# senresearch/BulkLMM.jl

Hardware: AMD Instinct MI355X
Metric: trait x marker LOD tests/sec (higher is better)
Workload: dtype f64

## Files before the change

### bulklmm.jl_amd/csrc/blmm_api.hip

```cpp
#include "blmm_internal.h"
#include "fastmath.h"
#include <algorithm>
#include <cmath>
#include <cstddef>
#include <chrono>
#include <cstring>
#include <limits>
#include <cstdlib>
#include <mutex>

using namespace blmm;

namespace blmm {

int fail(blmm_ctx* ctx, int code, const std::string& msg) {
  if (ctx) ctx->err = msg;
  return code;
}

int ensure(blmm_ctx* ctx, DevBuf& b, size_t bytes) {
  if (&b == &ctx->outL) clear_last(ctx);
  if (&b == &ctx->outL || &b == &ctx->outP) ctx->last_P = nullptr;
  if (bytes == 0) bytes = 8;
  if (b.cap >= bytes) return BLMM_OK;
// ... 223 lines not shown
  return {dCovar, ncov, add_int, ncov + add_int};
}

int prepare_eigen(blmm_ctx* ctx, const blmm_opts* o, int64_t n, const double* dCovar, int64_t ncov, const double* dK,
                  const double* dweights, int centered, Pipe& P, Timer& tm, const EigPre* pre = nullptr) {
  ctx->prep_valid = false;
  if (n < 1 || ncov < 0) return fail(ctx, BLMM_ERR_DIM, "Dimension mismatch.");
  if (n > 2048) return fail(ctx, BLMM_ERR_UNSUPPORTED, "more than 2048 individuals: the device eigensolver (tridiagonalisation + divide and conquer) stops at n = 2048");
  const NullCov nc = null_cov(o, dCovar, ncov);
  const int c = (int)nc.c;
  if (c < 1 || c > CMAX) return fail(ctx, BLMM_ERR_UNSUPPORTED, BLMM_C_ERR);
  if (c >= n) return fail(ctx, BLMM_ERR_DIM, "Dimension mismatch.");
  P.n = (int)n; P.c = c; P.npad = (int)round_up(n, 8); P.ldr = (int)round_up(P.npad, 16);
  int rc;
  if ((rc = ensure(ctx, ctx->U, sizeof(double) * n * n))) return rc;
  if ((rc = ensure(ctx, ctx->lam, sizeof(double) * n))) return rc;
  if ((rc = ensure(ctx, ctx->Zs, sizeof(double) * n * c))) return rc;
  if ((rc = ensure(ctx, ctx->Z0, sizeof(double) * n * c))) return rc;
  if ((rc = ensure(ctx, ctx->Rp, sizeof(double) * (size_t)P.npad * P.ldr))) return rc;
  P.Z0 = ptr<double>(ctx->Z0); P.lam = ptr<double>(ctx->lam);
  if (pre) {
    P.stat = pre->stat;
    ctx->audit_ran = false;
    ctx->brent_cnt_used = false;
    P.big = n > jacobi_lds_max_n();
    bool post_done = false;
    tm.mark();
    if ((rc = launch_jacobi_post(ctx, pre->Ks, pre->V, (int)n, pre->lraw, P.stat, ptr<double>(ctx->Zs), dweights, c, P.npad, P.ldr,
                                 o->decomp_scheme, centered, P.lam, ptr<double>(ctx->U), P.Z0, ptr<double>(ctx->Rp), &post_done))) return rc;
    if (!post_done && (rc = launch_post_eigen(ctx, pre->lraw, pre->V, ptr<double>(ctx->Zs), dweights, (int)n, c, P.npad, P.ldr,
                                              o->decomp_scheme, centered, P.lam, ptr<double>(ctx->U), P.Z0, ptr<double>(ctx->Rp), P.stat))) return rc;
    tm.mark();
    return BLMM_OK;
  }
  if ((rc = ensure(ctx, ctx->Ks, sizeof(double) * n * n))) return rc;
  if ((rc = ensure(ctx, ctx->V, sizeof(double) * (n * n + 4 * n + 16)))) return rc;
  if ((rc = ensure(ctx, ctx->lraw, sizeof(double) * n))) return rc;
  if ((rc = reset_stat(ctx, &P.stat))) return rc;
  tm.mark();
  if ((rc = launch_design(ctx, dK, nc.d, (int)nc.ncov, nc.add_int, dweights, (int)n, ptr<double>(ctx->Ks), ptr<double>(ctx->Zs)))) return rc;
  const double* evec = ptr<double>(ctx->V);
  const char* eig_env = dev_env("BLMM_EIGEN");
  if (!eig_env && ctx->tune.eigen_solver == 1) eig_env = "jacobi";
  if (!eig_env && ctx->tune.eigen_solver == 2) eig_env = "dc";
  const bool big = n > jacobi_lds_max_n();
  P.big = big;
  bool done = false, post_done = false;
  const bool want_dc = eig_env ? std::strcmp(eig_env, "dc") == 0 : big;
  if (!done && want_dc && n >= 3) {
    rc = launch_eig_dc(ctx, ptr<double>(ctx->Ks), (int)n, ptr<double>(ctx->lraw), ptr<double>(ctx->V), P.stat);
    if (rc == BLMM_OK) { done = true; P.big = true; }
    else if (rc != BLMM_ERR_UNSUPPORTED) return rc;
  }
  if (!done) {
    const bool want_fast = !(eig_env && std::strcmp(eig_env, "jacobi") == 0) && n >= 3 && n <= eig_fast_max_n();
    if (want_fast) {
      rc = launch_eig_fast(ctx, ptr<double>(ctx->Ks), (int)n, ptr<double>(ctx->lraw), ptr<double>(ctx->V), P.stat);
      if (rc != BLMM_OK && rc != BLMM_ERR_UNSUPPORTED) return rc;
    }
    if ((rc = launch_jacobi_post(ctx, ptr<double>(ctx->Ks), ptr<double>(ctx->V), (int)n, ptr<double>(ctx->lraw), P.stat, ptr<double>(ctx->Zs),
                                 dweights, c, P.npad, P.ldr, o->decomp_scheme, centered, P.lam, ptr<double>(ctx->U), P.Z0, ptr<double>(ctx->Rp),
                                 &post_done))) return rc;
  }
  if (!post_done && (rc = launch_post_eigen(ctx, ptr<double>(ctx->lraw), evec, ptr<double>(ctx->Zs), dweights, (int)n, c,
                              P.npad, P.ldr, o->decomp_scheme, centered, P.lam, ptr<double>(ctx->U), P.Z0,
                              ptr<double>(ctx->Rp), P.stat))) return rc;
  tm.mark();
  return BLMM_OK;
}

static int flush_upload(blmm_ctx* ctx) {
  if (!ctx->up_pending) return BLMM_OK;
  ctx->up_pending = false;
  for (int i = 0; i < 2; ++i) {
    if (ctx->up_bytes[i]) BLMM_HIP(hipMemcpyAsync(ctx->up_dst[i], ctx->up_src[i], ctx->up_bytes[i], hipMemcpyHostToDevice, ctx->copy));
    if (i == 0) BLMM_HIP(hipEventRecord(ctx->ev_inY, ctx->copy));
  }
  BLMM_HIP(hipEventRecord(ctx->ev_in, ctx->copy));
  ctx->in_wait = true;
  return BLMM_OK;
}

int rotate_markers(blmm_ctx* ctx, Pipe& P, const double* dG, int64_t p);
int start_wbasis(blmm_ctx* ctx, Pipe& P, const double* dG = nullptr, int64_t p = 0, bool xt_recorded = false) {
  int rc;
  const int64_t n = P.n;
  const LrSeg seg = lr_segments(ctx, P.n);
  if ((rc = ensure(ctx, ctx->wbQ, sizeof(double) * (size_t)seg.S * P.npad * n))) return rc;
  if ((rc = ensure(ctx, ctx->wbW, sizeof(double) * (size_t)n * (256 + 16)))) return rc;
  if ((rc = ensure(ctx, ctx->wbRk, sizeof(int) * 4 * LR_SEG_MAX))) return rc;
  if (!xt_recorded) BLMM_HIP(hipEventRecord(ctx->ev_xt, ctx->stream));
  BLMM_HIP(hipStreamWaitEvent(ctx->side, ctx->ev_xt, 0));
  ctx->wb_on_side2 = false;
  if (!dG) {
    OnStream on(ctx, ctx->side);
    return launch_wbasis(ctx, P.lam, (int)n, P.npad, seg, ptr<double>(ctx->wbW), ptr<double>(ctx->wbQ), ptr<int>(ctx->wbRk), P.stat);
  }
  {
    BLMM_HIP(hipStreamWaitEvent(ctx->side2, ctx->ev_xt, 0));
    ctx->wb_on_side2 = true;
    OnStream on(ctx, ctx->side2);
    if ((rc = launch_wbasis(ctx, P.lam, (int)n, P.npad, seg, ptr<double>(ctx->wbW), ptr<double>(ctx->wbQ), ptr<int>(ctx->wbRk), P.stat))) return rc;
  }
  OnStream on(ctx, ctx->side);
  if (ctx->in_wait) BLMM_HIP(hipStreamWaitEvent(ctx->side, ctx->ev_in, 0));
  if ((rc = rotate_markers(ctx, P, dG, p))) return rc;
  BLMM_HIP(hipEventRecord(ctx->ev_wb, ctx->side));
  return BLMM_OK;
}

int rotate_traits(blmm_ctx* ctx, Pipe& P, const double* dY, int64_t m) {
  if (m < 0) return fail(ctx, BLMM_ERR_DIM, "Dimension mismatch.");
  P.m = m; P.ldy = round_up(m > 0 ? m : 1, 128);
  int rc = ensure(ctx, ctx->Yt, sizeof(double) * (size_t)P.npad * P.ldy);
  if (rc) return rc;
  P.Yt = ptr<double>(ctx->Yt);
  return launch_rotate(ctx, ptr<double>(ctx->Rp), P.ldr, P.n, P.npad, dY, m, P.Yt, P.ldy, P.ldy);
}
int rotate_markers(blmm_ctx* ctx, Pipe& P, const double* dG, int64_t p) {
  if (p < 0) return fail(ctx, BLMM_ERR_DIM, "Dimension mismatch.");
  P.p = p; P.ldx = round_up(p > 0 ? p : 1, 128);
  int rc = ensure(ctx, ctx->Xt, sizeof(double) * (size_t)P.npad * P.ldx);
  if (rc) return rc;
  P.Xt = ptr<double>(ctx->Xt);
  return launch_rotate(ctx, ptr<double>(ctx->Rp), P.ldr, P.n, P.npad, dG, p, P.Xt, P.ldx, P.ldx);
}

int prepare(blmm_ctx* ctx, const blmm_opts* o, const double* dY, int64_t n, int64_t m, const double* dG, int64_t p,
            const double* dCovar, int64_t ncov, const double* dK, const double* dweights, int centered, Pipe& P, Timer& tm,
            bool early_wbasis = false, bool grid_side = false, bool skip_markers = false, const EigPre* pre = nullptr) {
  if (m < 0 || p < 0) return fail(ctx, BLMM_ERR_DIM, "Dimension mismatch.");
  const bool forks = m > 0 && p > 0 && (early_wbasis || grid_side);
  ctx->stop_event_used = false;
  ctx->stop_event_next = forks ? ctx->ev_xt : nullptr;
  int rc = prepare_eigen(ctx, o, n, dCovar, ncov, dK, dweights, centered, P, tm, pre);
  const bool xt_recorded = ctx->stop_event_used;
  ctx->stop_event_next = nullptr; ctx->stop_event_used = false;
  if (rc) return rc;
  if (ctx->up_pending) {
    if ((rc = flush_upload(ctx))) return rc;
    BLMM_HIP(hipStreamWaitEvent(ctx->stream, ctx->ev_inY, 0));
  }
  const bool up_flight = ctx->in_wait;
  static const bool rot_side = !(dev_env("BLMM_ROTATE_SIDE") && dev_env("BLMM_ROTATE_SIDE")[0] == '0');
  const bool side_g = early_wbasis && m > 0 && p > 0 && rot_side && n <= 160;
  if (early_wbasis && m > 0 && p > 0 && (rc = start_wbasis(ctx, P, side_g ? dG : nullptr, p, xt_recorded))) return rc;
  P.xt_side = side_g;
  if (grid_side && !early_wbasis && m > 0 && p > 0 && rot_side && n <= 160) {
    if (!xt_recorded) BLMM_HIP(hipEventRecord(ctx->ev_xt, ctx->stream));
    BLMM_HIP(hipStreamWaitEvent(ctx->side, ctx->ev_xt, 0));
    if (ctx->in_wait) BLMM_HIP(hipStreamWaitEvent(ctx->side, ctx->ev_in, 0));
    OnStream on(ctx, ctx->side);
    if ((rc = rotate_markers(ctx, P, dG, p))) return rc;
    P.xt_side = true;
  }
  if ((rc = rotate_traits(ctx, P, dY, m))) return rc;
  if (skip_markers) { P.p = p; P.ldx = round_up(p > 0 ? p : 1, 128); P.Xt = nullptr; }
  else if (!P.xt_side) {
    if (up_flight) BLMM_HIP(hipStreamWaitEvent(ctx->stream, ctx->ev_in, 0));
    if ((rc = rotate_markers(ctx, P, dG, p))) return rc;
  }
  ctx->in_wait = false;
  tm.mark();
  return BLMM_OK;
}

NullModel null_model(const Pipe& P, const blmm_opts* o) {
  NullModel nm;
  nm.n = P.n; nm.c = P.c; nm.npad = P.npad; nm.reml = o->reml ? 1 : 0;
  nm.optim_interval = o->optim_interval < 1 ? 1 : o->optim_interval;
  nm.prior_a = o->prior_variance; nm.prior_b = o->prior_sample_size;
  return nm;
}

int stage_to_device(blmm_ctx* ctx, DevBuf& dst, const void* src, size_t bytes) {
  blmm_ctx::GridSlot* slot = nullptr;
  for (auto& g : ctx->gstage)
    if (g.cap >= bytes && (!g.used || hipEventQuery(g.ev) == hipSuccess)) { slot = &g; break; }
  if (!slot) {
    blmm_ctx::GridSlot g;
    g.cap = bytes < 4096 ? 4096 : bytes;
    void* h = nullptr;
    BLMM_HIP(hipHostMalloc(&h, g.cap, hipHostMallocDefault));
    g.h = h;
    if (hipEventCreateWithFlags(&g.ev, hipEventDisableTiming) != hipSuccess) { (void)hipHostFree(h); return fail(ctx, BLMM_ERR_HIP, "hipEventCreate failed"); }
    ctx->gstage.push_back(g);
    slot = &ctx->gstage.back();
  }
  std::memcpy(slot->h, src, bytes);
  BLMM_HIP(hipMemcpyAsync(dst.p, slot->h, bytes, hipMemcpyHostToDevice, ctx->stream));
  BLMM_HIP(hipEventRecord(slot->ev, ctx->stream));
  slot->used = true;
  return BLMM_OK;
}

int check_grid(blmm_ctx* ctx, const double* h2_grid_host, int64_t ngrid) {
  if (!h2_grid_host || ngrid < 1) return fail(ctx, BLMM_ERR_INVALID, "h2 grid is empty");
  for (int64_t g = 0; g < ngrid; ++g) {
    const double h = h2_grid_host[g];
    if (std::isinf(h / (1.0 - h))) return fail(ctx, BLMM_ERR_H2_ONE, "Heritability of 1 is not allowed.");
  }
  return BLMM_OK;
}

int grid_to_device(blmm_ctx* ctx, const double* h2_grid_host, int64_t ngrid, double** out) {
  int rc;
  if ((rc = check_grid(ctx, h2_grid_host, ngrid)) || (rc = ensure(ctx, ctx->gridd, sizeof(double) * ngrid))) return rc;
  const size_t bytes = sizeof(double) * (size_t)ngrid;
  if (ctx->grid_async) {
    if ((rc = stage_to_device(ctx, ctx->gridd, h2_grid_host, bytes))) return rc;
  } else {
    BLMM_HIP(hipMemcpyAsync(ctx->gridd.p, h2_grid_host, bytes, hipMemcpyHostToDevice, ctx->stream));
    BLMM_HIP(hipStreamSynchronize(ctx->stream));
  }
  *out = ptr<double>(ctx->gridd);
  return BLMM_OK;
}

ScanArgs scan_args(blmm_ctx* ctx, const Pipe& P, const double* panels, int64_t ldp, double* L, int64_t ldL, int64_t m) {
  ScanArgs a;
  a.Xt = P.Xt; a.ldx = P.ldx; a.P = panels; a.ldp = ldp; a.pstride = (int64_t)P.npad * ldp;
  a.ks = P.npad / 4; a.n = P.n; a.p = P.p; a.m = m; a.L = L; a.ldL = ldL;
  a.isx = nullptr; a.ld_isx = 0; a.bin = nullptr; a.stat = P.stat; a.logtab = ptr<double>(ctx->logtab); a.lodtab = ptr<double>(ctx->lodtab);
  a.Pv = ctx->pv_cur; a.ldPv = ctx->pv_cur_ld; a.pvtab = ptr<double>(ctx->pvtab);
  a.red = ctx->red_cur;
  a.c = P.c;
  lod_poly5_host(-0.5 * (double)P.n, a.lodc);
  return a;
}

double lr_tolerance(const blmm_ctx* ctx) {
  const char* e = dev_env("BLMM_LR_TOL");
  return e ? atof(e) : ctx->tune.lr_tol;
}

int64_t lr_ldq(const Pipe& P) { return P.ldy + 128 + LR_TILE * LR_SEG_MAX; }
static LrRegion lr_region(const Pipe& P, int r) {
  LrRegion rg;
  rg.col0 = r * lr_ldq(P); rg.ncol = lr_ldq(P); rg.counts = P.stat + ST_LR_SHARED0 + 2 * r; rg.segcnt = P.stat + 24 + 20 * r;
  return rg;
}

int lr_begin(blmm_ctx* ctx, const Pipe& P, bool wbasis_started) {
  int rc;
  ctx->lr_last_ldq = lr_ldq(P); ctx->lr_last_m = P.m;
  const int64_t ldp = 2 * lr_ldq(P), tstride = (int64_t)P.npad * P.ldx;
  if ((rc = ensure(ctx, ctx->lrPerm, sizeof(int) * (size_t)ldp))) return rc;
  if ((rc = ensure(ctx, ctx->lrDen0, sizeof(double) * (size_t)P.ldx))) return rc;
  const LrSeg seg = lr_segments(ctx, P.n);
  if ((rc = ensure(ctx, ctx->lrT, sizeof(double) * (size_t)seg.S * (1 + P.c) * tstride))) return rc;
  if ((rc = ensure(ctx, ctx->lrC, sizeof(double) * (size_t)P.npad * ldp))) return rc;
  if ((rc = ensure(ctx, ctx->lrL, sizeof(double) * (size_t)(P.c * (P.c + 1) / 2) * ldp))) return rc;
  if ((rc = ensure(ctx, ctx->lrFlag, sizeof(int) * (size_t)ldp))) return rc;
  if ((rc = ensure(ctx, ctx->lrPart, sizeof(double) * 2 * (size_t)((P.n + 63) / 64) * ldp))) return rc;
  if ((rc = ensure(ctx, ctx->panels, sizeof(double) * (size_t)P.npad * ldp))) return rc;
  if ((rc = ensure(ctx, ctx->wbQ, sizeof(double) * (size_t)seg.S * P.npad * P.n))) return rc;
  if ((rc = ensure(ctx, ctx->wbW, sizeof(double) * (size_t)P.n * (256 + 16)))) return rc;
  if ((rc = ensure(ctx, ctx->wbRk, sizeof(int) * 4 * LR_SEG_MAX))) return rc;
  int* rk = ptr<int>(ctx->wbRk);
  if (!(wbasis_started && P.xt_side)) {
    BLMM_HIP(hipEventRecord(ctx->ev_fork, ctx->stream));
    BLMM_HIP(hipStreamWaitEvent(ctx->side, ctx->ev_fork, 0));
  }
  const bool on2 = wbasis_started && P.xt_side && ctx->wb_on_side2;
  hipStream_t lr_side = on2 ? ctx->side2 : ctx->side;
  OnStream on(ctx, lr_side);
  if (!wbasis_started && (rc = launch_wbasis(ctx, P.lam, P.n, P.npad, seg, ptr<double>(ctx->wbW), ptr<double>(ctx->wbQ), rk, P.stat))) return rc;
  BLMM_HIP(hipEventRecord(ctx->ev_q, lr_side));
  if (on2) BLMM_HIP(hipStreamWaitEvent(lr_side, ctx->ev_wb, 0));
  if ((rc = launch_lr_tpanels(ctx, P.Xt, P.ldx, P.p, P.n, P.c, P.npad, P.Z0, ptr<double>(ctx->wbQ), rk, seg, ptr<double>(ctx->lrT), tstride,
                              ptr<double>(ctx->lrDen0)))) return rc;
  BLMM_HIP(hipEventRecord(ctx->ev_join, lr_side));
  return BLMM_OK;
}

namespace {
double lr_shared_tol(const blmm_ctx* ctx) {
  const char* e = dev_env("BLMM_LR_SHARED");
  const bool on = e ? e[0] != '0' : ctx->tune.lr_shared != 0;
  return on ? lr_tolerance(ctx) : 0.0;
}
LrArgs lr_args(blmm_ctx* ctx, const Pipe& P, const LrRegion& rg, double* dL, int64_t ldL) {
  const int64_t ldp = 2 * lr_ldq(P);
  LrArgs la;
  la.s = scan_args(ctx, P, ptr<double>(ctx->panels), ldp, dL, ldL, P.m + 192 < rg.ncol ? P.m + 192 : rg.ncol);
  la.Cp = ptr<double>(ctx->lrC); la.T = ptr<double>(ctx->lrT); la.tstride = (int64_t)P.npad * P.ldx; la.Ls = ptr<double>(ctx->lrL);
  la.rk = ptr<int>(ctx->wbRk); la.c = P.c; la.perm = ptr<int>(ctx->lrPerm); la.rg = rg; la.den0 = ptr<double>(ctx->lrDen0);
  la.skip_shared = 0;
  la.seg = lr_segments(ctx, P.n);
  return la;
}
int lr_region_scan(blmm_ctx* ctx, const Pipe& P, const LrRegion& rg, double* dL, int64_t ldL) {
  static const bool lean = !(dev_env("BLMM_LR_LEAN") && dev_env("BLMM_LR_LEAN")[0] == '0');
  static const bool serial = dev_env("BLMM_LR_SERIAL") && dev_env("BLMM_LR_SERIAL")[0] == '1';
  if (serial) { (void)hipStreamSynchronize(ctx->side); (void)hipStreamSynchronize(ctx->side2); (void)hipStreamSynchronize(ctx->stream); }
  LrArgs la = lr_args(ctx, P, rg, dL, ldL);
  int rc;
  if (lean) {
    ScanArgs a = la.s;
    a.isx = la.den0; a.ld_isx = P.ldx; a.bin = nullptr;
    a.perm = la.perm; a.col0 = rg.col0; a.count = rg.counts;
    if ((rc = launch_scan_shared(ctx, a))) return rc;
    la.skip_shared = 1;
  }
  return launch_scan_lr(ctx, la);
}
int lr_region_panels(blmm_ctx* ctx, const Pipe& P, const NullModel& nm, const double* dh2, const LrRegion& rg) {
  return launch_lr_panels(ctx, nm, P.Yt, P.ldy, P.m, P.Z0, P.lam, dh2, ptr<double>(ctx->wbQ), ptr<int>(ctx->wbRk), lr_segments(ctx, P.n), ptr<int>(ctx->lrPerm),
                          rg, ptr<double>(ctx->panels), ptr<double>(ctx->lrC), ptr<double>(ctx->lrL), 2 * lr_ldq(P), P.stat);
}
int lr_region_resid(blmm_ctx* ctx, const Pipe& P, const NullModel& nm, const double* dh2, const LrRegion& rg) {
  OnStream on(ctx, ctx->side);
  return launch_lr_resid(ctx, nm, P.m, lr_tolerance(ctx), P.lam, dh2, ptr<double>(ctx->wbQ), ptr<int>(ctx->wbRk), lr_segments(ctx, P.n), ptr<int>(ctx->lrPerm), rg,
                         ptr<double>(ctx->lrC), 2 * lr_ldq(P), ptr<int>(ctx->lrFlag), ptr<double>(ctx->lrPart), P.stat, ctx->red_cur.flags);
}
int lr_fix(blmm_ctx* ctx, const Pipe& P, const NullModel& nm, const double* dh2, double* dL, int64_t ldL) {
  if (ctx->red_cur.pmax && !ctx->red_cur.flags) return BLMM_OK;
  return launch_scan_fix(ctx, nm, P.Xt, P.ldx, P.p, ptr<double>(ctx->panels), ptr<double>(ctx->lrL), 2 * lr_ldq(P), P.Z0, P.lam, dh2,
                         ptr<int>(ctx->lrFlag), ptr<int>(ctx->lrPerm), dL, ldL, P.stat, ctx->red_cur);
}
}

int illcond_rescan(blmm_ctx* ctx, const Pipe& P, const NullModel& nm, int64_t m, const double* dh2, double* dL, int64_t ldL) {
  if (P.c < 2 || m <= 0 || P.p <= 0) return BLMM_OK;
  int rc = ensure(ctx, ctx->illList, sizeof(int) * (size_t)m);
  if (rc) return rc;
  const bool patch = ctx->red_cur.pmax && ctx->red_cur.flags;
  if (!patch && (rc = launch_illcond_flag(ctx, nm, m, P.Z0, P.lam, dh2, ptr<int>(ctx->illList), P.stat))) return rc;
  if (ctx->red_cur.pmax && !patch) return BLMM_OK;
  return launch_scan_qr(ctx, nm, P.Yt, P.ldy, P.Xt, P.ldx, P.p, P.Z0, P.lam, dh2, ptr<int>(ctx->illList), dL, ldL, P.stat, ctx->red_cur);
}

int lr_finish(blmm_ctx* ctx, const Pipe& P, const NullModel& nm, const double* dh2, double* dL, int64_t ldL, Timer& tm) {
  int rc;
  const LrRegion rg = lr_region(P, 0);
  const LrSeg seg = lr_segments(ctx, P.n);
  hipStream_t main_stream = ctx->stream;
  BLMM_HIP(hipStreamWaitEvent(main_stream, ctx->ev_join, 0));
  if ((rc = launch_lr_classify(ctx, P.n, P.m, lr_shared_tol(ctx), P.lam, dh2, nullptr, nullptr, nullptr, ptr<int>(ctx->lrPerm), rg, seg))) return rc;
  if ((rc = lr_region_panels(ctx, P, nm, dh2, rg))) return rc;
  tm.mark();
  const bool ahead = ctx->red_cur.flags != nullptr;
  if (ahead && P.c >= 2 && (rc = ensure(ctx, ctx->illList, sizeof(int) * (size_t)P.m))) return rc;
  BLMM_HIP(hipEventRecord(ctx->ev_fork, main_stream));
  BLMM_HIP(hipStreamWaitEvent(ctx->side, ctx->ev_fork, 0));
  if ((rc = lr_region_resid(ctx, P, nm, dh2, rg))) return rc;
  if (ahead && P.c >= 2) {
    OnStream on(ctx, ctx->side);
    if ((rc = launch_illcond_flag(ctx, nm, P.m, P.Z0, P.lam, dh2, ptr<int>(ctx->illList), P.stat, ctx->red_cur.flags))) return rc;
  }
  BLMM_HIP(hipEventRecord(ctx->ev_join, ctx->side));
  if (ahead && ctx->red_cur.want_trip) BLMM_HIP(hipStreamWaitEvent(main_stream, ctx->ev_join, 0));
// ... 30 lines not shown
        (rc = lr_region_panels(ctx, P, nm, dh2, r1))) return rc;
  }
  BLMM_HIP(hipEventRecord(ctx->ev_b2, ctx->side2));
  tm.mark();
  BLMM_HIP(hipStreamWaitEvent(ctx->side, ctx->ev_b1, 0));
  if ((rc = lr_region_resid(ctx, P, nm, dh2, r0))) return rc;
  const bool ahead = ctx->red_cur.flags != nullptr && ctx->red_cur.want_trip;
  if (ahead) {
    BLMM_HIP(hipEventRecord(ctx->ev_join, ctx->side));
    BLMM_HIP(hipStreamWaitEvent(main_stream, ctx->ev_join, 0));
  }
  if ((rc = lr_region_scan(ctx, P, r0, dL, ldL))) return rc;
  BLMM_HIP(hipStreamWaitEvent(ctx->side, ctx->ev_b2, 0));
  if ((rc = lr_region_resid(ctx, P, nm, dh2, r1))) return rc;
  BLMM_HIP(hipEventRecord(ctx->ev_join, ctx->side));
  BLMM_HIP(hipStreamWaitEvent(main_stream, ctx->ev_b2, 0));
  if (ahead) BLMM_HIP(hipStreamWaitEvent(main_stream, ctx->ev_join, 0));
  if ((rc = lr_region_scan(ctx, P, r1, dL, ldL))) return rc;
  BLMM_HIP(hipStreamWaitEvent(main_stream, ctx->ev_join, 0));
  if ((rc = lr_fix(ctx, P, nm, dh2, dL, ldL))) return rc;
  if ((rc = illcond_rescan(ctx, P, nm, P.m, dh2, dL, ldL))) return rc;
  tm.mark();
  return BLMM_OK;
}

}

extern "C" {

int blmm_version(void) { return BLMM_VERSION; }

int blmm_device_count(void) {
  int n = 0;
  if (hipGetDeviceCount(&n) != hipSuccess) return 0;
  return n;
}

const char* blmm_err_string(int code) {
  switch (code) {
    case BLMM_OK: return "ok";
    case BLMM_ERR_INVALID: return "invalid argument";
    case BLMM_ERR_DIM: return "Dimension mismatch.";
    case BLMM_ERR_H2_ONE: return "Heritability of 1 is not allowed.";
    case BLMM_ERR_DECOMP: return "Please choose either `eigen` or `svd` for decomposition of the kinship matrix.";
    case BLMM_ERR_METHOD: return "unknown bulkscan method";
    case BLMM_ERR_ONE_TRAIT: return "Can only handle one trait.";
    case BLMM_ERR_NO_INTERCEPT: return "Intercept has to be added when no other covariate is given.";
    case BLMM_ERR_ZERO_NORM: return "Dividing by zeros: the input vector can not contain any zeros!";
    case BLMM_ERR_NPERMS: return "The required number of permutations must be a positive integer.";
    case BLMM_ERR_UNSUPPORTED: return "unsupported configuration";
    case BLMM_ERR_NO_DEVICE: return "no usable HIP device";
    case BLMM_ERR_HIP: return "HIP runtime error";
    case BLMM_ERR_ALLOC: return "device allocation failed";
  }
  return "unknown error";
}

int blmm_create(int device_id, void* hip_stream, blmm_ctx** out) {
  if (!out) return BLMM_ERR_INVALID;
  *out = nullptr;
  int ndev = 0;
  if (hipGetDeviceCount(&ndev) != hipSuccess || ndev <= 0 || device_id < 0 || device_id >= ndev) return BLMM_ERR_NO_DEVICE;
  if (hipSetDevice(device_id) != hipSuccess) return BLMM_ERR_NO_DEVICE;
  blmm_ctx* ctx = new blmm_ctx();
  ctx->device = device_id;
  if (hip_stream == BLMM_STREAM_NULL) {
    ctx->stream = nullptr;
  } else if (hip_stream) {
    ctx->stream = reinterpret_cast<hipStream_t>(hip_stream);
  } else {
    if (hipStreamCreateWithFlags(&ctx->stream, hipStreamNonBlocking) != hipSuccess) { delete ctx; return BLMM_ERR_HIP; }
    ctx->own_stream = true;
  }
  if (hipStreamCreateWithFlags(&ctx->side, hipStreamNonBlocking) != hipSuccess ||
      hipEventCreateWithFlags(&ctx->ev_fork, hipEventDisableTiming) != hipSuccess ||
      hipEventCreateWithFlags(&ctx->ev_join, hipEventDisableTiming) != hipSuccess ||
      hipEventCreateWithFlags(&ctx->ev_xt, hipEventDisableTiming) != hipSuccess ||
      hipStreamCreateWithFlags(&ctx->side2, hipStreamNonBlocking) != hipSuccess ||
      hipEventCreateWithFlags(&ctx->ev_b1, hipEventDisableTiming) != hipSuccess ||
      hipEventCreateWithFlags(&ctx->ev_b2, hipEventDisableTiming) != hipSuccess ||
      hipEventCreateWithFlags(&ctx->ev_q, hipEventDisableTiming) != hipSuccess ||
      hipEventCreateWithFlags(&ctx->ev_m, hipEventDisableTiming) != hipSuccess ||
      hipEventCreateWithFlags(&ctx->ev_wb, hipEventDisableTiming) != hipSuccess ||
      hipStreamCreateWithFlags(&ctx->copy, hipStreamNonBlocking) != hipSuccess ||
      hipEventCreateWithFlags(&ctx->ev_in, hipEventDisableTiming) != hipSuccess ||
      hipEventCreateWithFlags(&ctx->ev_inY, hipEventDisableTiming) != hipSuccess ||
      hipEventCreateWithFlags(&ctx->ev_call, hipEventDisableTiming) != hipSuccess) {
    blmm_destroy(ctx);
    return BLMM_ERR_HIP;
  }
  {
    int cus = 0;
    if (hipDeviceGetAttribute(&cus, hipDeviceAttributeMultiprocessorCount, device_id) == hipSuccess) ctx->num_cus = cus;
    void* hp = nullptr;
    if (hipHostMalloc(&hp, 64, hipHostMallocMapped) != hipSuccess) { blmm_destroy(ctx); return BLMM_ERR_HIP; }
    std::memset(hp, 0, 64);
    ctx->hflag = reinterpret_cast<volatile int64_t*>(hp);
  }
  if (ensure(ctx, ctx->logtab, sizeof(blmm_log_table_host)) != BLMM_OK ||
      hipMemcpy(ctx->logtab.p, blmm_log_table_host, sizeof(blmm_log_table_host), hipMemcpyHostToDevice) != hipSuccess ||
      ensure(ctx, ctx->lodtab, sizeof(blmm_lod_table_host)) != BLMM_OK ||
      hipMemcpy(ctx->lodtab.p, blmm_lod_table_host, sizeof(blmm_lod_table_host), hipMemcpyHostToDevice) != hipSuccess ||
      ensure(ctx, ctx->pvtab, sizeof(blmm_pv_table_host)) != BLMM_OK ||
      hipMemcpy(ctx->pvtab.p, blmm_pv_table_host, sizeof(blmm_pv_table_host), hipMemcpyHostToDevice) != hipSuccess) {
    blmm_destroy(ctx);
    return BLMM_ERR_HIP;
  }
  *out = ctx;
  return BLMM_OK;
}

void blmm_destroy(blmm_ctx* ctx) {
  if (!ctx) return;
  hipSetDevice(ctx->device);
  hipStreamSynchronize(ctx->stream);
  DevBuf* bufs[] = {&ctx->Ks, &ctx->V, &ctx->lam, &ctx->U, &ctx->Zs, &ctx->Z0, &ctx->Rp, &ctx->Yt, &ctx->Xt, &ctx->panels,
                    &ctx->iyy, &ctx->h2, &ctx->h2idx, &ctx->sig2, &ctx->ell, &ctx->isx, &ctx->stat, &ctx->gridd, &ctx->misc,
                    &ctx->EllTab, &ctx->inY, &ctx->inG, &ctx->inK, &ctx->inCov, &ctx->inW, &ctx->outL, &ctx->outH2,
                    &ctx->tmpA, &ctx->tmpB, &ctx->tmpC, &ctx->perm, &ctx->r0, &ctx->altbuf, &ctx->logtab, &ctx->lraw,
                    &ctx->wbQ, &ctx->wbW, &ctx->wbRk, &ctx->lrT, &ctx->lrC, &ctx->lrL, &ctx->lrFlag, &ctx->lrPart, &ctx->lrPerm, &ctx->lrDen0, &ctx->eigW, &ctx->xf32, &ctx->pf32, &ctx->brSt, &ctx->brList, &ctx->illList, &ctx->qrSlab, &ctx->lodtab, &ctx->dynFac, &ctx->pvtab, &ctx->outP, &ctx->redbuf, &ctx->redtrip, &ctx->altC, &ctx->rf32, &ctx->btG, &ctx->redflag, &ctx->bperm,
                    &ctx->locoK, &ctx->locoPart, &ctx->locoChr, &ctx->locoStat, &ctx->locoKs, &ctx->locoV, &ctx->locoLraw};
  for (DevBuf* b : bufs) if (b->p) hipFree(b->p);
  for (auto& s : ctx->evsets) for (auto& e : s.e) (void)hipEventDestroy(e);
  if (ctx->side) { (void)hipStreamSynchronize(ctx->side); (void)hipStreamDestroy(ctx->side); }
  if (ctx->ev_fork) (void)hipEventDestroy(ctx->ev_fork);
  if (ctx->ev_join) (void)hipEventDestroy(ctx->ev_join);
  if (ctx->ev_xt) (void)hipEventDestroy(ctx->ev_xt);
  if (ctx->ev_b1) (void)hipEventDestroy(ctx->ev_b1);
  if (ctx->ev_b2) (void)hipEventDestroy(ctx->ev_b2);
  if (ctx->ev_q) (void)hipEventDestroy(ctx->ev_q);
  if (ctx->ev_m) (void)hipEventDestroy(ctx->ev_m);
  if (ctx->ev_wb) (void)hipEventDestroy(ctx->ev_wb);
  if (ctx->ev_in) (void)hipEventDestroy(ctx->ev_in);
  if (ctx->ev_inY) (void)hipEventDestroy(ctx->ev_inY);
  if (ctx->ev_call) (void)hipEventDestroy(ctx->ev_call);
  for (auto& g : ctx->gstage) {
    if (g.ev) { (void)hipEventSynchronize(g.ev); (void)hipEventDestroy(g.ev); }
    if (g.h) (void)hipHostFree(g.h);
  }
  if (ctx->copy) { (void)hipStreamSynchronize(ctx->copy); (void)hipStreamDestroy(ctx->copy); }
  if (ctx->side2) { (void)hipStreamSynchronize(ctx->side2); (void)hipStreamDestroy(ctx->side2); }
  if (ctx->own_stream) hipStreamDestroy(ctx->stream);
  if (ctx->hflag) (void)hipHostFree(const_cast<int64_t*>(ctx->hflag));
  destroy_host_stage(ctx->hstage);
  delete ctx;
}

const char* blmm_last_error(const blmm_ctx* ctx) { return ctx ? ctx->err.c_str() : "ctx is NULL"; }

int blmm_set_stream(blmm_ctx* ctx, void* hip_stream) {
  if (!ctx) return BLMM_ERR_INVALID;
  hipStreamSynchronize(ctx->stream);
  if (ctx->own_stream) { hipStreamDestroy(ctx->stream); ctx->own_stream = false; }
  if (hip_stream == BLMM_STREAM_NULL) ctx->stream = nullptr;
  else if (hip_stream) ctx->stream = reinterpret_cast<hipStream_t>(hip_stream);
  else {
    if (hipStreamCreateWithFlags(&ctx->stream, hipStreamNonBlocking) != hipSuccess) return fail(ctx, BLMM_ERR_HIP, "hipStreamCreate");
    ctx->own_stream = true;
  }
  return BLMM_OK;
}

int blmm_set_timing(blmm_ctx* ctx, int on) {
  if (!ctx) return BLMM_ERR_INVALID;
  ctx->timing = on != 0;
  return BLMM_OK;
}

int blmm_read_timings(blmm_ctx* ctx, double* sums_ms, int64_t* ncalls) {
  if (!ctx || !sums_ms || !ncalls) return BLMM_ERR_INVALID;
  BLMM_HIP(hipStreamSynchronize(ctx->stream));
  for (int i = 0; i < 6; ++i) sums_ms[i] = 0.0;
  for (size_t k = 0; k < ctx->ev_used; ++k) {
    double t[6];
    phase_times(ctx->evsets[k], t);
    for (int i = 0; i < 6; ++i) sums_ms[i] += t[i];
  }
  *ncalls = (int64_t)ctx->ev_used;
  ctx->ev_used = 0;
  return BLMM_OK;
}

int blmm_lowrank_profile(blmm_ctx* ctx, int64_t* out) {
  if (!ctx || !out) return BLMM_ERR_INVALID;
  for (int i = 0; i < 2 + 2 * LR_SEG_MAX; ++i) out[i] = 0;
  if (!ctx->stat.p || !ctx->wbRk.p) return BLMM_OK;
  BLMM_HIP(hipSetDevice(ctx->device));
  int64_t h[NSTAT];
  int rk[4 * LR_SEG_MAX];
  BLMM_HIP(hipMemcpyAsync(h, ctx->stat.p, sizeof(h), hipMemcpyDeviceToHost, ctx->stream));
  BLMM_HIP(hipMemcpyAsync(rk, ctx->wbRk.p, sizeof(rk), hipMemcpyDeviceToHost, ctx->stream));
  BLMM_HIP(hipStreamSynchronize(ctx->stream));
  int S = 0;
  for (int s = 0; s < LR_SEG_MAX; ++s) {
    const int64_t cnt = h[24 + s] + h[44 + s];
    if (cnt > 0) { S = s + 1; out[2 + 2 * s] = cnt; out[3 + 2 * s] = rk[4 * s]; }
  }
  out[0] = S; out[1] = h[ST_LR_SHARED0] + h[ST_LR_SHARED1];
  return BLMM_OK;
}

int blmm_lowrank_columns(blmm_ctx* ctx, int64_t m, int32_t* col_out, int64_t* region_width, int64_t* counts_out) {
  if (!ctx || !col_out || m < 0) return BLMM_ERR_INVALID;
  for (int64_t j = 0; j < m; ++j) col_out[j] = -1;
  if (region_width) *region_width = ctx->lr_last_ldq;
  if (counts_out) for (int i = 0; i < 4; ++i) counts_out[i] = 0;
  if (!ctx->lrPerm.p || !ctx->stat.p || ctx->lr_last_ldq <= 0) return BLMM_OK;
  BLMM_HIP(hipSetDevice(ctx->device));
  const int64_t ldq = ctx->lr_last_ldq;
  std::vector<int> perm((size_t)(2 * ldq));
  int64_t h[NSTAT];
  BLMM_HIP(hipMemcpyAsync(perm.data(), ctx->lrPerm.p, sizeof(int) * perm.size(), hipMemcpyDeviceToHost, ctx->stream));
  BLMM_HIP(hipMemcpyAsync(h, ctx->stat.p, sizeof(h), hipMemcpyDeviceToHost, ctx->stream));
  BLMM_HIP(hipStreamSynchronize(ctx->stream));
  for (int r = 0; r < 2; ++r) {
// ... 157 lines not shown
  ctx->pv_armed = false; ctx->pv_out = nullptr; ctx->pv_ld = 0; ctx->pv_df = 1;
  return r;
}
void pv_hand_over(blmm_ctx* ctx, const PvReq& r) {
  ctx->pv_armed = r.armed; ctx->pv_out = r.out; ctx->pv_ld = r.ld; ctx->pv_df = r.df;
}
struct PvCall {
  blmm_ctx* ctx; PvReq req; double* P = nullptr; int64_t ld = 0; bool fused = false, owned = false;
  PvCall(blmm_ctx* c, const PvReq& r) : ctx(c), req(r) {}
  ~PvCall() { ctx->pv_cur = nullptr; ctx->pv_cur_ld = 0; }
  int resolve(int64_t p, int64_t m) {
    if (!req.armed) return BLMM_OK;
    if (p <= 0 || m <= 0) return BLMM_OK;
    P = req.out; ld = req.ld;
    if (P && ld < p) { P = nullptr; return fail(ctx, BLMM_ERR_INVALID, "log10p output: ldP < p"); }
    if (!P) {
      int rc = ensure(ctx, ctx->outP, sizeof(double) * (size_t)p * (size_t)m);
      if (rc) return rc;
      P = ptr<double>(ctx->outP); ld = p; owned = true;
    }
    return BLMM_OK;
  }
  int begin(const Pipe& Pp, const blmm_opts* o) {
    int rc = resolve(Pp.p, Pp.m);
    if (rc || !P) return rc;
    const char* pf = dev_env("BLMM_PVAL_FUSED");
    fused = req.df == 1 && o->method != BLMM_ALT_GRID && (pf ? pf[0] != '0' : ctx->tune.pval_fused != 0);
    if (fused) { ctx->pv_cur = P; ctx->pv_cur_ld = ld; }
    return BLMM_OK;
  }
  int finish(int64_t p, int64_t m, const double* dL, int64_t ldL) {
    ctx->pv_cur = nullptr; ctx->pv_cur_ld = 0;
    if (!P) return BLMM_OK;
    if (!fused) { int rc = launch_lod2log10p(ctx, dL, p, m, ldL, (int)req.df, P, ld); if (rc) return rc; }
    if (owned) { ctx->last_P = P; ctx->last_P_ld = ld; ctx->last_P_df = req.df; }
    return BLMM_OK;
  }
};
}
}

static int isx_maybe_side(blmm_ctx* ctx, const Pipe& P, const NullModel& nm, const double* dgrid, int ngrid) {
  int rc;
  if ((rc = ensure(ctx, ctx->isx, sizeof(double) * (size_t)ngrid * P.ldx))) return rc;
  {
    OnStream on(ctx, P.xt_side ? ctx->side : ctx->stream);
    if ((rc = launch_isx(ctx, nm, P.Xt, P.ldx, P.p, P.Z0, P.lam, dgrid, ngrid, ptr<double>(ctx->isx), P.ldx, P.stat))) return rc;
  }
  if (P.xt_side) {
    BLMM_HIP(hipEventRecord(ctx->ev_join, ctx->side));
    BLMM_HIP(hipStreamWaitEvent(ctx->stream, ctx->ev_join, 0));
  }
  return BLMM_OK;
}

static int scan_pipeline(blmm_ctx* ctx, const blmm_opts* opts, Pipe& P, Timer& tm, bool lowrank, bool wbasis_started, double* dgrid,
                         const double* h2_grid_host, int64_t ngrid, double* dL_out, int64_t ldL, double* dh2_out, blmm_status* status,
                         const PvReq& pvreq, int64_t ldH = -1) {
  int rc;
  const int64_t m = P.m, p = P.p;
  const NullModel nm = null_model(P, opts);
  const int64_t ldp = P.ldy;
  PvCall pvc(ctx, pvreq);
  if ((rc = pvc.begin(P, opts))) return rc;
  if (m == 0) { tm.mark(); tm.mark(); tm.mark(); return end_call(ctx, P, status, &tm); }
  if (p == 0) {
    if (opts->method == BLMM_NULL_EXACT) {
      if ((rc = launch_brent(ctx, nm, P.Yt, P.ldy, m, P.Z0, P.lam, dh2_out, nullptr, nullptr, P.stat))) return rc;
    } else if (opts->method == BLMM_NULL_GRID) {
      if ((rc = ensure(ctx, ctx->h2idx, sizeof(int) * (size_t)m))) return rc;
      if ((rc = launch_loglik_grid(ctx, nm, P.Yt, P.ldy, m, P.Z0, P.lam, dgrid, (int)ngrid, nullptr, ptr<int>(ctx->h2idx), dh2_out, P.stat))) return rc;
    }
    tm.mark(); tm.mark(); tm.mark();
    return end_call(ctx, P, status, &tm);
  }

  if (opts->method == BLMM_NULL_EXACT) {
    if (lowrank) {
      if ((rc = lr_begin(ctx, P, wbasis_started))) return rc;
      const char* split_env = dev_env("BLMM_LR_SPLIT");
      const bool split_on = (ctx->red_cur.flags && P.c >= 2) ? false
                          : split_env ? split_env[0] != '0' : (ctx->tune.lr_split < 0 ? m >= 8192 : ctx->tune.lr_split != 0);
      BrentSplit sp;
      if ((rc = launch_brent(ctx, nm, P.Yt, P.ldy, m, P.Z0, P.lam, dh2_out, nullptr, nullptr, P.stat, split_on ? 1 : 0, &sp))) return rc;
      tm.mark();
      if (sp.active) { if ((rc = lr_finish_split(ctx, P, nm, dh2_out, dL_out, ldL, tm, sp))) return rc; }
      else if ((rc = lr_finish(ctx, P, nm, dh2_out, dL_out, ldL, tm))) return rc;
    } else {
      if ((rc = launch_brent(ctx, nm, P.Yt, P.ldy, m, P.Z0, P.lam, dh2_out, nullptr, nullptr, P.stat))) return rc;
      tm.mark();
      if ((rc = ensure(ctx, ctx->panels, sizeof(double) * (size_t)(2 + P.c) * P.npad * ldp))) return rc;
      if ((rc = launch_panels(ctx, nm, P.Yt, P.ldy, m, P.Z0, P.lam, dh2_out, 1, ptr<double>(ctx->panels), ldp, P.stat))) return rc;
      tm.mark();
      ScanArgs a = scan_args(ctx, P, ptr<double>(ctx->panels), ldp, dL_out, ldL, m);
      if ((rc = launch_scan_exact(ctx, a, P.c))) return rc;
      if ((rc = illcond_rescan(ctx, P, nm, m, dh2_out, dL_out, ldL))) return rc;
      tm.mark();
    }
    if (opts->compat_flags & BLMM_FLAG_H2_AUDIT) {
      double gridh[16];
      for (int g = 0; g < 16; ++g) gridh[g] = g / 16.0;
      double* dg = nullptr;
      if ((rc = grid_to_device(ctx, gridh, 16, &dg))) return rc;
      if ((rc = ensure(ctx, ctx->EllTab, sizeof(double) * (size_t)16 * m))) return rc;
      if ((rc = launch_loglik_grid(ctx, nm, P.Yt, P.ldy, m, P.Z0, P.lam, dg, 16, ptr<double>(ctx->EllTab), nullptr, nullptr, P.stat))) return rc;
      if ((rc = launch_h2_audit(ctx, ptr<double>(ctx->EllTab), 16, m, P.stat))) return rc;
      ctx->audit_ran = true;
    }
  } else if (opts->method == BLMM_NULL_GRID) {
    if ((rc = ensure(ctx, ctx->h2idx, sizeof(int) * (size_t)m))) return rc;
    if ((rc = launch_loglik_grid(ctx, nm, P.Yt, P.ldy, m, P.Z0, P.lam, dgrid, (int)ngrid, nullptr, ptr<int>(ctx->h2idx), dh2_out, P.stat))) return rc;
    tm.mark();
    if ((rc = ensure(ctx, ctx->panels, sizeof(double) * (size_t)P.npad * ldp))) return rc;
    if ((rc = launch_panels(ctx, nm, P.Yt, P.ldy, m, P.Z0, P.lam, dh2_out, 0, ptr<double>(ctx->panels), ldp, P.stat))) return rc;
    if ((rc = isx_maybe_side(ctx, P, nm, dgrid, (int)ngrid))) return rc;
    tm.mark();
    ScanArgs a = scan_args(ctx, P, ptr<double>(ctx->panels), ldp, dL_out, ldL, m);
    a.isx = ptr<double>(ctx->isx); a.ld_isx = P.ldx; a.bin = ptr<int>(ctx->h2idx);
    if ((rc = launch_scan_table(ctx, a))) return rc;
    tm.mark();
  } else {
    if ((rc = ensure(ctx, ctx->EllTab, sizeof(double) * (size_t)ngrid * m))) return rc;
    if ((rc = launch_loglik_grid(ctx, nm, P.Yt, P.ldy, m, P.Z0, P.lam, dgrid, (int)ngrid, ptr<double>(ctx->EllTab), nullptr, nullptr, P.stat))) return rc;
    tm.mark();
    if ((rc = ensure(ctx, ctx->panels, sizeof(double) * (size_t)ngrid * P.npad * ldp))) return rc;
    if ((rc = ensure(ctx, ctx->h2, sizeof(double) * (size_t)m))) return rc;
    if (nm.c <= CTPL) {
      if ((rc = launch_panels(ctx, nm, P.Yt, P.ldy, m, P.Z0, P.lam, nullptr, 0, ptr<double>(ctx->panels), ldp, P.stat, dgrid, (int)ngrid))) return rc;
    } else {
      for (int64_t g = 0; g < ngrid; ++g) {
        if ((rc = fill(ctx, ptr<double>(ctx->h2), m, h2_grid_host[g]))) return rc;
        if ((rc = launch_panels(ctx, nm, P.Yt, P.ldy, m, P.Z0, P.lam, ptr<double>(ctx->h2), 0,
                                ptr<double>(ctx->panels) + (size_t)g * P.npad * ldp, ldp, P.stat))) return rc;
      }
    }
    if ((rc = isx_maybe_side(ctx, P, nm, dgrid, (int)ngrid))) return rc;
    if ((rc = ensure(ctx, ctx->altC, sizeof(double) * (size_t)ngrid * m))) return rc;
    if ((rc = launch_alt_ctab(ctx, ptr<double>(ctx->EllTab), (int)ngrid, m, P.n, ptr<double>(ctx->altC)))) return rc;
    tm.mark();
    AltArgs aa;
    aa.s = scan_args(ctx, P, ptr<double>(ctx->panels), ldp, dL_out, ldL, m);
    aa.s.isx = ptr<double>(ctx->isx); aa.s.ld_isx = P.ldx;
    aa.ngrid = (int)ngrid; aa.EllTab = ptr<double>(ctx->EllTab); aa.grid_dev = dgrid; aa.H2 = dh2_out; aa.ldH = ldH < 0 ? p : ldH;
    aa.Ctab = ptr<double>(ctx->altC);
    aa.counter_quirk = (opts->compat_flags & BLMM_COMPAT_ALT_COUNTER) ? 1 : 0;
    if ((rc = launch_scan_alt(ctx, aa))) return rc;
    tm.mark();
  }
  if ((rc = pvc.finish(p, m, dL_out, ldL))) return rc;
  return end_call(ctx, P, status, &tm);
}

int blmm_set_log10p_output(blmm_ctx* ctx, double* dP_out, int64_t ldP, int64_t chisq_df) {
  if (!ctx) return BLMM_ERR_INVALID;
  if (chisq_df < 0 || chisq_df > 1000000 || (dP_out && ldP < 1)) return fail(ctx, BLMM_ERR_INVALID, "set_log10p_output: bad arguments");
  ctx->pv_armed = chisq_df > 0;
  ctx->pv_out = dP_out; ctx->pv_ld = ldP; ctx->pv_df = chisq_df > 0 ? chisq_df : 1;
  return BLMM_OK;
}

static bool exact_full(const blmm_ctx* ctx) {
  const char* e = dev_env("BLMM_EXACT");
  return e ? std::strcmp(e, "full") == 0 : ctx->tune.exact_full_rank != 0;
}
static bool lowrank_form(const blmm_ctx* ctx, int c, int64_t n) { return !exact_full(ctx) && c <= 3 && n <= 6000; }
static bool wants_lowrank(const blmm_ctx* ctx, const blmm_opts* opts, int64_t n, const double* dCovar, int64_t ncov) {
  return opts->method == BLMM_NULL_EXACT && lowrank_form(ctx, (int)null_cov(opts, dCovar, ncov).c, n);
}

static int bulkscan_dev_impl(blmm_ctx* ctx, const blmm_opts* opts, const double* dY, int64_t n, int64_t m, const double* dG,
                             int64_t p, const double* dCovar, int64_t ncov, const double* dK, const double* dweights,
                             const double* h2_grid_host, int64_t ngrid, double* dL_out, int64_t ldL, double* dh2_out,
                             blmm_status* status, const PvReq& pvreq) {
  int rc = check_opts(ctx, opts);
  if (rc) return rc;
  if (!dY || !dG || !dK || (!dL_out && !ctx->red_cur.pmax) || !dh2_out) return fail(ctx, BLMM_ERR_INVALID, "bulkscan: NULL buffer");
  if (ldL < p) return fail(ctx, BLMM_ERR_INVALID, "bulkscan: ldL < p");
  if ((rc = check_method(ctx, opts)) || (rc = enter_device(ctx))) return rc;
  Timer tm(ctx);
  Pipe P;
  double* dgrid = nullptr;
  if (opts->method != BLMM_NULL_EXACT) {
    if ((rc = grid_to_device(ctx, h2_grid_host, ngrid, &dgrid))) return rc;
  }
  const bool lowrank = wants_lowrank(ctx, opts, n, dCovar, ncov);
  if ((rc = prepare(ctx, opts, dY, n, m, dG, p, dCovar, ncov, dK, dweights, 1, P, tm, lowrank, opts->method != BLMM_NULL_EXACT))) return rc;
  return scan_pipeline(ctx, opts, P, tm, lowrank,  lowrank && m > 0 && p > 0, dgrid, h2_grid_host, ngrid, dL_out, ldL, dh2_out, status, pvreq);
}

int blmm_bulkscan_dev(blmm_ctx* ctx, const blmm_opts* opts, const double* dY, int64_t n, int64_t m, const double* dG,
                      int64_t p, const double* dCovar, int64_t ncov, const double* dK, const double* dweights,
                      const double* h2_grid_host, int64_t ngrid, double* dL_out, int64_t ldL, double* dh2_out,
                      blmm_status* status) {
  if (!ctx) return BLMM_ERR_INVALID;
  const PvReq pvreq = pv_take(ctx);
  ctx->red_cur = RedArgs();
  return bulkscan_dev_impl(ctx, opts, dY, n, m, dG, p, dCovar, ncov, dK, dweights, h2_grid_host, ngrid, dL_out, ldL, dh2_out, status, pvreq);
}

static int reduced_check(blmm_ctx* ctx, const blmm_opts* opts, const double* dY, int64_t n, int64_t m, const double* dG, int64_t p,
                         const double* dK, const blmm_reduced* out, const double* dh2_out, const char* who) {
  int rc = check_opts(ctx, opts);
  if (rc) return rc;
  if (!out || !dY || !dG || !dK || (!dh2_out && opts->method != BLMM_ALT_GRID)) return fail(ctx, BLMM_ERR_INVALID, std::string(who) + ": NULL buffer");
  if (out->cap < 0 || (out->cap > 0 && (!out->ti || !out->tj || !out->tlod)) || (out->want_triplets && !out->count))
    return fail(ctx, BLMM_ERR_INVALID, std::string(who) + ": triplet buffers");
  if ((rc = check_method(ctx, opts))) return rc;
  if (n < 1 || m < 0 || p < 0 || p > 0x7fffffffLL || m > 0x7fffffffLL) return fail(ctx, BLMM_ERR_DIM, "Dimension mismatch.");
  return BLMM_OK;
}

static int reduced_args(blmm_ctx* ctx, const blmm_reduced* out, int64_t p, int64_t m, RedArgs* r, int* nslot) {
  *nslot = 2 * (int)((p + 127) / 128);
  const int64_t ldm = round_up(m, 64);
  int rc = ensure(ctx, ctx->redbuf, (sizeof(double) + sizeof(int)) * (size_t)*nslot * (size_t)ldm);
  if (rc) return rc;
  r->pmax = ptr<double>(ctx->redbuf); r->parg = reinterpret_cast<int*>(r->pmax + (size_t)*nslot * ldm); r->ldm = ldm;
  r->want_trip = out->want_triplets ? 1 : 0; r->thr = out->thr; r->cap = out->cap;
  r->ti = out->ti; r->tj = out->tj; r->tl = out->tlod; r->cnt = reinterpret_cast<unsigned long long*>(out->count);
  if (out->count) BLMM_HIP(hipMemsetAsync(out->count, 0, sizeof(int64_t), ctx->stream));
  return BLMM_OK;
}

static int reduced_resident(blmm_ctx* ctx, const blmm_opts* opts, const double* dY, int64_t n, int64_t m, const double* dG, int64_t p,
                            const double* dCovar, int64_t ncov, const double* dK, const double* dweights, const double* h2_grid_host,
                            int64_t ngrid, const blmm_reduced* out, double* dh2_out, blmm_status* status) {
  const int64_t ldL = p > 0 ? p : 1;
  const size_t pm = (size_t)ldL * (size_t)(m > 0 ? m : 1);
  int rc;
  if ((rc = ensure(ctx, ctx->outL, sizeof(double) * pm))) return rc;
  double* dL = ptr<double>(ctx->outL);
  double* dH = dh2_out;
  if (opts->method == BLMM_ALT_GRID) {
    if ((rc = ensure(ctx, ctx->altbuf, sizeof(double) * pm))) return rc;
    dH = ptr<double>(ctx->altbuf);
  }
  if ((rc = bulkscan_dev_impl(ctx, opts, dY, n, m, dG, p, dCovar, ncov, dK, dweights, h2_grid_host, ngrid, dL, ldL, dH, status, PvReq()))) return rc;
  if (m > 0) set_last(ctx, dL, p, m);
  if (out->colmax && m > 0 && (rc = launch_colmax(ctx, dL, p, m, ldL, out->colmax, out->argmax))) return rc;
  if (out->want_triplets && (rc = launch_threshold(ctx, dL, p, m, ldL, out->thr, out->cap, out->ti, out->tj, out->tlod, out->count))) return rc;
  return BLMM_OK;
}

static int reduced_impl(blmm_ctx* ctx, const blmm_opts* opts, const double* dY, int64_t n, int64_t m, const double* dG, int64_t p,
                        const double* dCovar, int64_t ncov, const double* dK, const double* dweights, const double* h2_grid_host,
                        int64_t ngrid, const blmm_reduced* out, double* dh2_out, blmm_status* status, int* route_out) {
  int rc = reduced_check(ctx, opts, dY, n, m, dG, p, dK, out, dh2_out, "bulkscan_reduced");
  if (rc) return rc;
  BLMM_HIP(hipSetDevice(ctx->device));
  const bool native = p > 0 && m > 0 && (opts->method == BLMM_NULL_GRID || wants_lowrank(ctx, opts, n, dCovar, ncov));
  if (route_out) *route_out = 0;
  if (native) {
    RedArgs r;
    int nslot;
    if ((rc = reduced_args(ctx, out, p, m, &r, &nslot))) return rc;
    ctx->red_cur = r;
    rc = bulkscan_dev_impl(ctx, opts, dY, n, m, dG, p, dCovar, ncov, dK, dweights, h2_grid_host, ngrid, nullptr, p, dh2_out, status, PvReq());
    ctx->red_cur = RedArgs();
    if (rc) { (void)hipStreamSynchronize(ctx->stream); return rc; }
    if ((rc = launch_red_final(ctx, r, nslot, m, out->colmax, out->argmax))) return rc;
    int64_t h[NSTAT];
    BLMM_HIP(hipMemcpyAsync(h, ctx->stat.p, sizeof(h), hipMemcpyDeviceToHost, ctx->stream));
    BLMM_HIP(hipStreamSynchronize(ctx->stream));
    if ((rc = check_sticky(ctx))) return rc;
    if (h[ST_LR_FIX] == 0 && h[ST_ILLCOND] == 0) { if (route_out) *route_out = 1; return BLMM_OK; }
  }
  if ((rc = reduced_resident(ctx, opts, dY, n, m, dG, p, dCovar, ncov, dK, dweights, h2_grid_host, ngrid, out, dh2_out, status))) {
    (void)hipStreamSynchronize(ctx->stream);
    return rc;
// ... 964 lines not shown
```

### bulklmm.jl_amd/csrc/blmm_internal.h

```cpp
#pragma once
#include <hip/hip_runtime.h>
#include <hip/hip_ext.h>
#include <stdint.h>
#include <stdlib.h>
#include <string>
#include <vector>
#include "../../include/bulklmm_hip.h"

namespace blmm {

typedef double d2 __attribute__((ext_vector_type(2)));
typedef double d4 __attribute__((ext_vector_type(4)));

constexpr int CMAX = 32;
constexpr int CTPL = 8;
constexpr int CFAST = 4;
#define BLMM_C_ERR "number of null covariates (incl. intercept) must be 1..32"
#define BLMM_FOR_EACH_C(M) \
  case 1: M(1); break; case 2: M(2); break; case 3: M(3); break; case 4: M(4); break; \
  case 5: M(5); break; case 6: M(6); break; case 7: M(7); break; case 8: M(8); break;
constexpr int TILE_T = 64;
constexpr int TILE_I = 128;
constexpr int NSTAT = 64;

enum StatIdx { ST_NEG_EIG = 0, ST_NONPOS_W = 1, ST_ZERO_NORM = 2, ST_NAN_LOD = 3, ST_BRENT_MAXIT = 4, ST_JACOBI_SWEEPS = 5,
               ST_EIG_CYCLES = 6, ST_EIG_TICKS = 7 ,
               ST_LR_RANK = 8 ,
               ST_LR_RESID2 = 9 , ST_LR_FIX = 10 ,
               ST_EIG_ABORT = 11 ,
               ST_LR_SHARED0 = 12, ST_LR_OTHER0 = 13, ST_LR_SHARED1 = 14, ST_LR_OTHER1 = 15
               ,
               ST_H2_BOUNDARY = 16, ST_H2_MULTIMODAL = 17, ST_ILLCOND = 18,
               ST_EIG_FAST = 19 , ST_EIG_BAD = 20 ,
               ST_BRENT_CNT = 21 ,
               ST_EIG_DONE = 23  };

inline int64_t round_up(int64_t x, int64_t q) { return (x + q - 1) / q * q; }

inline const char* dev_env(const char* name) {
  const char* on = getenv("BLMM_DEV_ENV");
  return (on && on[0] == '1') ? getenv(name) : nullptr;
}
struct Tuning {
  double lr_tol = 1e-13;
  double illcond_rho = 1e-4;
  int exact_full_rank = 0;
  int pval_libm = 0;
  int pval_fused = 1;
  int lr_segments = 0;
  int lr_shared = 1;
  int lr_split = -1;
  int f32_rotation = 1;
  int eigen_solver = 0;
  int bulk_perm_cols = 0;
};

struct DevBuf {
  void* p = nullptr;
  size_t cap = 0;
};

struct Pipe {
  int n = 0, c = 0, npad = 0, ldr = 0;
  int64_t m = 0, p = 0, ldy = 0, ldx = 0;
  double *Yt = nullptr, *Xt = nullptr, *Z0 = nullptr, *lam = nullptr;
  int64_t* stat = nullptr;
  bool big = false;
  bool xt_side = false;
};

struct RedArgs {
  double* pmax = nullptr; int* parg = nullptr; int64_t ldm = 0;
  int want_trip = 0; double thr = 0.0; int64_t cap = 0;
  int32_t* ti = nullptr; int32_t* tj = nullptr; double* tl = nullptr; unsigned long long* cnt = nullptr;
  int* flags = nullptr;
};
}

namespace blmm { struct HostStage; }

struct blmm_ctx {
  int device = 0;
  hipStream_t stream = nullptr;
  bool own_stream = false;
  bool timing = false;
  std::string err;
  blmm::DevBuf Ks, V, lam, U, Zs, Z0, Rp, Yt, Xt, panels, iyy, h2, h2idx, sig2, ell, isx, stat, gridd, misc, EllTab,
      inY, inG, inK, inCov, inW, outL, outH2, tmpA, tmpB, tmpC, perm, r0, altbuf, logtab, lraw, wbQ, wbW, wbRk, lrT, lrC, lrL, lrFlag, lrPart, lrPerm, lrDen0, eigW, xf32, pf32, brSt, brList, illList, qrSlab, lodtab, dynFac, pvtab, outP, redbuf, redtrip, altC, rf32, btG, redflag, bperm,
      locoK, locoPart, locoChr, locoStat, locoKs, locoV, locoLraw;
  struct EvSet { hipEvent_t e[8]; int n; };
  std::vector<EvSet> evsets;
  size_t ev_used = 0;
  hipStream_t side = nullptr, side2 = nullptr;
  hipEvent_t ev_fork = nullptr, ev_join = nullptr, ev_xt = nullptr, ev_b1 = nullptr, ev_b2 = nullptr, ev_q = nullptr, ev_m = nullptr, ev_wb = nullptr;
  hipEvent_t stop_event_next = nullptr; bool stop_event_used = false;
  bool wb_on_side2 = false;
  hipStream_t copy = nullptr; hipEvent_t ev_in = nullptr, ev_inY = nullptr;
  bool up_pending = false, in_wait = false;
  const void* up_src[2] = {nullptr, nullptr}; void* up_dst[2] = {nullptr, nullptr}; size_t up_bytes[2] = {0, 0};
  int num_cus = 0;
  volatile int64_t* hflag = nullptr;
  const double* last_L = nullptr; int64_t last_p = 0, last_m = 0; bool last_f32 = false;
  bool pv_armed = false; double* pv_out = nullptr; int64_t pv_ld = 0, pv_df = 1;
  double* pv_cur = nullptr; int64_t pv_cur_ld = 0;
  const double* last_P = nullptr; int64_t last_P_ld = 0, last_P_df = 0;
  blmm::RedArgs red_cur; int last_reduced_route = 0;
  bool grid_async = false;
  struct GridSlot { void* h = nullptr; size_t cap = 0; hipEvent_t ev = nullptr; bool used = false; };
  std::vector<GridSlot> gstage;
  hipEvent_t ev_call = nullptr;
  blmm::Tuning tune;
  bool perm_ready = false; int perm_ready_n = 0; int64_t perm_ready_nperms = 0; uint64_t perm_ready_seed = 0;
  int64_t lr_last_ldq = 0, lr_last_m = 0;
  blmm::Pipe prep; bool prep_valid = false;
  bool brent_cnt_used = false;
  bool audit_ran = false;
  int eig_plan_n = -1;
  blmm::HostStage* hstage = nullptr;
};

namespace blmm {

inline void set_last(blmm_ctx* ctx, const double* L, int64_t p, int64_t m, bool f32 = false) {
  ctx->last_L = L; ctx->last_p = p; ctx->last_m = m; ctx->last_f32 = f32;
}
inline void clear_last(blmm_ctx* ctx) { set_last(ctx, nullptr, 0, 0); }

int fail(blmm_ctx* ctx, int code, const std::string& msg);
#define BLMM_HIP(call)                                                                              \
  do {                                                                                              \
    hipError_t e__ = (call);                                                                        \
    if (e__ != hipSuccess)                                                                          \
      return blmm::fail(ctx, BLMM_ERR_HIP, std::string(#call) + ": " + hipGetErrorString(e__));     \
  } while (0)

int ensure(blmm_ctx* ctx, DevBuf& b, size_t bytes);
struct GridKernelGuard {
  blmm_ctx* ctx; int dev; int rc = 0;
  explicit GridKernelGuard(blmm_ctx* c);
  int record();
  ~GridKernelGuard();
  GridKernelGuard(const GridKernelGuard&) = delete;
  GridKernelGuard& operator=(const GridKernelGuard&) = delete;
};
int copy_to_host(blmm_ctx* ctx, void* dst, const void* dsrc, size_t bytes);
struct HostCall {
  blmm_ctx* ctx;
  bool done = false;
  explicit HostCall(blmm_ctx* c) : ctx(c) {}
  ~HostCall();
  HostCall(const HostCall&) = delete;
  HostCall& operator=(const HostCall&) = delete;
  int begin();
  int up(void* dst, const void* src, size_t bytes);
  int up(DevBuf& b, const void* src, size_t bytes);
  int up_opt(DevBuf& b, const double* src, int64_t count, const double** dev);
  int defer_yg(const double* Y, size_t ybytes, const double* G, size_t gbytes);
  struct In { const double *Y, *G, *K, *Cov, *W; int64_t ncov; };
  int inputs(const double* Y, int64_t n, int64_t m, const double* G, int64_t p, const double* K, const double* Covar, int64_t ncov,
             const double* weights, bool defer, In* in);
  int down(void* dst, const void* dsrc, size_t bytes);
  int finish(bool sync = true);
};
void destroy_host_stage(HostStage* hs);
template <typename T>
inline T* ptr(DevBuf& b) { return reinterpret_cast<T*>(b.p); }

struct Design {
  int n = 0, c = 0, npad = 0;
  int ldr = 0;
};

int launch_design(blmm_ctx* ctx, const double* dK, const double* dCovar, int ncov, int add_intercept,
                  const double* dweights, int n, double* Ks, double* Zs);
struct PostEigenArgs;
int launch_jacobi(blmm_ctx* ctx, double* A, double* V, int n, double* lraw, int64_t* stat, const PostEigenArgs* pe = nullptr, bool* fused = nullptr);
int launch_jacobi_post(blmm_ctx* ctx, double* A, double* V, int n, double* lraw, int64_t* stat, const double* Zs, const double* dweights,
                       int c, int npad, int ldr, int decomp, int centered, double* lam, double* U, double* Z0, double* Rp, bool* fused);
int launch_eig_dc(blmm_ctx* ctx, const double* A, int n, double* lraw, double* evec, int64_t* stat);
int eig_dc_max_n(const blmm_ctx* ctx);
int launch_eig_fast(blmm_ctx* ctx, const double* A, int n, double* lraw, double* evec, int64_t* stat);
int launch_eig_fast_batch(blmm_ctx* ctx, const double* A, int64_t sA, int n, int nb, double* lraw, int64_t sL, double* evec, int64_t sE,
                          int64_t* stat, int64_t sS);
int eig_fast_max_n();
int jacobi_lds_max_n();
int launch_post_eigen(blmm_ctx* ctx, const double* lraw, const double* V, const double* Zs, const double* dweights, int n,
                      int c, int npad, int ldr, int decomp, int centered, double* lam, double* U, double* Z0, double* Rp,
                      int64_t* stat);
int launch_rotate(blmm_ctx* ctx, const double* Rp, int ldr, int n, int npad, const double* In, int64_t ncols,
                  double* Out, int64_t ldo, int64_t ncols_pad);
int launch_rotate_single(blmm_ctx* ctx, const double* Rp, int ldr, int n, int npad, const double* In, int64_t ncols, double* Out, int64_t ldo);
int launch_untranspose(blmm_ctx* ctx, const double* In, int64_t ld, int n, int64_t ncols, double* Out);

struct NullModel {
  int n, c, npad, reml, optim_interval;
  double prior_a, prior_b;
};
struct BrentSplit {
  bool active = false;
  const int* fin = nullptr;
  const int* list = nullptr;
  const unsigned int* cnt = nullptr;
};
int launch_brent(blmm_ctx* ctx, const NullModel& nm, const double* Yt, int64_t ldy, int64_t m, const double* Z0,
                 const double* lam, double* h2, double* sigma2, double* ell, int64_t* stat, int phase = 0,
                 BrentSplit* sp = nullptr);
int launch_alt_brent(blmm_ctx* ctx, const NullModel& nm, const double* Yt, int64_t ldy, const double* Xt, int64_t ldx, int64_t p,
                     const double* Z0, const double* lam, const double* h2null, int true_w, double* lod, double* h2each,
                     int64_t* stat, int64_t m = 1, int64_t ldL = 0, int64_t ldH = 0);
int launch_loglik_grid(blmm_ctx* ctx, const NullModel& nm, const double* Yt, int64_t ldy, int64_t m, const double* Z0,
                       const double* lam, const double* grid_dev, int ngrid, double* EllTab, int* h2idx, double* h2,
                       int64_t* stat);
int launch_h2_audit(blmm_ctx* ctx, const double* EllTab, int ngrid, int64_t m, int64_t* stat);
int launch_panels(blmm_ctx* ctx, const NullModel& nm, const double* Yt, int64_t ldy, int64_t m, const double* Z0,
                  const double* lam, const double* h2, int full, double* panels, int64_t ldp, int64_t* stat,
                  const double* gridv = nullptr, int ngrid = 0);
int launch_isx(blmm_ctx* ctx, const NullModel& nm, const double* Xt, int64_t ldx, int64_t p, const double* Z0,
               const double* lam, const double* grid_dev, int ngrid, double* isx, int64_t ld_isx, int64_t* stat);
int launch_kinship(blmm_ctx* ctx, const double* dG, int64_t n, int64_t p, double* dK, double* partial);
int loco_kinship_splits(int64_t n, int64_t nchr);
int launch_kinship_loco(blmm_ctx* ctx, const double* dG, int64_t n, const int64_t* dchr, int64_t nchr, int64_t digits, double* dK,
                        double* partial, int nsplit);
int launch_colmax(blmm_ctx* ctx, const double* L, int64_t p, int64_t m, int64_t ldL, double* mx, int64_t* arg);
int launch_lod2log10p(blmm_ctx* ctx, const double* dL, int64_t p, int64_t m, int64_t ldL, int df, double* dP, int64_t ldP);
int launch_perm_gen(blmm_ctx* ctx, int n, int64_t nperms, uint64_t seed);
int launch_perm_panel(blmm_ctx* ctx, const NullModel& nm, const double* Yt, int64_t ldy, const double* Z0,
                      const double* lam, const double* h2, const int32_t* perm_idx, int64_t nperms, uint64_t seed,
                      int orig, double* panel, int64_t ldp, int64_t* stat);

struct ScanArgs {
  const double* Xt; int64_t ldx;
  const double* P; int64_t ldp; int64_t pstride;
  int ks;
  int n;
  int64_t p, m;
  double* L; int64_t ldL;
  const double* isx; int64_t ld_isx; const int* bin;
  const int* perm = nullptr; int64_t col0 = 0; const int64_t* count = nullptr;
  int c = 1;
  const double* logtab;
  const double* lodtab;
  double lodc[6];
  int64_t* stat;
  double* Pv = nullptr; int64_t ldPv = 0; const double* pvtab = nullptr;
  RedArgs red;
};
int launch_threshold(blmm_ctx* ctx, const double* dL, int64_t p, int64_t m, int64_t ldL, double thr, int64_t cap,
                     int32_t* di, int32_t* dj, double* dlod, int64_t* dcount);
int launch_red_final(blmm_ctx* ctx, const RedArgs& r, int nslot, int64_t m, double* mx, int64_t* arg);
int launch_red_info(blmm_ctx* ctx, const int64_t* stat, int route, const int64_t* count, int64_t* info);
int launch_scan_exact(blmm_ctx* ctx, const ScanArgs& a, int c);
constexpr int LR_TILE = 64;
struct LrRegion {
  int64_t col0 = 0, ncol = 0;
  int64_t* counts = nullptr;
  int64_t* segcnt = nullptr;
};
constexpr int LR_SEG_MAX = 8;
struct LrSeg {
  int S = 1;
  double edge[LR_SEG_MAX + 1] = {0.0, 2.0, 2.0, 2.0, 2.0, 2.0, 2.0, 2.0, 2.0};
};
__host__ __device__ inline int64_t lr_seg_width(int64_t cnt) { return (cnt + LR_TILE - 1) / LR_TILE * LR_TILE; }
__host__ __device__ inline int lr_seg_of(int64_t dist, const int64_t* segcnt, int S) {
  for (int s = 0; s + 1 < S; ++s) {
    const int64_t w = lr_seg_width(segcnt[s]);
    if (dist < w) return s;
    dist -= w;
  }
  return S - 1;
}
struct LrArgs {
  ScanArgs s;
  const double* Cp;
  const double* T; int64_t tstride;
  const double* Ls;
  const int* rk;
  LrSeg seg;
  const int* perm;
  LrRegion rg;
  const double* den0;
  int skip_shared;
  int c;
};
int launch_scan_lr(blmm_ctx* ctx, const LrArgs& la);
int launch_lr_resid(blmm_ctx* ctx, const NullModel& nm, int64_t m, double tol, const double* lam, const double* h2,
                    const double* Q, const int* rk, const LrSeg& seg, const int* perm, const LrRegion& rg, const double* Cp, int64_t ldp,
                    int* flag_list, double* part, int64_t* stat, int* flags = nullptr);
int launch_scan_fix(blmm_ctx* ctx, const NullModel& nm, const double* Xt, int64_t ldx, int64_t p, const double* P0,
                    const double* Ls, int64_t ldp, const double* Z0, const double* lam, const double* h2,
                    const int* flag_list, const int* perm, double* L, int64_t ldL, int64_t* stat, const RedArgs& red = RedArgs());
int launch_lr_classify(blmm_ctx* ctx, int n, int64_t m, double tol, const double* lam, const double* h2, const int* fin,
                       const int* list, const unsigned int* list_cnt, int* perm, const LrRegion& rg, const LrSeg& seg);
int launch_cvt_f32(blmm_ctx* ctx, const double* M, int64_t ld_in, int rows_valid, int64_t cols_valid, float* F,
                   int64_t ld_out, int kblocks);
int launch_rotate_f32(blmm_ctx* ctx, const double* Rp, int ldr, int n, int npad, const double* dG, int64_t p, float* RF, float* XF, int64_t ldxf,
                      const double* a0, int64_t lda, double* v_work , double* num );
int launch_lod_from_num(blmm_ctx* ctx, const double* num, const double* isx, int n, int64_t p, double* lod, int64_t* stat);
int launch_isx_f32(blmm_ctx* ctx, const NullModel& nm, const float* XF, int64_t ldxf, int64_t p, const double* Z0, const double* lam,
                   const double* h2_dev, double* isx, int64_t ld_isx, int64_t* stat);
int launch_scan_f32(blmm_ctx* ctx, const float* XF, int64_t ldxf, const float* PF, int64_t ldpf, int npad, int n,
                    int64_t p, int64_t m, const double* isx, float* L, int64_t ldL, int64_t* stat);
int launch_dyn_brent(blmm_ctx* ctx, const NullModel& nm, const double* Yt, int64_t ldy, int64_t m, const double* Z0, const double* lam,
                     double* h2, double* sigma2, double* ell, int64_t* stat);
int launch_dyn_alt_brent(blmm_ctx* ctx, const NullModel& nm, const double* Yt, int64_t ldy, const double* Xt, int64_t ldx, int64_t p,
                         const double* Z0, const double* lam, const double* h2null, int true_w, double* lod, double* h2each,
                         int64_t* stat, int64_t m, int64_t ldL, int64_t ldH);
int launch_dyn_loglik_grid(blmm_ctx* ctx, const NullModel& nm, const double* Yt, int64_t ldy, int64_t m, const double* Z0,
                           const double* lam, const double* grid_dev, int ngrid, double* EllTab, int* h2idx, double* h2, int64_t* stat);
int launch_dyn_panels(blmm_ctx* ctx, const NullModel& nm, const double* Yt, int64_t ldy, int64_t m, const double* Z0, const double* lam,
                      const double* h2, int full, double* panels, int64_t ldp, int64_t* stat);
int launch_dyn_isx(blmm_ctx* ctx, const NullModel& nm, const double* Xt, int64_t ldx, int64_t p, const double* Z0, const double* lam,
                   const double* grid_dev, int ngrid, double* isx, int64_t ld_isx, int64_t* stat);
int launch_dyn_perm(blmm_ctx* ctx, const NullModel& nm, const double* Yt, int64_t ldy, const double* Z0, const double* lam, const double* h2,
                    const int32_t* perm, int64_t ncols, int orig, double* r0, double* panel, int64_t ldp, int64_t* stat);
int launch_illcond_flag(blmm_ctx* ctx, const NullModel& nm, int64_t m, const double* Z0, const double* lam, const double* h2,
                        int* list, int64_t* stat, int* flags = nullptr);
int launch_scan_qr(blmm_ctx* ctx, const NullModel& nm, const double* Yt, int64_t ldy, const double* Xt, int64_t ldx, int64_t p,
                   const double* Z0, const double* lam, const double* h2, const int* list, double* L, int64_t ldL, int64_t* stat,
                   const RedArgs& red = RedArgs());
LrSeg lr_segments(const blmm_ctx* ctx, int n);
int launch_wbasis(blmm_ctx* ctx, const double* lam, int n, int npad, const LrSeg& seg, double* Wk, double* Q, int* rk, int64_t* stat);
int launch_lr_tpanels(blmm_ctx* ctx, const double* Xt, int64_t ldx, int64_t p, int n, int c, int npad, const double* Z0,
                      const double* Q, const int* rk, const LrSeg& seg, double* T, int64_t tstride, double* den0);
int launch_lr_panels(blmm_ctx* ctx, const NullModel& nm, const double* Yt, int64_t ldy, int64_t m, const double* Z0,
                     const double* lam, const double* h2, const double* Q, const int* rk, const LrSeg& seg, const int* perm, const LrRegion& rg,
                     double* P0, double* Cp, double* Ls, int64_t ldp, int64_t* stat);
int launch_scan_table(blmm_ctx* ctx, const ScanArgs& a);
int launch_scan_shared(blmm_ctx* ctx, const ScanArgs& a);
struct AltArgs {
  ScanArgs s;
  int ngrid; const double* EllTab;  const double* grid_dev; double* H2; int64_t ldH; int counter_quirk;
  const double* Ctab;
};
int launch_scan_alt(blmm_ctx* ctx, const AltArgs& a);
int launch_alt_ctab(blmm_ctx* ctx, const double* EllTab, int ngrid, int64_t m, int n, double* C);
int launch_bperm_panels(blmm_ctx* ctx, const NullModel& nm, const double* Yt, int64_t ldy, const double* Z0, const double* lam,
                        const double* h2c, int64_t mt, const int32_t* perm, int64_t nperms, double* panel, int64_t ldp, int* bin,
                        int64_t* stat);
struct BpermProbs { double v[64]; };
int launch_bperm_summary(blmm_ctx* ctx, const double* mx, const int64_t* arg, int64_t mt, int64_t nperms, const BpermProbs& probs,
                         int nprobs, int64_t j0, double* lod_max, int64_t* lod_argmax, double* max_perms, double* thr, double* pval);
constexpr int BPERM_MAX_NPERMS = 16384;

}

#define BLMM_LAUNCH_STOP(ctx_, kernel_, grid_, block_, lds_, ...)                                                          \
  do {                                                                                                                   \
    if ((ctx_)->stop_event_next) {                                                                                       \
      hipExtLaunchKernelGGL(kernel_, grid_, block_, (std::uint32_t)(lds_), (ctx_)->stream, nullptr, (ctx_)->stop_event_next, 0, __VA_ARGS__); \
      (ctx_)->stop_event_next = nullptr; (ctx_)->stop_event_used = true;                                                 \
    } else hipLaunchKernelGGL(kernel_, grid_, block_, lds_, (ctx_)->stream, __VA_ARGS__);                                 \
  } while (0)
```

### bulklmm.jl_amd/csrc/kernels_eig.hip

```cpp
#include "blmm_internal.h"
#include "fastmath.h"
#include <cmath>
#include <cstdlib>
#include <cstring>

namespace blmm {

#define KCHECK()                                                                                      \
  do {                                                                                                \
    hipError_t e__ = hipGetLastError();                                                               \
    if (e__ != hipSuccess) return fail(ctx, BLMM_ERR_HIP, std::string("kernel launch: ") + hipGetErrorString(e__)); \
  } while (0)

namespace {

constexpr double EPS = 2.220446049250313e-16;
constexpr int LEAF = 32;

template <int CTRL>
__device__ __forceinline__ double dpp_mov(double x) {
  int lo = __double2loint(x), hi = __double2hiint(x);
  lo = __builtin_amdgcn_update_dpp(lo, lo, CTRL, 0xf, 0xf, false);
  hi = __builtin_amdgcn_update_dpp(hi, hi, CTRL, 0xf, 0xf, false);
  return __hiloint2double(hi, lo);
// ... 1329 lines not shown
  }
  __syncthreads();
  if (wave < 2) {
    const double gam = (t < n) ? fabs(sDp[t] + sDm[t] - (sd[t] - l)) : INFINITY;
    const double gmin = -wmax(-gam);
    unsigned long long m = __ballot(gam == gmin);
    const int first = m ? (wave * 64 + (int)__builtin_ctzll(m)) : 0x7fffffff;
    if (lane == 0) { s_red[2 + wave] = gmin; s_cnt[0][wave] = first; }
  }
  __syncthreads();
  if (t == 0) s_r = (s_red[2] <= s_red[3]) ? s_cnt[0][0] : s_cnt[0][1];
  __syncthreads();
  const int r = s_r;
  double fct = 1.0;
  if (t < n) { if (t < r) fct = -quot_fast(se[t], sDp[t]); else if (t > r) fct = -quot_fast(se[t - 1], sDm[t]); }
  __syncthreads();
  double* za = sDp; double* zb = sDm;
  if (t < 128) za[t] = fct;
  __syncthreads();
  for (int s_ = 1; s_ < n; s_ <<= 1) {
    if (t < n) {
      double v = za[t];
      if (t > r && t - s_ > r) v *= za[t - s_]; else if (t < r && t + s_ < r) v *= za[t + s_];
      zb[t] = v;
    }
    __syncthreads();
    double* tmp = za; za = zb; zb = tmp;
  }
  if (wave < 2) {
    const double zt = (t < n) ? za[t] : 0.0;
    const double nr = wsum(zt * zt);
    if (lane == 0) s_red[wave] = nr;
  }
  __syncthreads();
  EPSTAMP(2);
  const double inv = fast_rsqrt(s_red[0] + s_red[1]);
  double res = 0.0;
  if (t < n) {
    auto zat = [&](int i) { return za[i] * inv; };
    const double zi = zat(t);
    g.Zc[(size_t)k * n + t] = zi;
    double rr = (sd[t] - l) * zi;
    if (t > 0) rr = fma(se[t - 1], zat(t - 1), rr);
    if (t < n - 1) rr = fma(se[t], zat(t + 1), rr);
    res = fabs(rr);
    if (!(rr == rr)) res = INFINITY;
  }
  if (t == 0) lam_out[k] = l;
  if (wave < 2) {
    res = wmax(res);
    if (lane == 0) eigf_note(stat, res, 2e-14 * tn);
  }
  EPSTAMP(3);
#ifdef EIGF_PROF
  if (t == 0 && (k == 0 || k == n / 2 || k == n - 1))
    printf("eigf_pairs prof k %d: load %lld | %d rounds %lld | twisted %lld | finish %lld cycles\n", k, pf[0], prounds, pf[1], pf[2], pf[3]);
#endif
}

}

int eig_dc_max_n(const blmm_ctx*) { return 2048; }

int eig_fast_max_n() { return 124; }
static int eig_fast_impl(blmm_ctx* ctx, const double* A, int64_t sA, int n, int nb, double* lraw, int64_t sL, double* evec, int64_t sE,
                         int64_t* stat, int64_t sS) {
  if (nb < 1 || nb > 65535) return fail(ctx, BLMM_ERR_UNSUPPORTED, "eig_fast: 1 .. 65535 matrices per batched launch");
  if (n < 3 || n > eig_fast_max_n()) return BLMM_ERR_UNSUPPORTED;
  int rc;
  const size_t w1 = (size_t)2 * n * n + (size_t)5 * n + 8;
  const int64_t sW = nb > 1 ? round_up((int64_t)w1 + 32, 32) : 0;
  if ((rc = ensure(ctx, ctx->eigW, nb > 1 ? sizeof(double) * (size_t)nb * sW : sizeof(double) * w1 + 256))) return rc;
  const size_t lds = sizeof(double) * ((size_t)n * n + (size_t)9 * n + 8 * 128 + 16) + 64;
  if (lds > 158 * 1024) return BLMM_ERR_UNSUPPORTED;
  double* Vg = ptr<double>(ctx->eigW);
  double* wsb = Vg + (size_t)n * n;
  const EigfWs g = eigf_ws(wsb, n);
  BLMM_HIP(hipFuncSetAttribute(reinterpret_cast<const void*>(&k_eigf_reduce), hipFuncAttributeMaxDynamicSharedMemorySize, (int)lds));
  hipLaunchKernelGGL(k_eigf_reduce, dim3(1, nb), dim3(1024), lds, ctx->stream, A, n, Vg, wsb, stat, sA, sW, sS);
  KCHECK();
  const int64_t sG = nb > 1 ? round_up((int64_t)8 * bt_groups(n), 32) : 0;
  if ((rc = ensure(ctx, ctx->btG, nb > 1 ? sizeof(double) * (size_t)nb * sG : sizeof(double) * 8 * (size_t)bt_groups(n)))) return rc;
  double* btG = ptr<double>(ctx->btG);
  hipLaunchKernelGGL(k_eigf_pairs<256>, dim3(n + (bt_groups(n) + 3) / 4, nb), dim3(256), 0, ctx->stream, n, (const double*)wsb, lraw, stat,
                     (const double*)Vg, btG, sW, sL, sS, sG);
  KCHECK();
  static const bool bt_stage_off = dev_env("BLMM_BT_STAGE") && dev_env("BLMM_BT_STAGE")[0] == '0';
  const int stage_v = (bt_lds_staged(2, n) <= 158 * 1024 && !bt_stage_off) ? 1 : 0;
  const size_t lds_bt = stage_v ? bt_lds_staged(2, n) : bt_lds_chk(2, n);
  BLMM_HIP(hipFuncSetAttribute(reinterpret_cast<const void*>(&k_backtransform<2, 1, 256>), hipFuncAttributeMaxDynamicSharedMemorySize, (int)lds_bt));
  BtBatch bb;
  bb.w = sW; bb.g = sG; bb.z = sE; bb.s = sS;
  hipLaunchKernelGGL((k_backtransform<2, 1, 256>), dim3((n + 3) / 4, nb), dim3(256), lds_bt, ctx->stream, Vg, g.tau, (const double*)btG, n, evec,
                     (const double*)g.Zc, stat, stage_v, bb);
  KCHECK();
  ctx->eig_plan_n = -1;
  return BLMM_OK;
}

int launch_eig_fast(blmm_ctx* ctx, const double* A, int n, double* lraw, double* evec, int64_t* stat) {
  return eig_fast_impl(ctx, A, 0, n, 1, lraw, 0, evec, 0, stat, 0);
}

int launch_eig_fast_batch(blmm_ctx* ctx, const double* A, int64_t sA, int n, int nb, double* lraw, int64_t sL, double* evec, int64_t sE,
                          int64_t* stat, int64_t sS) {
  return eig_fast_impl(ctx, A, sA, n, nb, lraw, sL, evec, sE, stat, sS);
}

int launch_eig_dc(blmm_ctx* ctx, const double* A, int n, double* lraw, double* evec, int64_t* stat) {
  if (n < 3) return fail(ctx, BLMM_ERR_UNSUPPORTED, "eig_dc: n < 3");
  if (n > eig_dc_max_n(ctx)) return BLMM_ERR_UNSUPPORTED;
  const size_t nn = (size_t)n * n;
  static const int leaf_env = dev_env("BLMM_EIG_LEAF") ? atoi(dev_env("BLMM_EIG_LEAF")) : 0;
  const int leaf = (leaf_env >= 2 && leaf_env <= LEAF) ? leaf_env : 12;
  int nl = 1;
  while ((n + nl - 1) / nl > leaf) nl *= 2;
  std::vector<int> bounds(nl + 1);
  for (int i = 0; i <= nl; ++i) bounds[i] = (int)std::llround((double)i * n / nl);
  std::vector<std::vector<int>> levels;
  {
    std::vector<int> cur(bounds);
    while (cur.size() > 2) {
      std::vector<int> nodes, nxt;
      for (size_t i = 0; i + 2 < cur.size(); i += 2) {
        nodes.push_back(cur[i]); nodes.push_back(cur[i + 1]); nodes.push_back(cur[i + 2]);
      }
      for (size_t i = 0; i < cur.size(); i += 2) nxt.push_back(cur[i]);
      levels.push_back(nodes);
      cur = nxt;
    }
  }
  size_t nnodes_total = 0;
  for (auto& l : levels) nnodes_total += l.size() / 3;
  int rc;
  const size_t ints = (size_t)7 * n + 320 + 2 * ABSMAX_PARTS + 2 + 4 * nnodes_total + 3 * nnodes_total + (nl + 1) + 64;
  const size_t dbls = 5 * nn + (size_t)14 * n + nnodes_total + 64;
  if ((rc = ensure(ctx, ctx->eigW, sizeof(double) * dbls + sizeof(int) * ints + 256))) return rc;
  double* base = ptr<double>(ctx->eigW);
  double* V = base; double* Qa = V + nn; double* Qb = Qa + nn; double* Dm = Qb + nn; double* Wt = Dm + nn;
  double* vec = Wt + nn;
  double* d = vec; double* e = d + n; double* tau = e + n; double* lamA = tau + n; double* lamB = lamA + n;
  double* dl = lamB + n; double* zl = dl + n; double* zh = zl + n; double* defld = zh + n; double* lamnew = defld + n;
  double* rotc = lamnew + n; double* rots = rotc + n; double* pbuf = rots + n;
  double* rho = pbuf + 2 * n;
  double* rowbuf = Dm;
  int* ib = reinterpret_cast<int*>(rho + nnodes_total + 8);
  int* colidx = ib; int* deflcol = colidx + n; int* rota = deflcol + n; int* rotb = rota + n; int* posn = rotb + n;
  int* posd = posn + n; int* sync = posd + n;
  int* info = sync + n + 320 + 2 * ABSMAX_PARTS + 2; int* nodes_dev = info + 4 * nnodes_total; int* bounds_dev = nodes_dev + 3 * nnodes_total;
  if (ctx->eig_plan_n != n) {
    std::vector<int> flat;
    for (auto& l : levels) flat.insert(flat.end(), l.begin(), l.end());
    BLMM_HIP(hipMemcpyAsync(nodes_dev, flat.data(), sizeof(int) * flat.size(), hipMemcpyHostToDevice, ctx->stream));
    BLMM_HIP(hipMemcpyAsync(bounds_dev, bounds.data(), sizeof(int) * bounds.size(), hipMemcpyHostToDevice, ctx->stream));
    BLMM_HIP(hipStreamSynchronize(ctx->stream));
    ctx->eig_plan_n = n;
  }
  {
    const int cus = ctx->num_cus > 0 ? ctx->num_cus : 256;
    if (sizeof(double) * ((size_t)7 * n + 128) + 64 > 156 * 1024) return BLMM_ERR_UNSUPPORTED;
    const size_t budget = 156 * 1024 - sizeof(double) * ((size_t)7 * n + 128) - 64;
    int nloc = (int)(budget / (sizeof(double) * (size_t)n));
    int G = nloc >= 1 ? (n + nloc - 1) / nloc : cus + 1;
    const bool glb = G > cus || (dev_env("BLMM_SYTRD_GLB") && dev_env("BLMM_SYTRD_GLB")[0] == '1');
    if (glb) G = 1;
    const int Gmin = G;
    if ((n + 9) / 10 > G) G = std::min(cus, (n + 9) / 10);
    if (const char* ge = dev_env("BLMM_SYTRD_G")) { const int gv = atoi(ge); if (gv >= Gmin && gv <= cus) G = gv; }
// ... 112 lines not shown
```

### bulklmm.jl_amd/csrc/kernels_lowrank.hip

```cpp
#include "blmm_internal.h"
#include <vector>
#include <algorithm>
#include "fastmath.h"
#include <cmath>
#include <cstdlib>
#include <cstring>

namespace blmm {

#define KCHECK()                                                                                      \
  do {                                                                                                \
    hipError_t e__ = hipGetLastError();                                                               \
    if (e__ != hipSuccess) return fail(ctx, BLMM_ERR_HIP, std::string("kernel launch: ") + hipGetErrorString(e__)); \
  } while (0)

constexpr int WB_NS = 256;
constexpr int WB_QCAP = 48;

__device__ __forceinline__ double wave_sum(double x) {
#pragma unroll
  for (int o = 32; o > 0; o >>= 1) x += __shfl_xor(x, o, 64);
  return x;
}

// ... 37 lines not shown
  const double tol2 = 2e-31 * (double)n;
  int R = 0;
  for (; R < n; ++R) {
    if (part == 0) { s_red[s] = res2; s_arg[s] = s; }
    __syncthreads();
    for (int cnt = NS; cnt > 1;) {
      const int o = (cnt + 1) >> 1;
      if (t + o < cnt && (s_red[t + o] > s_red[t] || (s_red[t + o] == s_red[t] && s_arg[t + o] < s_arg[t]))) { s_red[t] = s_red[t + o]; s_arg[t] = s_arg[t + o]; }
      cnt = o;
      __syncthreads();
    }
    const double mx = s_red[0];
    const int piv = s_arg[0];
    __syncthreads();
    if (!(mx > tol2)) break;
    for (int k = t; k < n; k += NT) sq[k] = WLDS ? Wl[k * ldw + piv] : Wg[(size_t)k * ldw + piv];
    __syncthreads();
    for (int pass = 0; pass < 2; ++pass) {
      for (int r = wave; r < R; r += nwave) {
        double d = 0.0;
        if (r < qcap) { for (int k = lane; k < n; k += 64) d = fma(Ql[r * n + k], sq[k], d); }
        else { for (int k = lane; k < n; k += 64) d = fma(Q[(size_t)r * n + k], sq[k], d); }
        d = wave_sum(d);
        if (lane == 0) sd[r] = d;
      }
      __syncthreads();
      for (int k = t; k < n; k += NT) {
        double v = sq[k];
        const int rl = R < qcap ? R : qcap;
        for (int r = 0; r < rl; ++r) v = fma(-sd[r], Ql[r * n + k], v);
        for (int r = rl; r < R; ++r) v = fma(-sd[r], Q[(size_t)r * n + k], v);
        sq[k] = v;
      }
      __syncthreads();
    }
    double pn = 0.0;
    for (int k = t; k < n; k += NT) pn = fma(sq[k], sq[k], pn);
    pn = wave_sum(pn);
    if (lane == 0) s_red[wave] = pn;
    __syncthreads();
    double tot = 0.0;
    for (int w = 0; w < nwave; ++w) tot += s_red[w];
    const double qn = 1.0 / sqrt(tot);
    __syncthreads();
    if (!(tot > 1e-8 * mx)) break;
    for (int k = t; k < n; k += NT) { const double v = sq[k] * qn; sq[k] = v; Q[(size_t)R * n + k] = v; if (R < qcap) Ql[R * n + k] = v; }
    __syncthreads();
    double c = 0.0;
    {
      int k = part;
      for (; k + 7 * TPS < n; k += 8 * TPS) {
        double wv[8];
#pragma unroll
        for (int u = 0; u < 8; ++u) wv[u] = WK(k + u * TPS);
#pragma unroll
        for (int u = 0; u < 8; ++u) c = fma(sq[k + u * TPS], wv[u], c);
      }
      for (; k < n; k += TPS) c = fma(sq[k], WK(k), c);
    }
    TPS_SUM(c);
    double r2 = 0.0;
    {
      int k = part;
      for (; k + 7 * TPS < n; k += 8 * TPS) {
        double wv[8];
#pragma unroll
        for (int u = 0; u < 8; ++u) wv[u] = WK(k + u * TPS);
#pragma unroll
        for (int u = 0; u < 8; ++u) { const double v = fma(-c, sq[k + u * TPS], wv[u]); WK(k + u * TPS) = v; r2 = fma(v, v, r2); }
      }
      for (; k < n; k += TPS) { const double v = fma(-c, sq[k], WK(k)); WK(k) = v; r2 = fma(v, v, r2); }
    }
    TPS_SUM(r2);
    res2 = r2;
    __syncthreads();
  }
#undef WK
#undef TPS_SUM
  if (t == 0) { rk[0] = R; rk[1] = (R + 3) / 4; stat[ST_LR_RANK] = R; }
}

template <int NKR>
__global__ void __launch_bounds__(1024) k_wbasis_reg(const double* __restrict__ lam, int n, double* __restrict__ Q,
                                                     int* __restrict__ rk, int64_t* stat, int qcap, LrSeg seg, int64_t qstride) {
  extern __shared__ __attribute__((aligned(16))) double sh[];
  constexpr int TPS = 4, NS = 256, NT = 1024;
  const int sg = blockIdx.x;
  Q += (int64_t)sg * qstride; rk += 4 * sg;
  double* sq = sh;
  double* sd = sh + n;
  double* Ql = sh + 2 * n;
  __shared__ double s_red[NS];
  __shared__ int s_arg[NS];
  __shared__ int s_neg;
  __shared__ double s_piv_val;
  const int t = threadIdx.x, lane = t & 63, wave = t >> 6, nwave = NT >> 6;
  const int s = t / TPS, part = t % TPS;
  if (t == 0) s_neg = 0;
  __syncthreads();
  for (int k = t; k < n; k += NT) if (lam[k] < -1e-12) s_neg = 1;
  __syncthreads();
  if (s_neg) {
    for (int e = t; e < n * n; e += NT) Q[e] = ((e / n) == (e % n)) ? 1.0 : 0.0;
    if (t == 0) { rk[0] = n; rk[1] = (n + 3) / 4; stat[ST_LR_RANK] = n; }
    return;
  }
  double delta;
  if (seg.S <= 1) delta = (s == 0) ? 0.0 : exp(2.302585092994046 * (-6.0 + 15.0 * (double)(s - 1) / (double)(NS - 2)));
  else {
    const double ha = seg.edge[sg], hb = seg.edge[sg + 1];
    const double da = ha / (1.0 - ha), db = (sg + 1 < seg.S && hb < 1.0) ? hb / (1.0 - hb) : 1e9;
    const double lo = log(fmax(da, 1e-6)), hi = log(fmin(fmax(db, 2e-6), 1e9));
    delta = (s == 0) ? da : exp(lo + (hi - lo) * (double)(s - 1) / (double)(NS - 2));
  }
  double wv[NKR];
  double nrm = 0.0;
#pragma unroll
  for (int i = 0; i < NKR; ++i) {
    const int k = part + TPS * i;
    wv[i] = (k < n) ? 1.0 / fma(delta, fabs(lam[k]), 1.0) : 0.0;
    nrm = fma(wv[i], wv[i], nrm);
  }
  nrm += __shfl_xor(nrm, 1, 64); nrm += __shfl_xor(nrm, 2, 64);
  const double inv = 1.0 / sqrt(nrm);
#pragma unroll
  for (int i = 0; i < NKR; ++i) wv[i] *= inv;
  double res2 = 1.0;
  const double tol2 = 2e-31 * (double)n;
  int R = 0;
  for (; R < n; ++R) {
    if (part == 0) s_red[s] = res2;
    __syncthreads();
    if (wave == 0) {
      double bv = s_red[4 * lane];
      int bi = 4 * lane;
#pragma unroll
      for (int u = 1; u < 4; ++u) { const double v = s_red[4 * lane + u]; if (v > bv) { bv = v; bi = 4 * lane + u; } }
      double wm = bv;
#pragma unroll
      for (int o = 32; o > 0; o >>= 1) wm = fmax(wm, __shfl_xor(wm, o, 64));
      const unsigned long long who = __ballot(bv == wm);
      const int first = who ? __ffsll((long long)who) - 1 : 0;
      const int pi = __shfl(bi, first, 64);
      if (lane == 0) { s_arg[0] = pi; s_piv_val = wm; }
    }
    __syncthreads();
    const double mx = s_piv_val;
    const int piv = s_arg[0];
    if (!(mx > tol2)) break;
    if (s == piv) {
#pragma unroll
      for (int i = 0; i < NKR; ++i) { const int k = part + TPS * i; if (k < n) sq[k] = wv[i]; }
    }
    __syncthreads();
    for (int pass = 0; pass < 2; ++pass) {
      for (int r = wave; r < R; r += nwave) {
        double d = 0.0;
        if (r < qcap) { for (int k = lane; k < n; k += 64) d = fma(Ql[r * n + k], sq[k], d); }
        else { for (int k = lane; k < n; k += 64) d = fma(Q[(size_t)r * n + k], sq[k], d); }
        d = wave_sum(d);
        if (lane == 0) sd[r] = d;
      }
      __syncthreads();
      for (int k = t; k < n; k += NT) {
        double v = sq[k];
        const int rl = R < qcap ? R : qcap;
        for (int r = 0; r < rl; ++r) v = fma(-sd[r], Ql[r * n + k], v);
        for (int r = rl; r < R; ++r) v = fma(-sd[r], Q[(size_t)r * n + k], v);
        sq[k] = v;
      }
      __syncthreads();
    }
    double pn = 0.0;
    for (int k = t; k < n; k += NT) pn = fma(sq[k], sq[k], pn);
    pn = wave_sum(pn);
    if (lane == 0) s_red[wave] = pn;
    __syncthreads();
    double tot = 0.0;
    for (int w = 0; w < nwave; ++w) tot += s_red[w];
    const double qn = 1.0 / sqrt(tot);
    __syncthreads();
    if (!(tot > 1e-8 * mx)) break;
    for (int k = t; k < n; k += NT) { const double v = sq[k] * qn; sq[k] = v; Q[(size_t)R * n + k] = v; if (R < qcap) Ql[R * n + k] = v; }
    __syncthreads();
    double qv[NKR];
    double c = 0.0;
#pragma unroll
    for (int i = 0; i < NKR; ++i) {
      const int k = part + TPS * i;
      qv[i] = (k < n) ? sq[k] : 0.0;
      c = fma(qv[i], wv[i], c);
    }
    c += __shfl_xor(c, 1, 64); c += __shfl_xor(c, 2, 64);
    double r2 = 0.0;
#pragma unroll
    for (int i = 0; i < NKR; ++i) { wv[i] = fma(-c, qv[i], wv[i]); r2 = fma(wv[i], wv[i], r2); }
    r2 += __shfl_xor(r2, 1, 64); r2 += __shfl_xor(r2, 2, 64);
    res2 = r2;
    __syncthreads();
  }
  if (t == 0) { rk[0] = R; rk[1] = (R + 3) / 4; atomicMax((unsigned long long*)&stat[ST_LR_RANK], (unsigned long long)R); }
}

struct WbExch {
  double* val;
  double* col;
  unsigned int* cnt;
};

__global__ void __launch_bounds__(1024) k_wbasis_mw(const double* __restrict__ lam, int n, int S, int qcap,
                                                    double* __restrict__ Q, int* __restrict__ rk, int64_t* stat,
                                                    WbExch x) {
  extern __shared__ __attribute__((aligned(16))) double sh[];
  const int G = gridDim.x, g = blockIdx.x, NS = G * S;
  double* sq = sh;
  double* sd = sh + n;
  double* Ql = sh + 2 * n;
  double* Wl = Ql + (size_t)qcap * n;
  __shared__ double s_res[16], s_red[16], s_val[64];
  __shared__ int s_i0, s_i1;
  const int t = threadIdx.x, lane = t & 63, wave = t >> 6, NT = blockDim.x, nwave = NT >> 6;
  if (t == 0) s_i0 = 0;
  __syncthreads();
  for (int k = t; k < n; k += NT) if (lam[k] < -1e-12) s_i0 = 1;
  __syncthreads();
  if (s_i0) {
    for (size_t e = (size_t)g * NT + t; e < (size_t)n * n; e += (size_t)G * NT) Q[e] = ((e / n) == (e % n)) ? 1.0 : 0.0;
    if (g == 0 && t == 0) { rk[0] = n; rk[1] = (n + 3) / 4; stat[ST_LR_RANK] = n; }
    return;
  }
  for (int ss = wave; ss < S; ss += nwave) {
    const int s = g * S + ss;
    const double delta = (s == 0) ? 0.0 : exp(2.302585092994046 * (-6.0 + 15.0 * (double)(s - 1) / (double)(NS - 2)));
    double nrm = 0.0;
    for (int k = lane; k < n; k += 64) { const double w = 1.0 / fma(delta, fabs(lam[k]), 1.0); Wl[(size_t)ss * n + k] = w; nrm = fma(w, w, nrm); }
    nrm = wave_sum(nrm);
    const double inv = 1.0 / sqrt(nrm);
    for (int k = lane; k < n; k += 64) Wl[(size_t)ss * n + k] *= inv;
    if (lane == 0) s_res[ss] = 1.0;
  }
  const double tol2 = 2e-31 * (double)n;
  int R = 0;
  bool aborted = false;
  for (; R < n; ++R) {
    const int par = R & 1;
    __syncthreads();
    if (t == 0) {
      int b = 0;
      for (int ss = 1; ss < S; ++ss) if (s_res[ss] > s_res[b]) b = ss;
      s_i0 = b;
      x.val[par * G + g] = s_res[b];
    }
    __syncthreads();
    {
      const double* wb = Wl + (size_t)s_i0 * n;
      double* dst = x.col + ((size_t)par * G + g) * n;
      for (int k = t; k < n; k += NT) dst[k] = wb[k];
    }
    __threadfence();
    __syncthreads();
    if (t == 0) {
      __hip_atomic_fetch_add(x.cnt, 1u, __ATOMIC_RELEASE, __HIP_MEMORY_SCOPE_AGENT);
      const unsigned int target = (unsigned int)G * (unsigned int)(R + 1);
      int ok = 0;
      for (int spin = 0; spin < (1 << 22); ++spin) {
        if (__hip_atomic_load(x.cnt, __ATOMIC_ACQUIRE, __HIP_MEMORY_SCOPE_AGENT) >= target) { ok = 1; break; }
        __builtin_amdgcn_s_sleep(2);
      }
      s_i1 = ok;
    }
    __syncthreads();
    if (!s_i1) { aborted = true; break; }
    __builtin_amdgcn_fence(__ATOMIC_ACQUIRE, "agent");
    if (t < G) s_val[t] = x.val[par * G + t];
    __syncthreads();
    if (t == 0) {
      int b = 0;
      for (int w = 1; w < G; ++w) if (s_val[w] > s_val[b]) b = w;
      s_i0 = b;
    }
    __syncthreads();
    const double mx = s_val[s_i0];
    if (!(mx > tol2)) break;
    {
      const double* src = x.col + ((size_t)par * G + s_i0) * n;
      for (int k = t; k < n; k += NT) sq[k] = src[k];
    }
    __syncthreads();
    for (int pass = 0; pass < 2; ++pass) {
      for (int r = wave; r < R; r += nwave) {
        double d = 0.0;
        if (r < qcap) { for (int k = lane; k < n; k += 64) d = fma(Ql[(size_t)r * n + k], sq[k], d); }
        else { for (int k = lane; k < n; k += 64) d = fma(Q[(size_t)r * n + k], sq[k], d); }
        d = wave_sum(d);
        if (lane == 0) sd[r] = d;
      }
      __syncthreads();
      for (int k = t; k < n; k += NT) {
        double v = sq[k];
        const int rl = R < qcap ? R : qcap;
        for (int r = 0; r < rl; ++r) v = fma(-sd[r], Ql[(size_t)r * n + k], v);
        for (int r = rl; r < R; ++r) v = fma(-sd[r], Q[(size_t)r * n + k], v);
        sq[k] = v;
      }
      __syncthreads();
    }
    double pn = 0.0;
    for (int k = t; k < n; k += NT) pn = fma(sq[k], sq[k], pn);
    pn = wave_sum(pn);
    if (lane == 0) s_red[wave] = pn;
    __syncthreads();
    double tot = 0.0;
    for (int w = 0; w < nwave; ++w) tot += s_red[w];
    const double qn = 1.0 / sqrt(tot);
    if (!(tot > 1e-8 * mx)) break;
    for (int k = t; k < n; k += NT) { const double v = sq[k] * qn; sq[k] = v; Q[(size_t)R * n + k] = v; if (R < qcap) Ql[(size_t)R * n + k] = v; }
    __syncthreads();
    for (int ss = wave; ss < S; ss += nwave) {
      double* w = Wl + (size_t)ss * n;
      double c = 0.0;
      for (int k = lane; k < n; k += 64) c = fma(sq[k], w[k], c);
      c = wave_sum(c);
      double r2 = 0.0;
      for (int k = lane; k < n; k += 64) { const double v = fma(-c, sq[k], w[k]); w[k] = v; r2 = fma(v, v, r2); }
      r2 = wave_sum(r2);
      if (lane == 0) s_res[ss] = r2;
    }
  }
  if (g == 0 && t == 0) {
    if (aborted) { rk[0] = -1; rk[1] = 0; stat[ST_LR_RANK] = -1; }
    else { rk[0] = R; rk[1] = (R + 3) / 4; stat[ST_LR_RANK] = R; }
  }
}

LrSeg lr_segments(const blmm_ctx* ctx, int n) {
  LrSeg sg;
  static const char* mw_env = dev_env("BLMM_WBASIS");
  static const char* wide_env = dev_env("BLMM_LR_PANELS_WIDE");
  static const int nb_env = dev_env("BLMM_LR_PANELS_BATCH") ? atoi(dev_env("BLMM_LR_PANELS_BATCH")) : 0;
  const char* se = dev_env("BLMM_LR_SEGMENTS");
  const int want = se ? atoi(se) : ctx->tune.lr_segments;
  if (n > 80 || n < 8 || want == 1 || (mw_env && std::strcmp(mw_env, "lds") == 0) || (wide_env && wide_env[0] == '0') || nb_env > 1) return sg;
  if (want >= 2 && want <= LR_SEG_MAX) {
    sg.S = want;
    for (int i = 0; i <= LR_SEG_MAX; ++i) sg.edge[i] = (i < want) ? (double)i / want : 2.0;
    return sg;
  }
  static const double def[7] = {0.0, 0.25, 0.5, 0.7, 0.85, 0.95, 2.0};
  sg.S = 6;
  for (int i = 0; i <= LR_SEG_MAX; ++i) sg.edge[i] = (i < 7) ? def[i] : 2.0;
  return sg;
}

int launch_wbasis(blmm_ctx* ctx, const double* lam, int n, int npad, const LrSeg& seg, double* Wk, double* Q, int* rk, int64_t* stat) {
  const size_t budget = 156 * 1024, work = sizeof(double) * (size_t)2 * n, row = sizeof(double) * (size_t)n;
  if (work + row > budget) return fail(ctx, BLMM_ERR_UNSUPPORTED, "n too large for the weight-basis kernel");
  int ns = 0;
  for (int cand : {256, 192, 128})
    if (work + row * (size_t)(cand + 16) + row * 16 <= budget) { ns = cand; break; }
  static const char* mw_env = dev_env("BLMM_WBASIS");
  if (n <= 80 && !(mw_env && std::strcmp(mw_env, "lds") == 0)) {
    const int qcap = (int)std::min<size_t>(WB_QCAP, (budget - work) / row);
    const size_t lds = work + row * qcap;
    BLMM_HIP(hipFuncSetAttribute(reinterpret_cast<const void*>(&k_wbasis_reg<20>), hipFuncAttributeMaxDynamicSharedMemorySize, (int)lds));
    hipLaunchKernelGGL(k_wbasis_reg<20>, dim3((unsigned)seg.S), dim3(1024), lds, ctx->stream, lam, n, Q, rk, stat, qcap, seg, (int64_t)npad * n);
    KCHECK();
    return BLMM_OK;
  }
  if (seg.S != 1) return fail(ctx, BLMM_ERR_INVALID, "launch_wbasis: several segments need the register-resident basis kernel");
  if (ns) {
    const size_t wbytes = row * (size_t)(ns + 16);
    const int qcap = (int)std::min<size_t>(WB_QCAP, (budget - work - wbytes) / row);
    const size_t lds = work + row * qcap + wbytes;
    BLMM_HIP(hipFuncSetAttribute(reinterpret_cast<const void*>(&k_wbasis<true, 4>), hipFuncAttributeMaxDynamicSharedMemorySize, (int)lds));
    hipLaunchKernelGGL((k_wbasis<true, 4>), dim3(1), dim3(ns * 4), lds, ctx->stream, lam, n, Wk, Q, rk, stat, qcap);
    KCHECK();
    return BLMM_OK;
  }
  int S = 0;
  for (int cand : {16, 8, 4})
    if (work + row * (size_t)cand + row * 2 <= budget) { S = cand; break; }
  while (S && S < 16 && 256 / S > (ctx->num_cus > 0 ? ctx->num_cus : 256) && work + row * (size_t)(2 * S) + row * 2 <= budget) S *= 2;
  if (S && 256 / S <= (ctx->num_cus > 0 ? ctx->num_cus : 256) && !(mw_env && std::strcmp(mw_env, "single") == 0)) {
    const int G = 256 / S;
    const int qcap = (int)std::min<size_t>(WB_QCAP, (budget - work - row * S) / row);
    const size_t lds = work + row * qcap + row * S;
    WbExch x;
    x.val = Wk; x.col = Wk + 2 * G; x.cnt = reinterpret_cast<unsigned int*>(Wk + 2 * G + (size_t)2 * G * n);
    BLMM_HIP(hipMemsetAsync(x.cnt, 0, sizeof(unsigned int) * 2, ctx->stream));
    BLMM_HIP(hipFuncSetAttribute(reinterpret_cast<const void*>(&k_wbasis_mw), hipFuncAttributeMaxDynamicSharedMemorySize, (int)lds));
    GridKernelGuard gk(ctx);
    if (gk.rc) return gk.rc;
    hipLaunchKernelGGL(k_wbasis_mw, dim3(G), dim3(1024), lds, ctx->stream, lam, n, S, qcap, Q, rk, stat, x);
    KCHECK();
    return gk.record();
  }
  {
    const int qcap = (int)std::min<size_t>(WB_QCAP, (budget - work) / row);
    const size_t lds = work + row * qcap;
    BLMM_HIP(hipFuncSetAttribute(reinterpret_cast<const void*>(&k_wbasis<false, 4>), hipFuncAttributeMaxDynamicSharedMemorySize, (int)lds));
    hipLaunchKernelGGL((k_wbasis<false, 4>), dim3(1), dim3(WB_NS * 4), lds, ctx->stream, lam, n, Wk, Q, rk, stat, qcap);
  }
  KCHECK();
  return BLMM_OK;
}

template <int C, bool STAGE>
__global__ void __launch_bounds__(256) k_lr_tpanels(const double* __restrict__ Xt, int64_t ldx, int64_t p, int n,
                                                    const double* __restrict__ Z0, const double* __restrict__ Q,
                                                    const int* __restrict__ rk, double* __restrict__ T, int64_t tstride,
                                                    double* __restrict__ den0, int nchunk, int64_t qstride) {
  extern __shared__ __attribute__((aligned(16))) double sh[];
  const int sgi = blockIdx.y / nchunk;
  Q += (int64_t)sgi * qstride; rk += 4 * sgi; T += (int64_t)sgi * (1 + C) * tstride;
  const int R = rk[0], R4 = rk[1] * 4;
  const int r0 = (blockIdx.y - sgi * nchunk) * 16;
  const bool first = r0 == 0 && sgi == 0;
  if (r0 >= R4 && !first) return;
  if constexpr (STAGE) {
    for (int e = threadIdx.x; e < 16 * n; e += blockDim.x) { const int t = e / n; sh[e] = (r0 + t < R) ? Q[(size_t)(r0 + t) * n + (e % n)] : 0.0; }
    for (int e = threadIdx.x; e < C * n; e += blockDim.x) sh[16 * n + e] = Z0[e];
    __syncthreads();
  }
  auto qval = [&](int t, int k) -> double {
    if constexpr (STAGE) return sh[t * n + k];
    else return (r0 + t < R) ? Q[(size_t)(r0 + t) * n + k] : 0.0;
  };
  auto zval = [&](int q, int k) -> double {
    if constexpr (STAGE) return sh[16 * n + q * n + k];
    else return Z0[q * n + k];
  };
  const int64_t i = (int64_t)blockIdx.x * blockDim.x + threadIdx.x;
  if (i >= ldx) return;
  constexpr int NA = C * (C + 1) / 2;
  double un[1 + C], A0[NA];
#pragma unroll
  for (int q = 0; q <= C; ++q) un[q] = 0.0;
#pragma unroll
  for (int a = 0; a < NA; ++a) A0[a] = 0.0;
  double acc[1 + C][16];
#pragma unroll
  for (int q = 0; q <= C; ++q)
#pragma unroll
    for (int t = 0; t < 16; ++t) acc[q][t] = 0.0;
  if (i < p) {
    double xn[8];
#pragma unroll
    for (int u = 0; u < 8; ++u) xn[u] = (u < n) ? Xt[(int64_t)u * ldx + i] : 0.0;
// ... 808 lines not shown
```

### bulklmm.jl_amd/csrc/kernels_prep.hip

```cpp
#include "blmm_internal.h"
#include "fastmath.h"
#include <cmath>
#include <cstring>
#include <algorithm>
#include <cstdlib>
#include <type_traits>

namespace blmm {

#define KCHECK()                                                                                      \
  do {                                                                                                \
    hipError_t e__ = hipGetLastError();                                                               \
    if (e__ != hipSuccess) return fail(ctx, BLMM_ERR_HIP, std::string("kernel launch: ") + hipGetErrorString(e__)); \
  } while (0)

__global__ void k_design(const double* __restrict__ K, const double* __restrict__ Covar, int ncov, int add_intercept,
                         const double* __restrict__ wd, int n, double* __restrict__ Ks, double* __restrict__ Zs) {
  const int64_t tid = blockIdx.x * (int64_t)blockDim.x + threadIdx.x;
  const int64_t stride = (int64_t)gridDim.x * blockDim.x;
  for (int64_t e = tid; e < (int64_t)n * n; e += stride) {
    const int i = (int)(e % n), j = (int)(e / n);
    double v = K[e];
    if (wd) v *= wd[i] * wd[j];
    Ks[e] = v;
// ... 612 lines not shown
    double g = 0.0;
    for (int k = t; k < n; k += 256) g = fma(Z0[(size_t)a * n + k], Z0[(size_t)b * n + k], g);
    for (int o = 32; o > 0; o >>= 1) g += __shfl_xor(g, o, 64);
    if (lane == 0) s_g[ab][wave] = g;
  }
  __syncthreads();
  if (t == 0) {
    __shared__ double G[CMAX][2 * CMAX];
    for (int a = 0; a < c; ++a)
      for (int b = 0; b < c; ++b) {
        const int ab = a * c + b;
        G[a][b] = (s_g[ab][0] + s_g[ab][1]) + (s_g[ab][2] + s_g[ab][3]);
        G[a][c + b] = (a == b) ? 1.0 : 0.0;
      }
    for (int a = 0; a < c; ++a) {
      int piv = a;
      for (int r = a + 1; r < c; ++r) if (fabs(G[r][a]) > fabs(G[piv][a])) piv = r;
      if (piv != a) for (int b = 0; b < 2 * c; ++b) { double tt = G[a][b]; G[a][b] = G[piv][b]; G[piv][b] = tt; }
      const double d = 1.0 / G[a][a];
      for (int b = 0; b < 2 * c; ++b) G[a][b] *= d;
      for (int r = 0; r < c; ++r) if (r != a) { const double f = G[r][a]; for (int b = 0; b < 2 * c; ++b) G[r][b] -= f * G[a][b]; }
    }
    for (int a = 0; a < c; ++a) for (int b = 0; b < c; ++b) Ginv[a * CMAX + b] = G[a][c + b];
  }
  __syncthreads();
  for (int e = t; e < n * c; e += 256) {
    const int i = e % n, q = e / n;
    double sacc = 0;
    for (int r = 0; r < c; ++r) sacc = fma(Ginv[q * CMAX + r], Zs[(size_t)r * n + i], sacc);
    Bq[(size_t)q * n + i] = sacc * (wd ? wd[i] : 1.0);
  }
}
__global__ void __launch_bounds__(256) k_pe_rp(const double* __restrict__ U, const double* __restrict__ Z0,
                                               const double* __restrict__ Bq, const double* __restrict__ wd, int n, int c,
                                               int npad, int ldr, int centered, double* __restrict__ Rp) {
  __shared__ double tile[32][33];
  const int k0 = blockIdx.x * 32, i0 = blockIdx.y * 32;
  const int tx = threadIdx.x & 31, ty = threadIdx.x >> 5;
  for (int r = ty; r < 32; r += 8) {
    const int k = k0 + r, i = i0 + tx;
    tile[r][tx] = (k < n && i < n) ? U[(size_t)k * n + i] : 0.0;
  }
  __syncthreads();
  for (int r = ty; r < 32; r += 8) {
    const int i = i0 + r, k = k0 + tx;
    if (i >= npad || k >= ldr) continue;
    double v = 0.0;
    if (i < n && k < n) {
      v = tile[tx][r] * (wd ? wd[i] : 1.0);
      if (centered)
        for (int q = 0; q < c; ++q) v = fma(-Z0[(size_t)q * n + k], Bq[(size_t)q * n + i], v);
    }
    Rp[(size_t)i * ldr + k] = v;
  }
}

int launch_post_eigen(blmm_ctx* ctx, const double* lraw, const double* V, const double* Zs, const double* dweights, int n,
                      int c, int npad, int ldr, int decomp, int centered, double* lam, double* U, double* Z0, double* Rp,
                      int64_t* stat) {
  int rc = ensure(ctx, ctx->misc, sizeof(double) * ((size_t)n + (size_t)c * n + 64));
  if (rc) return rc;
  const size_t lds = sizeof(double) * ((size_t)2 * n * n + (size_t)3 * n * c + n);
  static const size_t lds_static = [] {
    hipFuncAttributes fa;
    return hipFuncGetAttributes(&fa, reinterpret_cast<const void*>(&k_post_eigen<true>)) == hipSuccess ? (size_t)fa.sharedSizeBytes : (size_t)32768;
  }();
  const PostEigenArgs pa{Zs, dweights, c, npad, ldr, decomp, centered, lam, U, Z0, Rp, ptr<double>(ctx->misc)};
  if (lds + lds_static <= 158 * 1024) {
    BLMM_HIP(hipFuncSetAttribute(reinterpret_cast<const void*>(&k_post_eigen<true>), hipFuncAttributeMaxDynamicSharedMemorySize, (int)lds));
    BLMM_LAUNCH_STOP(ctx, (k_post_eigen<true>), dim3(1), dim3(1024), lds, lraw, V, n, pa, stat);
  } else {
    double* Bq = ptr<double>(ctx->misc);
    int* rankof = reinterpret_cast<int*>(Bq + (size_t)c * n);
    hipLaunchKernelGGL(k_pe_rank, dim3((unsigned)((n + 255) / 256)), dim3(256), 0, ctx->stream, lraw, n, decomp, lam, rankof, stat);
    hipLaunchKernelGGL(k_pe_cols, dim3((unsigned)n), dim3(256), 0, ctx->stream, V, rankof, Zs, n, c, U, Z0);
    hipLaunchKernelGGL(k_pe_bq, dim3(1), dim3(256), 0, ctx->stream, Z0, Zs, dweights, n, c, Bq);
    hipLaunchKernelGGL(k_pe_rp, dim3((unsigned)((ldr + 31) / 32), (unsigned)((npad + 31) / 32)), dim3(256), 0, ctx->stream, U, Z0,
                       Bq, dweights, n, c, npad, ldr, centered, Rp);
  }
  KCHECK();
  return BLMM_OK;
}

template <int MBLK>
__global__ void __launch_bounds__(256) k_rotate(const double* __restrict__ Rp, int ldr, int n, int npad,
                                                const double* __restrict__ In, int64_t ncols,
                                                double* __restrict__ Out, int64_t ldo, int64_t ncols_pad) {
  const int lane = threadIdx.x & 63, wave = threadIdx.x >> 6;
  const int64_t col = ((int64_t)blockIdx.x * 4 + wave) * 16 + (lane & 15);
  const int rb0 = blockIdx.y * MBLK;
  const int kk = lane >> 4;
  d4 acc[MBLK];
#pragma unroll
  for (int b = 0; b < MBLK; ++b) acc[b] = (d4){0, 0, 0, 0};
  const bool colok = col < ncols;
  const double* pin = In + (colok ? col : 0) * (int64_t)n;
  for (int i0 = 0; i0 < npad; i0 += 16) {
    double bv[4], av[4][MBLK];
#pragma unroll
    for (int u = 0; u < 4; ++u) {
      const int i = i0 + 4 * u + kk;
      bv[u] = (colok && i < n) ? pin[i] : 0.0;
      const double* pr = Rp + (size_t)(i < npad ? i : 0) * ldr + (lane & 15);
#pragma unroll
      for (int b = 0; b < MBLK; ++b) {
        const int r0 = (rb0 + b) * 16;
        av[u][b] = (r0 < ldr && i < npad) ? pr[r0] : 0.0;
      }
    }
#pragma unroll
    for (int u = 0; u < 4; ++u)
#pragma unroll
      for (int b = 0; b < MBLK; ++b) acc[b] = __builtin_amdgcn_mfma_f64_16x16x4f64(av[u][b], bv[u], acc[b], 0, 0, 0);
  }
  if (col < ncols_pad) {
#pragma unroll
    for (int b = 0; b < MBLK; ++b)
#pragma unroll
      for (int r = 0; r < 4; ++r) {
        const int row = (rb0 + b) * 16 + kk + 4 * r;
        if (row < npad) Out[(int64_t)row * ldo + col] = acc[b][r];
      }
  }
}

__global__ void __launch_bounds__(256) k_rotate_vec(const double* __restrict__ Rp, int ldr, int n, int npad,
                                                    const double* __restrict__ In, int64_t col, double* __restrict__ Out,
                                                    int64_t ldo) {
  __shared__ double s_acc[4][64];
  const int lane = threadIdx.x & 63, wave = threadIdx.x >> 6;
  const int k = blockIdx.x * 64 + lane;
  const double* x = In + col * (int64_t)n;
  double a0 = 0.0, a1 = 0.0, a2 = 0.0, a3 = 0.0;
  const int kc = (k < npad) ? k : 0;
  int i = wave;
  for (; i + 28 < n; i += 32) {
    double r[8], xv[8];
#pragma unroll
    for (int u = 0; u < 8; ++u) { r[u] = Rp[(size_t)(i + 4 * u) * ldr + kc]; xv[u] = x[i + 4 * u]; }
    a0 = fma(r[0], xv[0], a0); a1 = fma(r[1], xv[1], a1); a2 = fma(r[2], xv[2], a2); a3 = fma(r[3], xv[3], a3);
    a0 = fma(r[4], xv[4], a0); a1 = fma(r[5], xv[5], a1); a2 = fma(r[6], xv[6], a2); a3 = fma(r[7], xv[7], a3);
  }
  for (; i < n; i += 4) a0 = fma(Rp[(size_t)i * ldr + kc], x[i], a0);
  const double acc = (k < npad) ? (a0 + a1) + (a2 + a3) : 0.0;
  s_acc[wave][lane] = acc;
  __syncthreads();
  if (wave == 0 && k < npad) Out[(int64_t)k * ldo + col] = (s_acc[0][lane] + s_acc[1][lane]) + (s_acc[2][lane] + s_acc[3][lane]);
}

typedef double d2ua __attribute__((ext_vector_type(2), aligned(8)));
template <int NB, bool PREF, int TR = 8>
__global__ void __launch_bounds__(256, 2) k_rotate_big(const double* __restrict__ Rp, int ldr, int n, int npad,
                                                       const double* __restrict__ In, int64_t ncols,
                                                       double* __restrict__ Out, int64_t ldo, int64_t ncols_pad, int nkt,
                                                       int64_t nct) {
  constexpr int MB = 4;
  const int lane = threadIdx.x & 63, wave = threadIdx.x >> 6;
  const int c16 = lane & 15, gq = lane >> 4;
  const int64_t bid = blockIdx.x;
  const int64_t xcd = bid & 7, idx = bid >> 3;
  const int64_t ctile = (idx / nkt) * 8 + xcd;
  const int ktile = (int)(idx % nkt);
  if (ctile >= nct) return;
  const int k0 = ktile * 128 + (wave >> 1) * 64;
  const int64_t col0 = ctile * (32 * NB) + (wave & 1) * (16 * NB);
  d4 acc[MB][NB];
#pragma unroll
  for (int a = 0; a < MB; ++a)
#pragma unroll
    for (int b = 0; b < NB; ++b) acc[a][b] = (d4){0, 0, 0, 0};
  const double* pcol[NB];
  bool cok[NB];
#pragma unroll
  for (int b = 0; b < NB; ++b) {
    const int64_t col = col0 + 16 * b + c16;
    cok[b] = col < ncols;
    pcol[b] = In + (cok[b] ? col : 0) * (int64_t)n;
  }
  auto loadB = [&](double (&bv)[NB][TR], int i0) {
#pragma unroll
    for (int b = 0; b < NB; ++b) {
      const int ib = i0 + TR * gq;
      if (cok[b] && ib + TR <= n) {
#pragma unroll
        for (int h = 0; h < TR / 2; ++h) { const d2ua v = *reinterpret_cast<const d2ua*>(pcol[b] + ib + 2 * h); bv[b][2 * h] = v[0]; bv[b][2 * h + 1] = v[1]; }
      } else {
#pragma unroll
        for (int s = 0; s < TR; ++s) bv[b][s] = (cok[b] && ib + s < n) ? pcol[b][ib + s] : 0.0;
      }
    }
  };
  auto loadA = [&](double (&av)[MB], int i) {
    const double* pr = Rp + (size_t)(i < npad ? i : 0) * ldr + c16;
#pragma unroll
    for (int a = 0; a < MB; ++a) { const int k = k0 + 16 * a; av[a] = (i < npad && k + c16 < ldr) ? pr[k] : 0.0; }
  };
  typedef unsigned int u32x4r __attribute__((ext_vector_type(4)));
// ... 28 lines not shown
#pragma unroll
    for (int a = 0; a < MB; ++a) {
      const u32x2r v = __builtin_amdgcn_raw_buffer_load_b64(srdA, voffA[a], (unsigned)irow * (unsigned)ldr * 8u, 0);
      av[a] = __builtin_bit_cast(double, v);
    }
  };
  constexpr int TRIP = 4 * TR;
  double bcur[NB][TR], bnext[PREF ? NB : 1][TR];
  const int nfull = fast ? (n / TRIP) * TRIP : 0;
  auto trip = [&](auto FTc, int i0) {
    constexpr bool FT = decltype(FTc)::value;
    if constexpr (PREF) { if (i0 + TRIP < n) { if (i0 + TRIP < nfull) loadB_fast(bnext, i0 + TRIP); else loadB(bnext, i0 + TRIP); } }
    double a0[MB], a1[MB];
    if constexpr (FT) loadA_fast(a0, i0); else loadA(a0, i0 + TR * gq);
#pragma unroll
    for (int s = 0; s < TR; s += 2) {
      if constexpr (FT) loadA_fast(a1, i0 + s + 1); else loadA(a1, i0 + TR * gq + s + 1);
#pragma unroll
      for (int a = 0; a < MB; ++a)
#pragma unroll
        for (int b = 0; b < NB; ++b) acc[a][b] = __builtin_amdgcn_mfma_f64_16x16x4f64(a0[a], bcur[b][s], acc[a][b], 0, 0, 0);
      if (s + 2 < TR) { if constexpr (FT) loadA_fast(a0, i0 + s + 2); else loadA(a0, i0 + TR * gq + s + 2); }
#pragma unroll
      for (int a = 0; a < MB; ++a)
#pragma unroll
        for (int b = 0; b < NB; ++b) acc[a][b] = __builtin_amdgcn_mfma_f64_16x16x4f64(a1[a], bcur[b][s + 1], acc[a][b], 0, 0, 0);
    }
    if (i0 + TRIP < n) {
      if constexpr (PREF) {
#pragma unroll
        for (int b = 0; b < NB; ++b)
#pragma unroll
          for (int s = 0; s < TR; ++s) bcur[b][s] = bnext[b][s];
      } else {
        if (i0 + TRIP < nfull) loadB_fast(bcur, i0 + TRIP); else loadB(bcur, i0 + TRIP);
      }
    }
  };
  if (nfull > 0) loadB_fast(bcur, 0); else loadB(bcur, 0);
  int i0 = 0;
  for (; i0 < nfull; i0 += TRIP) trip(std::true_type{}, i0);
  for (; i0 < n; i0 += TRIP) trip(std::false_type{}, i0);
#pragma unroll
  for (int a = 0; a < MB; ++a)
#pragma unroll
    for (int r = 0; r < 4; ++r) {
      const int k = k0 + 16 * a + gq + 4 * r;
      if (k >= npad) continue;
#pragma unroll
      for (int b = 0; b < NB; ++b) {
        const int64_t col = col0 + 16 * b + c16;
        if (col < ncols_pad) Out[(int64_t)k * ldo + col] = acc[a][b][r];
      }
    }
}

int launch_rotate(blmm_ctx* ctx, const double* Rp, int ldr, int n, int npad, const double* In, int64_t ncols,
                  double* Out, int64_t ldo, int64_t ncols_pad) {
  if (ncols > 0 && ncols <= 4 && n > 256) {
    BLMM_HIP(hipMemsetAsync(Out, 0, sizeof(double) * (size_t)npad * ldo, ctx->stream));
    for (int64_t col = 0; col < ncols; ++col)
      hipLaunchKernelGGL(k_rotate_vec, dim3((unsigned)((npad + 63) / 64)), dim3(256), 0, ctx->stream, Rp, ldr, n, npad, In, col, Out, ldo);
    KCHECK();
    return BLMM_OK;
  }
  if (n > 160 && ncols >= 64 && !(dev_env("BLMM_ROTATE") && std::strcmp(dev_env("BLMM_ROTATE"), "small") == 0)) {
    const int nkt = (npad + 127) / 128;
    const char* rv = dev_env("BLMM_ROTATE_TILE");
    const bool wide = !(rv && std::strcmp(rv, "64") == 0);
    const bool pref4 = rv ? std::strcmp(rv, "128p") == 0 : (n >= 900);
    const int64_t nct = (ncols_pad + (wide ? 127 : 63)) / (wide ? 128 : 64);
    const int64_t nblk = ((nct + 7) / 8) * 8 * nkt;
    if (nblk <= 0x7fffffffLL) {
      if (wide && pref4) hipLaunchKernelGGL((k_rotate_big<4, true, 4>), dim3((unsigned)nblk), dim3(256), 0, ctx->stream, Rp, ldr, n, npad, In, ncols,
                                            Out, ldo, ncols_pad, nkt, nct);
      else if (wide) hipLaunchKernelGGL((k_rotate_big<4, false>), dim3((unsigned)nblk), dim3(256), 0, ctx->stream, Rp, ldr, n, npad, In, ncols, Out, ldo,
                                   ncols_pad, nkt, nct);
      else hipLaunchKernelGGL((k_rotate_big<2, true>), dim3((unsigned)nblk), dim3(256), 0, ctx->stream, Rp, ldr, n, npad, In, ncols, Out, ldo,
                         ncols_pad, nkt, nct);
      KCHECK();
      return BLMM_OK;
    }
  }
  constexpr int MBLK = 5;
  const int nrb = (npad + 15) / 16;
  dim3 grid((unsigned)((ncols_pad + 63) / 64), (unsigned)((nrb + MBLK - 1) / MBLK));
  hipLaunchKernelGGL(k_rotate<MBLK>, grid, dim3(256), 0, ctx->stream, Rp, ldr, n, npad, In, ncols, Out, ldo, ncols_pad);
  KCHECK();
  return BLMM_OK;
}

__global__ void __launch_bounds__(256) k_rotate_vec_cols(const double* __restrict__ Rp, int ldr, int n, int npad,
                                                         const double* __restrict__ In, int64_t first, double* __restrict__ Out,
                                                         int64_t ldo) {
  __shared__ double s_acc[4][64];
  const int lane = threadIdx.x & 63, wave = threadIdx.x >> 6;
  const int k = blockIdx.x * 64 + lane;
  const int64_t col = first + blockIdx.y;
  const double* x = In + col * (int64_t)n;
  double a0 = 0.0, a1 = 0.0, a2 = 0.0, a3 = 0.0;
  const int kc = (k < npad) ? k : 0;
  int i = wave;
  for (; i + 28 < n; i += 32) {
    double r[8], xv[8];
#pragma unroll
    for (int u = 0; u < 8; ++u) { r[u] = Rp[(size_t)(i + 4 * u) * ldr + kc]; xv[u] = x[i + 4 * u]; }
    a0 = fma(r[0], xv[0], a0); a1 = fma(r[1], xv[1], a1); a2 = fma(r[2], xv[2], a2); a3 = fma(r[3], xv[3], a3);
    a0 = fma(r[4], xv[4], a0); a1 = fma(r[5], xv[5], a1); a2 = fma(r[6], xv[6], a2); a3 = fma(r[7], xv[7], a3);
  }
  for (; i < n; i += 4) a0 = fma(Rp[(size_t)i * ldr + kc], x[i], a0);
  const double acc = (k < npad) ? (a0 + a1) + (a2 + a3) : 0.0;
  s_acc[wave][lane] = acc;
  __syncthreads();
  if (wave == 0 && k < npad) Out[(int64_t)k * ldo + col] = (s_acc[0][lane] + s_acc[1][lane]) + (s_acc[2][lane] + s_acc[3][lane]);
}

int launch_rotate_single(blmm_ctx* ctx, const double* Rp, int ldr, int n, int npad, const double* In, int64_t ncols, double* Out, int64_t ldo) {
  if (ncols <= 0) return BLMM_OK;
  if (n <= 256) {
    constexpr int MBLK = 5;
    const int nrb = (npad + 15) / 16;
    dim3 grid((unsigned)((ldo + 63) / 64), (unsigned)((nrb + MBLK - 1) / MBLK));
    hipLaunchKernelGGL(k_rotate<MBLK>, grid, dim3(256), 0, ctx->stream, Rp, ldr, n, npad, In, ncols, Out, ldo, ldo);
    KCHECK();
    return BLMM_OK;
  }
  BLMM_HIP(hipMemsetAsync(Out, 0, sizeof(double) * (size_t)npad * ldo, ctx->stream));
  for (int64_t c0 = 0; c0 < ncols; c0 += 65535) {
    const int64_t nc = std::min<int64_t>(65535, ncols - c0);
    hipLaunchKernelGGL(k_rotate_vec_cols, dim3((unsigned)((npad + 63) / 64), (unsigned)nc), dim3(256), 0, ctx->stream, Rp, ldr, n, npad,
                       In, c0, Out, ldo);
  }
  KCHECK();
  return BLMM_OK;
}

__global__ void k_untranspose(const double* __restrict__ In, int64_t ld, int n, int64_t ncols, double* __restrict__ Out) {
  __shared__ double tile[32][33];
  const int64_t c0 = (int64_t)blockIdx.x * 32;
  const int r0 = blockIdx.y * 32;
  const int tx = threadIdx.x & 31, ty = threadIdx.x >> 5;
  for (int r = ty; r < 32; r += 8) {
    const int row = r0 + r; const int64_t col = c0 + tx;
    tile[r][tx] = (row < n && col < ncols) ? In[(int64_t)row * ld + col] : 0.0;
  }
  __syncthreads();
  for (int cc = ty; cc < 32; cc += 8) {
    const int64_t col = c0 + cc; const int row = r0 + tx;
    if (row < n && col < ncols) Out[col * n + row] = tile[tx][cc];
  }
}

int launch_untranspose(blmm_ctx* ctx, const double* In, int64_t ld, int n, int64_t ncols, double* Out) {
  dim3 grid((unsigned)((ncols + 31) / 32), (unsigned)((n + 31) / 32));
  hipLaunchKernelGGL(k_untranspose, grid, dim3(256), 0, ctx->stream, In, ld, n, ncols, Out);
  KCHECK();
  return BLMM_OK;
}

struct EllOut { double ell, sigma2, yy; };

template <int C, int LPT>
__device__ __forceinline__ EllOut null_ell(double h2, const double* __restrict__ ycol, int64_t ystride, int sub, int n,
                                           const double* __restrict__ sZ , const double* __restrict__ sLam,
                                           double prior_a, double prior_b, int reml, int* nonpos) {
  constexpr int NA = C * (C + 1) / 2;
  const double delta = h2 / (1.0 - h2);
  double A[NA], v[C], syy = 0.0, logsum = 0.0, prod = 1.0;
#pragma unroll
  for (int a = 0; a < NA; ++a) A[a] = 0.0;
#pragma unroll
  for (int q = 0; q < C; ++q) v[q] = 0.0;
  int cnt = 0, bad = 0;
  for (int k = sub; k < n; k += LPT) {
    const double t = fma(delta, sLam[k], 1.0);
    const double w = 1.0 / t;
    bad |= !(w > 0.0);
    prod *= t;
    if (++cnt == 8) { logsum += log(prod); prod = 1.0; cnt = 0; }
    const double y = ycol[(int64_t)k * ystride];
    const double wy = w * y;
    syy = fma(wy, y, syy);
#pragma unroll
    for (int q = 0; q < C; ++q) {
      const double zq = sZ[q * n + k];
      v[q] = fma(wy, zq, v[q]);
      const double wz = w * zq;
#pragma unroll
      for (int r = 0; r <= q; ++r) A[q * (q + 1) / 2 + r] = fma(wz, sZ[r * n + k], A[q * (q + 1) / 2 + r]);
    }
  }
  logsum += log(prod);
  syy = group_sum<LPT>(syy); logsum = group_sum<LPT>(logsum);
#pragma unroll
  for (int a = 0; a < NA; ++a) A[a] = group_sum<LPT>(A[a]);
#pragma unroll
  for (int q = 0; q < C; ++q) v[q] = group_sum<LPT>(v[q]);
  if (bad && nonpos) *nonpos = 1;
  double L[NA], t[C], logdet = 0.0, tt = 0.0;
#pragma unroll
  for (int q = 0; q < C; ++q) {
#pragma unroll
    for (int r = 0; r <= q; ++r) {
// ... 210 lines not shown
            old_old_minimizer = new_x; old_old_minimum = new_f;
          }
        }
      }
    }
    if (it >= 1000 && !done) *hit_max = 1;
    if (new_minimum < best_f || iv == 0) { best_f = new_minimum; best_x = new_minimizer; }
  }
  return best_x;
}

struct BrentState {
  double xl, xu, x, fx, step, old_step, ox, oox, ofx, oofx;
  int done;
};
template <typename F>
__device__ __forceinline__ void brent_init(F& f, BrentState& S, double a, double b, bool valid) {
  const double golden = 0.5 * (3.0 - sqrt(5.0));
  S.xl = a; S.xu = b;
  S.x = a + golden * (b - a);
  S.fx = f(S.x);
  S.step = 0.0; S.old_step = 0.0;
  S.ox = S.x; S.oox = S.x; S.ofx = S.fx; S.oofx = S.fx;
  S.done = !valid;
}
template <typename F>
__device__ __forceinline__ int brent_run(F& f, BrentState& S, int max_it) {
  const double golden = 0.5 * (3.0 - sqrt(5.0));
  const double rel_tol = 1.4901161193847656e-08, abs_tol = 2.220446049250313e-16;
  int it = 0;
  for (; it < max_it; ++it) {
    double p = 0.0, q = 0.0;
    const double x_tol = rel_tol * fabs(S.x) + abs_tol;
    const double x_mid = (S.xu + S.xl) / 2;
    if (fabs(S.x - x_mid) <= 2 * x_tol - (S.xu - S.xl) / 2) S.done = 1;
    if (__all(S.done)) break;
    if (fabs(S.old_step) > x_tol) {
      const double r = (S.x - S.ox) * (S.fx - S.oofx);
      q = (S.x - S.oox) * (S.fx - S.ofx);
      p = (S.x - S.oox) * q - (S.x - S.ox) * r;
      q = 2 * (q - r);
      if (q > 0) p = -p; else q = -q;
    }
    double nstep, nold;
    if (fabs(p) < fabs(q * S.old_step / 2) && p < q * (S.xu - S.x) && p < q * (S.x - S.xl)) {
      nold = S.step;
      nstep = p / q;
      const double x_temp = S.x + nstep;
      if ((x_temp - S.xl) < 2 * x_tol || (S.xu - x_temp) < 2 * x_tol) nstep = (S.x < x_mid) ? x_tol : -x_tol;
    } else {
      nold = (S.x < x_mid) ? S.xu - S.x : S.xl - S.x;
      nstep = golden * nold;
    }
    const double new_x = (fabs(nstep) >= x_tol) ? S.x + nstep : S.x + ((nstep > 0) ? x_tol : -x_tol);
    const double new_f = f(S.done ? S.x : new_x);
    if (!S.done) {
      S.old_step = nold; S.step = nstep;
      if (new_f < S.fx) {
        if (new_x < S.x) S.xu = S.x; else S.xl = S.x;
        S.oox = S.ox; S.oofx = S.ofx;
        S.ox = S.x; S.ofx = S.fx;
        S.x = new_x; S.fx = new_f;
      } else {
        if (new_x < S.x) S.xl = new_x; else S.xu = new_x;
        if (new_f <= S.ofx || S.ox == S.x) {
          S.oox = S.ox; S.oofx = S.ofx;
          S.ox = new_x; S.ofx = new_f;
        } else if (new_f <= S.oofx || S.oox == S.x || S.oox == S.ox) {
          S.oox = new_x; S.oofx = new_f;
        }
      }
    }
  }
  return it;
}

struct BrentCont {
  double* st;
  int* list;
  unsigned int* cnt;
  int* fin;
};

template <int C, int LPT, bool REG>
__global__ void __launch_bounds__(256, BRENT_MINW) k_brent(NullModel nm, const double* __restrict__ Yt, int64_t ldy, int64_t m,
                                               const double* __restrict__ Z0, const double* __restrict__ lam,
                                               const double* __restrict__ logtab, double* __restrict__ h2out,
                                               double* __restrict__ s2out, double* __restrict__ ellout, int64_t* stat,
                                               BrentCont cont) {
  extern __shared__ __attribute__((aligned(16))) double sh[];
  __shared__ dpair s_ln[BLMM_LOG_TABLE_N];
  const int n = nm.n;
  double* sLam = sh;
  double* sZ = sh + n;
  if (!REG) {
    for (int e = threadIdx.x; e < n; e += blockDim.x) sLam[e] = lam[e];
    for (int e = threadIdx.x; e < n * C; e += blockDim.x) sZ[e] = Z0[e];
  } else {
    stage_null_lz<C, LPT>(sh, n, Z0, lam);
  }
  stage_log_table<false>(s_ln, logtab);
  __syncthreads();
  const int64_t j = ((int64_t)blockIdx.x * blockDim.x + threadIdx.x) / LPT;
  const int sub = threadIdx.x % LPT;
  const bool valid = j < m;
  const double* ycol = Yt + (valid ? j : 0);
  int nonpos = 0, hit_max = 0;
  const int nint = nm.optim_interval < 1 ? 1 : nm.optim_interval;
  double best_x;
  EllOut fin;
  double* sY = sh + LPT * NULL_NK * (1 + C);
  if constexpr (REG) {
    stage_null_y<LPT>(sY, ycol, ldy, sub, n, valid);
    __syncthreads();
  }
  if constexpr (REG && (64 / LPT) > 1) {
    if (nint == 1) {
      constexpr int TPW = 256 / LPT;
      constexpr int TPV = 64 / LPT;
      __shared__ double s_bst[10][TPW];
      __shared__ int s_bit[TPW], s_blist[TPW], s_bnp[TPW], s_bcnt;
      NullRegs<C, LPT> R;
      R.base = sh; R.lo = sub * NULL_NK * (1 + C); R.yo = LPT * NULL_NK * (1 + C) + threadIdx.x;
      auto f = [&](double h2) { return -null_ell_reg<C, LPT>(h2, R, n, nm.prior_a, nm.prior_b, nm.reml, s_ln, &nonpos).ell; };
      BrentState S;
      brent_init(f, S, 0.0, 1.0, valid);
      const int it1 = brent_run(f, S, BRENT_PHASE1);
      fin = null_ell_reg<C, LPT>(S.x, R, n, nm.prior_a, nm.prior_b, nm.reml, s_ln, &nonpos);
      const int ts = threadIdx.x / LPT;
      wave_count(&stat[ST_H2_BOUNDARY], sub == 0 && valid && S.done && h2_on_boundary(S.x));
      if (sub == 0) {
        if (valid && cont.fin) cont.fin[j] = S.done ? 1 : 0;
        if (valid && S.done) {
          h2out[j] = S.x;
          if (s2out) s2out[j] = fin.sigma2;
          if (ellout) ellout[j] = fin.ell;
          if (nonpos) atomicAdd((unsigned long long*)&stat[ST_NONPOS_W], 1ull);
        }
        s_bst[0][ts] = S.xl; s_bst[1][ts] = S.xu; s_bst[2][ts] = S.x; s_bst[3][ts] = S.fx; s_bst[4][ts] = S.step;
        s_bst[5][ts] = S.old_step; s_bst[6][ts] = S.ox; s_bst[7][ts] = S.oox; s_bst[8][ts] = S.ofx; s_bst[9][ts] = S.oofx;
        s_bit[ts] = S.done ? -1 : it1;
        s_bnp[ts] = nonpos;
      }
      __syncthreads();
      if (threadIdx.x == 0) {
        int cnt = 0;
        for (int e = 0; e < TPW; ++e) if (s_bit[e] >= 0) s_blist[cnt++] = e;
        s_bcnt = cnt;
      }
      __syncthreads();
      const int U = s_bcnt;
      if (cont.list) {
        __shared__ unsigned int s_bbase;
        if (threadIdx.x == 0 && U > 0) s_bbase = atomicAdd(cont.cnt, (unsigned int)U);
        __syncthreads();
        for (int e = threadIdx.x; e < U; e += blockDim.x) cont.list[s_bbase + e] = (int)(blockIdx.x * TPW + s_blist[e]);
        for (int e = threadIdx.x; e < U * 12; e += blockDim.x) {
          const int fi = e / U, src = s_blist[e % U];
          const int64_t jt = (int64_t)blockIdx.x * TPW + src;
          cont.st[(int64_t)fi * m + jt] = (fi < 10) ? s_bst[fi][src] : (fi == 10 ? (double)s_bit[src] : (double)s_bnp[src]);
        }
        return;
      }
      const int wave = ((threadIdx.x >> 6) + 4 - (int)(blockIdx.x & 3)) & 3;
      if (wave * TPV >= U) return;
      const int qslot = wave * TPV + (threadIdx.x & 63) / LPT;
      const bool valid2 = qslot < U;
      const int src = s_blist[valid2 ? qslot : 0];
      const int64_t j2 = (int64_t)blockIdx.x * TPW + src;
      R.yo = LPT * NULL_NK * (1 + C) + src * LPT + sub;
      S.xl = s_bst[0][src]; S.xu = s_bst[1][src]; S.x = s_bst[2][src]; S.fx = s_bst[3][src]; S.step = s_bst[4][src];
      S.old_step = s_bst[5][src]; S.ox = s_bst[6][src]; S.oox = s_bst[7][src]; S.ofx = s_bst[8][src]; S.oofx = s_bst[9][src];
      S.done = !valid2;
      nonpos = s_bnp[src];
      const int it0 = s_bit[src];
      const int it2 = brent_run(f, S, 1000 - it0);
      fin = null_ell_reg<C, LPT>(S.x, R, n, nm.prior_a, nm.prior_b, nm.reml, s_ln, &nonpos);
      wave_count(&stat[ST_H2_BOUNDARY], valid2 && sub == 0 && h2_on_boundary(S.x));
      if (valid2 && sub == 0) {
        h2out[j2] = S.x;
        if (s2out) s2out[j2] = fin.sigma2;
        if (ellout) ellout[j2] = fin.ell;
        if (it0 + it2 >= 1000 && !S.done) atomicAdd((unsigned long long*)&stat[ST_BRENT_MAXIT], 1ull);
        if (nonpos) atomicAdd((unsigned long long*)&stat[ST_NONPOS_W], 1ull);
      }
      return;
    }
  }
  if constexpr (REG) {
    NullRegs<C, LPT> R;
    R.base = sh; R.lo = sub * NULL_NK * (1 + C); R.yo = LPT * NULL_NK * (1 + C) + threadIdx.x;
    auto f = [&](double h2) { return -null_ell_reg<C, LPT>(h2, R, n, nm.prior_a, nm.prior_b, nm.reml, s_ln, &nonpos).ell; };
    best_x = brent_search(f, nint, valid, &hit_max);
    fin = null_ell_reg<C, LPT>(best_x, R, n, nm.prior_a, nm.prior_b, nm.reml, s_ln, &nonpos);
  } else {
    auto f = [&](double h2) { return -null_ell<C, LPT>(h2, ycol, ldy, sub, n, sZ, sLam, nm.prior_a, nm.prior_b, nm.reml, &nonpos).ell; };
    best_x = brent_search(f, nint, valid, &hit_max);
    fin = null_ell<C, LPT>(best_x, ycol, ldy, sub, n, sZ, sLam, nm.prior_a, nm.prior_b, nm.reml, &nonpos);
  }
  wave_count(&stat[ST_H2_BOUNDARY], valid && sub == 0 && h2_on_boundary(best_x));
  if (valid && sub == 0) {
    h2out[j] = best_x;
    if (s2out) s2out[j] = fin.sigma2;
    if (ellout) ellout[j] = fin.ell;
    if (hit_max) atomicAdd((unsigned long long*)&stat[ST_BRENT_MAXIT], 1ull);
    if (nonpos) atomicAdd((unsigned long long*)&stat[ST_NONPOS_W], 1ull);
  }
}

template <int C, int LPT, int NK = NULL_NK>
__global__ void __launch_bounds__(256, BRENT_MINW2) k_brent2(NullModel nm, const double* __restrict__ Yt, int64_t ldy, int64_t m,
                                                const double* __restrict__ Z0, const double* __restrict__ lam,
                                                const double* __restrict__ logtab, double* __restrict__ h2out,
                                                double* __restrict__ s2out, double* __restrict__ ellout, int64_t* stat,
                                                BrentCont cont) {
  extern __shared__ __attribute__((aligned(16))) double sh[];
  __shared__ dpair s_ln[BLMM_LOG_TABLE_N];
  constexpr int TPW = 256 / LPT;
  const unsigned int U = *cont.cnt;
  if ((unsigned int)blockIdx.x * TPW >= U) return;
  const int n = nm.n;
  stage_null_lz<C, LPT, NK>(sh, n, Z0, lam);
  stage_log_table<false>(s_ln, logtab);
  double* sY = sh + LPT * NK * (1 + C);
  const unsigned int q = (unsigned int)blockIdx.x * TPW + threadIdx.x / LPT;
  const int sub = threadIdx.x % LPT;
  const bool valid = q < U;
  const int64_t j = cont.list[valid ? q : (unsigned int)blockIdx.x * TPW];
  stage_null_y<LPT, NK>(sY, Yt + j, ldy, sub, n, true);
  __syncthreads();
  int nonpos = (int)cont.st[(int64_t)11 * m + j];
  NullRegs<C, LPT> R;
  R.base = sh; R.lo = sub * NK * (1 + C); R.yo = LPT * NK * (1 + C) + threadIdx.x;
  auto f = [&](double h2) { return -null_ell_reg<C, LPT, (NK / 4 < BRENT_UNROLL2 ? NK / 4 : BRENT_UNROLL2), NK>(h2, R, n, nm.prior_a, nm.prior_b, nm.reml, s_ln, &nonpos).ell; };
  BrentState S;
  S.xl = cont.st[j]; S.xu = cont.st[m + j]; S.x = cont.st[2 * m + j]; S.fx = cont.st[3 * m + j];
  S.step = cont.st[4 * m + j]; S.old_step = cont.st[5 * m + j]; S.ox = cont.st[6 * m + j]; S.oox = cont.st[7 * m + j];
  S.ofx = cont.st[8 * m + j]; S.oofx = cont.st[9 * m + j];
  S.done = !valid;
  const int it0 = (int)cont.st[(int64_t)10 * m + j];
  const int it2 = brent_run(f, S, 1000 - it0);
  const EllOut fin = null_ell_reg<C, LPT, (NK / 4 < BRENT_UNROLL2 ? NK / 4 : BRENT_UNROLL2), NK>(S.x, R, n, nm.prior_a, nm.prior_b, nm.reml, s_ln, &nonpos);
  wave_count(&stat[ST_H2_BOUNDARY], valid && sub == 0 && h2_on_boundary(S.x));
  if (valid && sub == 0) {
    h2out[j] = S.x;
    if (s2out) s2out[j] = fin.sigma2;
    if (ellout) ellout[j] = fin.ell;
    if (it0 + it2 >= 1000 && !S.done) atomicAdd((unsigned long long*)&stat[ST_BRENT_MAXIT], 1ull);
    if (nonpos) atomicAdd((unsigned long long*)&stat[ST_NONPOS_W], 1ull);
  }
}

template <int C, int LPT, bool REG>
static int launch_brent_t(blmm_ctx* ctx, const NullModel& nm, const double* Yt, int64_t ldy, int64_t m, const double* Z0,
                          const double* lam, double* h2, double* sigma2, double* ell, int64_t* stat, int phase, BrentSplit* sp) {
  const int64_t threads = m * LPT;
  const unsigned blocks = (unsigned)((threads + 255) / 256);
  const size_t lds = REG ? sizeof(double) * ((size_t)LPT * NULL_NK * (1 + C) + (size_t)NULL_NK * 256) : sizeof(double) * (size_t)nm.n * (1 + C);
  if (lds > 48 * 1024)
    BLMM_HIP(hipFuncSetAttribute(reinterpret_cast<const void*>(&k_brent<C, LPT, REG>), hipFuncAttributeMaxDynamicSharedMemorySize, (int)lds));
  BrentCont cont{nullptr, nullptr, nullptr, nullptr};
  static const char* two_env = dev_env("BLMM_BRENT_TWO");
  const bool two = REG && (64 / LPT) > 1 && nm.optim_interval <= 1 && m >= 1024 && !(two_env && two_env[0] == '0');
  if (two) {
    int rc = ensure(ctx, ctx->brSt, sizeof(double) * (size_t)12 * m);
    if (!rc) rc = ensure(ctx, ctx->brList, sizeof(int) * 2 * (size_t)m + 16);
    if (rc) return rc;
    cont.st = ptr<double>(ctx->brSt);
    cont.cnt = reinterpret_cast<unsigned int*>(stat + ST_BRENT_CNT);
    cont.list = ptr<int>(ctx->brList) + 4;
    cont.fin = cont.list + m;
    if (phase != 2) {
      if (ctx->brent_cnt_used) BLMM_HIP(hipMemsetAsync(cont.cnt, 0, 16, ctx->stream));
      ctx->brent_cnt_used = true;
    }
  }
  if (sp) { sp->active = two && phase == 1; sp->fin = cont.fin; sp->list = cont.list; sp->cnt = cont.cnt; }
  if (phase != 2) {
    hipLaunchKernelGGL((k_brent<C, LPT, REG>), dim3(blocks), dim3(256), lds, ctx->stream, nm, Yt, ldy, m, Z0, lam,
                       ptr<double>(ctx->logtab), h2, sigma2, ell, stat, cont);
    KCHECK();
  }
  if (phase == 1 && two) return BLMM_OK;
  if (phase == 2 && !two) return BLMM_OK;
  if constexpr (REG) {
    if (two) {
      static const int lpt2_env = dev_env("BLMM_BRENT2_LPT") ? atoi(dev_env("BLMM_BRENT2_LPT")) : 0;
      auto launch2 = [&](auto kern, int lpt2, int nk2) -> int {
        const size_t lds2 = sizeof(double) * ((size_t)lpt2 * nk2 * (1 + C) + (size_t)nk2 * 256);
        if (lds2 > 48 * 1024)
          BLMM_HIP(hipFuncSetAttribute(reinterpret_cast<const void*>(kern), hipFuncAttributeMaxDynamicSharedMemorySize, (int)lds2));
        const unsigned blocks2 = (unsigned)((m * lpt2 + 255) / 256);
        hipLaunchKernelGGL(kern, dim3(blocks2), dim3(256), lds2, ctx->stream, nm, Yt, ldy, m, Z0, lam, ptr<double>(ctx->logtab), h2,
                           sigma2, ell, stat, cont);
        KCHECK();
        return BLMM_OK;
      };
      if constexpr (LPT == 4) {
        if (lpt2_env == 16 && nm.n <= 16 * 8) return launch2(&k_brent2<C, 16, 8>, 16, 8);
        if (lpt2_env == 8 && nm.n <= 8 * 12) return launch2(&k_brent2<C, 8, 12>, 8, 12);
      }
      return launch2(&k_brent2<C, LPT, NULL_NK>, LPT, NULL_NK);
    }
  }
  return BLMM_OK;
}

template <int C>
static int launch_brent_c(blmm_ctx* ctx, const NullModel& nm, const double* Yt, int64_t ldy, int64_t m, const double* Z0,
                          const double* lam, double* h2, double* sigma2, double* ell, int64_t* stat, int phase, BrentSplit* sp) {
  const int n = nm.n;
  static const int lpt_env = dev_env("BLMM_BRENT_LPT") ? atoi(dev_env("BLMM_BRENT_LPT")) : 0;
  if (lpt_env == 8 && n <= 8 * NULL_NK) return launch_brent_t<C, 8, true>(ctx, nm, Yt, ldy, m, Z0, lam, h2, sigma2, ell, stat, phase, sp);
  if (lpt_env == 16 && n <= 16 * NULL_NK) return launch_brent_t<C, 16, true>(ctx, nm, Yt, ldy, m, Z0, lam, h2, sigma2, ell, stat, phase, sp);
  if (n <= 4 * NULL_NK) return launch_brent_t<C, 4, true>(ctx, nm, Yt, ldy, m, Z0, lam, h2, sigma2, ell, stat, phase, sp);
  if (n <= 8 * NULL_NK) return launch_brent_t<C, 8, true>(ctx, nm, Yt, ldy, m, Z0, lam, h2, sigma2, ell, stat, phase, sp);
  if (n <= 16 * NULL_NK) return launch_brent_t<C, 16, true>(ctx, nm, Yt, ldy, m, Z0, lam, h2, sigma2, ell, stat, phase, sp);
  if (n <= 32 * NULL_NK) return launch_brent_t<C, 32, true>(ctx, nm, Yt, ldy, m, Z0, lam, h2, sigma2, ell, stat, phase, sp);
  if (n <= 64 * NULL_NK) return launch_brent_t<C, 64, true>(ctx, nm, Yt, ldy, m, Z0, lam, h2, sigma2, ell, stat, phase, sp);
  return launch_brent_t<C, BRENT_LPT, false>(ctx, nm, Yt, ldy, m, Z0, lam, h2, sigma2, ell, stat, phase, sp);
}

int launch_brent(blmm_ctx* ctx, const NullModel& nm, const double* Yt, int64_t ldy, int64_t m, const double* Z0,
                 const double* lam, double* h2, double* sigma2, double* ell, int64_t* stat, int phase, BrentSplit* sp) {
  if (nm.c > CTPL && nm.c <= CMAX) {
    if (sp) sp->active = false;
    return phase == 2 ? BLMM_OK : launch_dyn_brent(ctx, nm, Yt, ldy, m, Z0, lam, h2, sigma2, ell, stat);
  }
  switch (nm.c) {
    case 1: return launch_brent_c<1>(ctx, nm, Yt, ldy, m, Z0, lam, h2, sigma2, ell, stat, phase, sp);
    case 2: return launch_brent_c<2>(ctx, nm, Yt, ldy, m, Z0, lam, h2, sigma2, ell, stat, phase, sp);
    case 3: return launch_brent_c<3>(ctx, nm, Yt, ldy, m, Z0, lam, h2, sigma2, ell, stat, phase, sp);
    case 4: return launch_brent_c<4>(ctx, nm, Yt, ldy, m, Z0, lam, h2, sigma2, ell, stat, phase, sp);
#define BG(C) return launch_brent_t<C, 16, false>(ctx, nm, Yt, ldy, m, Z0, lam, h2, sigma2, ell, stat, phase, sp)
    case 5: BG(5);
    case 6: BG(6);
    case 7: BG(7);
    case 8: BG(8);
#undef BG
  }
  return fail(ctx, BLMM_ERR_UNSUPPORTED, BLMM_C_ERR);
}

template <int C, int X, int LPT, bool SQW>
__device__ __forceinline__ EllOut alt_ell(double h2, const double* __restrict__ xcol, int64_t xstride, int sub, int n,
                                          const double* __restrict__ sY, const double* __restrict__ sZ,
                                          const double* __restrict__ sLam, double prior_a, double prior_b, int reml, int* nonpos) {
  constexpr int D = C + X, NA = D * (D + 1) / 2;
  const double delta = h2 / (1.0 - h2);
  double A[NA], v[D], syy = 0.0, logsum = 0.0, prod = 1.0;
#pragma unroll
  for (int a = 0; a < NA; ++a) A[a] = 0.0;
#pragma unroll
  for (int q = 0; q < D; ++q) v[q] = 0.0;
  int cnt = 0, bad = 0;
  for (int k = sub; k < n; k += LPT) {
    const double t = fma(delta, sLam[k], 1.0);
    double w = 1.0 / t;
    bad |= !(w > 0.0);
    if (SQW) w = sqrt(w);
    prod *= t;
    if (++cnt == 8) { logsum += log(prod); prod = 1.0; cnt = 0; }
    const double y = sY[k];
    const double wy = w * y;
    syy = fma(wy, y, syy);
    double col[D];
#pragma unroll
    for (int q = 0; q < C; ++q) col[q] = sZ[q * n + k];
    if (X) col[D - 1] = xcol[(int64_t)k * xstride];
#pragma unroll
    for (int q = 0; q < D; ++q) {
      v[q] = fma(wy, col[q], v[q]);
      const double wz = w * col[q];
#pragma unroll
      for (int r = 0; r <= q; ++r) A[q * (q + 1) / 2 + r] = fma(wz, col[r], A[q * (q + 1) / 2 + r]);
    }
  }
  logsum += log(prod);
  if (SQW) logsum *= 0.5;
  syy = group_sum<LPT>(syy); logsum = group_sum<LPT>(logsum);
#pragma unroll
  for (int a = 0; a < NA; ++a) A[a] = group_sum<LPT>(A[a]);
#pragma unroll
  for (int q = 0; q < D; ++q) v[q] = group_sum<LPT>(v[q]);
  if (bad && nonpos) *nonpos = 1;
  double L[NA], t[D], logdet = 0.0, tt = 0.0;
#pragma unroll
  for (int q = 0; q < D; ++q) {
#pragma unroll
    for (int r = 0; r <= q; ++r) {
      double s = A[q * (q + 1) / 2 + r];
#pragma unroll
      for (int u = 0; u < r; ++u) s = fma(-L[q * (q + 1) / 2 + u], L[r * (r + 1) / 2 + u], s);
      if (r == q) { L[q * (q + 1) / 2 + q] = sqrt(s); logdet += log(s); }
      else L[q * (q + 1) / 2 + r] = s / L[r * (r + 1) / 2 + r];
    }
    double s = v[q];
#pragma unroll
    for (int u = 0; u < q; ++u) s = fma(-L[q * (q + 1) / 2 + u], t[u], s);
    t[q] = s / L[q * (q + 1) / 2 + q];
    tt = fma(t[q], t[q], tt);
  }
  const double rss = syy - tt;
  const double prior_df = prior_b > 0.0 ? prior_b + 2.0 : prior_b;
  const double num = rss + prior_a * prior_b;
  const double sigma2 = num / ((reml ? (double)(n - D) : (double)n) + prior_df);
  const double ls = log(sigma2);
  double ell = -0.5 * (((double)n + prior_b) * ls + logsum + num / sigma2);
  if (reml) ell += 0.5 * ((double)D * ls - logdet);
  EllOut o; o.ell = ell; o.sigma2 = sigma2; o.yy = rss;
  return o;
}

template <int C, int LPT>
__global__ void __launch_bounds__(256) k_alt_brent(NullModel nm, const double* __restrict__ Yt, int64_t ldy,
                                                   const double* __restrict__ Xt, int64_t ldx, int64_t p, const double* __restrict__ Z0,
                                                   const double* __restrict__ lam, const double* __restrict__ h2null,
// ... 956 lines not shown
```

Before: 162.9 billion.

## Start weight basis from raw eigenvalues early and fuse trait rotation into Brent

Records an event right after the eigen-pair kernel so the low-rank weight-basis kernel can start on a side stream from the raw eigenvalues, with a later check pass that reuses the result when the final eigenvalues are bit-identical and the fast eigen path is healthy. It also defers rotating the traits: the null-model Brent kernel rotates its own tile of Y into shared memory and writes Yt back, which removes a separate rotate launch and a global round trip. The aim is to overlap basis construction with the rest of the eigen work and cut launch and memory traffic. The cost is extra event and stream complexity, a possible recompute when the check fails, more shared memory in the Brent kernel, and redundant rotate work in padded blocks.

Result: no change. 165.9 billion (median of 6 runs) (+1.8%).

```diff
diff --git a/bulklmm.jl_amd/csrc/blmm_api.hip b/bulklmm.jl_amd/csrc/blmm_api.hip
--- a/bulklmm.jl_amd/csrc/blmm_api.hip
+++ b/bulklmm.jl_amd/csrc/blmm_api.hip
@@ -329,7 +329,7 @@
 }
 
 int rotate_markers(blmm_ctx* ctx, Pipe& P, const double* dG, int64_t p);
-int start_wbasis(blmm_ctx* ctx, Pipe& P, const double* dG = nullptr, int64_t p = 0, bool xt_recorded = false) {
+int start_wbasis(blmm_ctx* ctx, Pipe& P, const double* dG = nullptr, int64_t p = 0, bool xt_recorded = false, bool raw_recorded = false) {
   int rc;
   const int64_t n = P.n;
   const LrSeg seg = lr_segments(ctx, P.n);
@@ -339,6 +339,22 @@
   if (!xt_recorded) BLMM_HIP(hipEventRecord(ctx->ev_xt, ctx->stream));
   BLMM_HIP(hipStreamWaitEvent(ctx->side, ctx->ev_xt, 0));
   ctx->wb_on_side2 = false;
+  ctx->wb_raw = false;
+  if (dG && raw_recorded) {
+    BLMM_HIP(hipStreamWaitEvent(ctx->side2, ctx->ev_raw, 0));
+    ctx->wb_on_side2 = true;
+    ctx->wb_raw = true;
+    {
+      OnStream on(ctx, ctx->side2);
+      if ((rc = launch_wbasis(ctx, ptr<double>(ctx->lraw), (int)n, P.npad, seg, ptr<double>(ctx->wbW), ptr<double>(ctx->wbQ), ptr<int>(ctx->wbRk),
+                              P.stat, WB_RAW))) return rc;
+    }
+    OnStream on(ctx, ctx->side);
+    if (ctx->in_wait) BLMM_HIP(hipStreamWaitEvent(ctx->side, ctx->ev_in, 0));
+    if ((rc = rotate_markers(ctx, P, dG, p))) return rc;
+    BLMM_HIP(hipEventRecord(ctx->ev_wb, ctx->side));
+    return BLMM_OK;
+  }
   if (!dG) {
     OnStream on(ctx, ctx->side);
     return launch_wbasis(ctx, P.lam, (int)n, P.npad, seg, ptr<double>(ctx->wbW), ptr<double>(ctx->wbQ), ptr<int>(ctx->wbRk), P.stat);
@@ -375,14 +391,21 @@
 
 int prepare(blmm_ctx* ctx, const blmm_opts* o, const double* dY, int64_t n, int64_t m, const double* dG, int64_t p,
             const double* dCovar, int64_t ncov, const double* dK, const double* dweights, int centered, Pipe& P, Timer& tm,
-            bool early_wbasis = false, bool grid_side = false, bool skip_markers = false, const EigPre* pre = nullptr) {
+            bool early_wbasis = false, bool grid_side = false, bool skip_markers = false, const EigPre* pre = nullptr,
+            bool defer_traits = false) {
   if (m < 0 || p < 0) return fail(ctx, BLMM_ERR_DIM, "Dimension mismatch.");
   const bool forks = m > 0 && p > 0 && (early_wbasis || grid_side);
   ctx->stop_event_used = false;
   ctx->stop_event_next = forks ? ctx->ev_xt : nullptr;
+  const bool raw_basis = !(dev_env("BLMM_LR_RAW_BASIS") && dev_env("BLMM_LR_RAW_BASIS")[0] == '0');
+  ctx->raw_event_used = false;
+  ctx->raw_event_next = (raw_basis && early_wbasis && m > 0 && p > 0 && !pre && o->decomp_scheme != BLMM_SVD && n <= 160 &&
+                         wbasis_raw_ok((int)n)) ? ctx->ev_raw : nullptr;
   int rc = prepare_eigen(ctx, o, n, dCovar, ncov, dK, dweights, centered, P, tm, pre);
   const bool xt_recorded = ctx->stop_event_used;
+  const bool raw_recorded = ctx->raw_event_used;
   ctx->stop_event_next = nullptr; ctx->stop_event_used = false;
+  ctx->raw_event_next = nullptr; ctx->raw_event_used = false;
   if (rc) return rc;
   if (ctx->up_pending) {
     if ((rc = flush_upload(ctx))) return rc;
@@ -391,7 +414,7 @@
   const bool up_flight = ctx->in_wait;
   static const bool rot_side = !(dev_env("BLMM_ROTATE_SIDE") && dev_env("BLMM_ROTATE_SIDE")[0] == '0');
   const bool side_g = early_wbasis && m > 0 && p > 0 && rot_side && n <= 160;
-  if (early_wbasis && m > 0 && p > 0 && (rc = start_wbasis(ctx, P, side_g ? dG : nullptr, p, xt_recorded))) return rc;
+  if (early_wbasis && m > 0 && p > 0 && (rc = start_wbasis(ctx, P, side_g ? dG : nullptr, p, xt_recorded, raw_recorded && side_g))) return rc;
   P.xt_side = side_g;
   if (grid_side && !early_wbasis && m > 0 && p > 0 && rot_side && n <= 160) {
     if (!xt_recorded) BLMM_HIP(hipEventRecord(ctx->ev_xt, ctx->stream));
@@ -401,7 +424,13 @@
     if ((rc = rotate_markers(ctx, P, dG, p))) return rc;
     P.xt_side = true;
   }
-  if ((rc = rotate_traits(ctx, P, dY, m))) return rc;
+  P.Yraw = nullptr;
+  if (defer_traits && m > 0 && p > 0 && n <= eig_fast_max_n()) {
+    P.m = m; P.ldy = round_up(m, 128);
+    if ((rc = ensure(ctx, ctx->Yt, sizeof(double) * (size_t)P.npad * P.ldy))) return rc;
+    P.Yt = ptr<double>(ctx->Yt);
+    P.Yraw = dY;
+  } else if ((rc = rotate_traits(ctx, P, dY, m))) return rc;
   if (skip_markers) { P.p = p; P.ldx = round_up(p > 0 ? p : 1, 128); P.Xt = nullptr; }
   else if (!P.xt_side) {
     if (up_flight) BLMM_HIP(hipStreamWaitEvent(ctx->stream, ctx->ev_in, 0));
@@ -513,8 +542,16 @@
   hipStream_t lr_side = on2 ? ctx->side2 : ctx->side;
   OnStream on(ctx, lr_side);
   if (!wbasis_started && (rc = launch_wbasis(ctx, P.lam, P.n, P.npad, seg, ptr<double>(ctx->wbW), ptr<double>(ctx->wbQ), rk, P.stat))) return rc;
-  BLMM_HIP(hipEventRecord(ctx->ev_q, lr_side));
-  if (on2) BLMM_HIP(hipStreamWaitEvent(lr_side, ctx->ev_wb, 0));
+  if (on2 && ctx->wb_raw) {
+    BLMM_HIP(hipStreamWaitEvent(lr_side, ctx->ev_wb, 0));
+    if ((rc = launch_wbasis(ctx, P.lam, P.n, P.npad, seg, ptr<double>(ctx->wbW), ptr<double>(ctx->wbQ), rk, P.stat, WB_CHECK,
+                            ptr<double>(ctx->lraw)))) return rc;
+    BLMM_HIP(hipEventRecord(ctx->ev_q, lr_side));
+  } else {
+    BLMM_HIP(hipEventRecord(ctx->ev_q, lr_side));
+    if (on2) BLMM_HIP(hipStreamWaitEvent(lr_side, ctx->ev_wb, 0));
+  }
+  ctx->wb_raw = false;
   if ((rc = launch_lr_tpanels(ctx, P.Xt, P.ldx, P.p, P.n, P.c, P.npad, P.Z0, ptr<double>(ctx->wbQ), rk, seg, ptr<double>(ctx->lrT), tstride,
                               ptr<double>(ctx->lrDen0)))) return rc;
   BLMM_HIP(hipEventRecord(ctx->ev_join, lr_side));
@@ -711,6 +748,7 @@
       hipEventCreateWithFlags(&ctx->ev_q, hipEventDisableTiming) != hipSuccess ||
       hipEventCreateWithFlags(&ctx->ev_m, hipEventDisableTiming) != hipSuccess ||
       hipEventCreateWithFlags(&ctx->ev_wb, hipEventDisableTiming) != hipSuccess ||
+      hipEventCreateWithFlags(&ctx->ev_raw, hipEventDisableTiming) != hipSuccess ||
       hipStreamCreateWithFlags(&ctx->copy, hipStreamNonBlocking) != hipSuccess ||
       hipEventCreateWithFlags(&ctx->ev_in, hipEventDisableTiming) != hipSuccess ||
       hipEventCreateWithFlags(&ctx->ev_inY, hipEventDisableTiming) != hipSuccess ||
@@ -760,6 +798,7 @@
   if (ctx->ev_q) (void)hipEventDestroy(ctx->ev_q);
   if (ctx->ev_m) (void)hipEventDestroy(ctx->ev_m);
   if (ctx->ev_wb) (void)hipEventDestroy(ctx->ev_wb);
+  if (ctx->ev_raw) (void)hipEventDestroy(ctx->ev_raw);
   if (ctx->ev_in) (void)hipEventDestroy(ctx->ev_in);
   if (ctx->ev_inY) (void)hipEventDestroy(ctx->ev_inY);
   if (ctx->ev_call) (void)hipEventDestroy(ctx->ev_call);
@@ -1083,7 +1122,10 @@
       const bool split_on = (ctx->red_cur.flags && P.c >= 2) ? false
                           : split_env ? split_env[0] != '0' : (ctx->tune.lr_split < 0 ? m >= 8192 : ctx->tune.lr_split != 0);
       BrentSplit sp;
-      if ((rc = launch_brent(ctx, nm, P.Yt, P.ldy, m, P.Z0, P.lam, dh2_out, nullptr, nullptr, P.stat, split_on ? 1 : 0, &sp))) return rc;
+      BrentRot rot;
+      rot.Rp = ptr<double>(ctx->Rp); rot.ldr = P.ldr; rot.Y = P.Yraw;
+      if ((rc = launch_brent(ctx, nm, P.Yt, P.ldy, m, P.Z0, P.lam, dh2_out, nullptr, nullptr, P.stat, split_on ? 1 : 0, &sp,
+                             P.Yraw ? &rot : nullptr))) return rc;
       tm.mark();
       if (sp.active) { if ((rc = lr_finish_split(ctx, P, nm, dh2_out, dL_out, ldL, tm, sp))) return rc; }
       else if ((rc = lr_finish(ctx, P, nm, dh2_out, dL_out, ldL, tm))) return rc;
@@ -1185,7 +1227,8 @@
     if ((rc = grid_to_device(ctx, h2_grid_host, ngrid, &dgrid))) return rc;
   }
   const bool lowrank = wants_lowrank(ctx, opts, n, dCovar, ncov);
-  if ((rc = prepare(ctx, opts, dY, n, m, dG, p, dCovar, ncov, dK, dweights, 1, P, tm, lowrank, opts->method != BLMM_NULL_EXACT))) return rc;
+  if ((rc = prepare(ctx, opts, dY, n, m, dG, p, dCovar, ncov, dK, dweights, 1, P, tm, lowrank, opts->method != BLMM_NULL_EXACT, false, nullptr,
+                     lowrank))) return rc;
   return scan_pipeline(ctx, opts, P, tm, lowrank,  lowrank && m > 0 && p > 0, dgrid, h2_grid_host, ngrid, dL_out, ldL, dh2_out, status, pvreq);
 }
 
diff --git a/bulklmm.jl_amd/csrc/blmm_internal.h b/bulklmm.jl_amd/csrc/blmm_internal.h
--- a/bulklmm.jl_amd/csrc/blmm_internal.h
+++ b/bulklmm.jl_amd/csrc/blmm_internal.h
@@ -67,6 +67,7 @@
   int64_t* stat = nullptr;
   bool big = false;
   bool xt_side = false;
+  const double* Yraw = nullptr;
 };
 
 struct RedArgs {
@@ -95,6 +96,8 @@
   hipEvent_t ev_fork = nullptr, ev_join = nullptr, ev_xt = nullptr, ev_b1 = nullptr, ev_b2 = nullptr, ev_q = nullptr, ev_m = nullptr, ev_wb = nullptr;
   hipEvent_t stop_event_next = nullptr; bool stop_event_used = false;
   bool wb_on_side2 = false;
+  hipEvent_t ev_raw = nullptr, raw_event_next = nullptr; bool raw_event_used = false;
+  bool wb_raw = false;
   hipStream_t copy = nullptr; hipEvent_t ev_in = nullptr, ev_inY = nullptr;
   bool up_pending = false, in_wait = false;
   const void* up_src[2] = {nullptr, nullptr}; void* up_dst[2] = {nullptr, nullptr}; size_t up_bytes[2] = {0, 0};
@@ -202,9 +205,12 @@
   const int* list = nullptr;
   const unsigned int* cnt = nullptr;
 };
+struct BrentRot {
+  const double* Rp = nullptr; int ldr = 0; const double* Y = nullptr;
+};
 int launch_brent(blmm_ctx* ctx, const NullModel& nm, const double* Yt, int64_t ldy, int64_t m, const double* Z0,
                  const double* lam, double* h2, double* sigma2, double* ell, int64_t* stat, int phase = 0,
-                 BrentSplit* sp = nullptr);
+                 BrentSplit* sp = nullptr, const BrentRot* rot = nullptr);
 int launch_alt_brent(blmm_ctx* ctx, const NullModel& nm, const double* Yt, int64_t ldy, const double* Xt, int64_t ldx, int64_t p,
                      const double* Z0, const double* lam, const double* h2null, int true_w, double* lod, double* h2each,
                      int64_t* stat, int64_t m = 1, int64_t ldL = 0, int64_t ldH = 0);
@@ -320,7 +326,10 @@
                    const double* Z0, const double* lam, const double* h2, const int* list, double* L, int64_t ldL, int64_t* stat,
                    const RedArgs& red = RedArgs());
 LrSeg lr_segments(const blmm_ctx* ctx, int n);
-int launch_wbasis(blmm_ctx* ctx, const double* lam, int n, int npad, const LrSeg& seg, double* Wk, double* Q, int* rk, int64_t* stat);
+enum WbMode { WB_FULL = 0, WB_RAW = 1, WB_CHECK = 2 };
+bool wbasis_raw_ok(int n);
+int launch_wbasis(blmm_ctx* ctx, const double* lam, int n, int npad, const LrSeg& seg, double* Wk, double* Q, int* rk, int64_t* stat,
+                  int mode = WB_FULL, const double* lraw = nullptr);
 int launch_lr_tpanels(blmm_ctx* ctx, const double* Xt, int64_t ldx, int64_t p, int n, int c, int npad, const double* Z0,
                       const double* Q, const int* rk, const LrSeg& seg, double* T, int64_t tstride, double* den0);
 int launch_lr_panels(blmm_ctx* ctx, const NullModel& nm, const double* Yt, int64_t ldy, int64_t m, const double* Z0,
diff --git a/bulklmm.jl_amd/csrc/kernels_eig.hip b/bulklmm.jl_amd/csrc/kernels_eig.hip
--- a/bulklmm.jl_amd/csrc/kernels_eig.hip
+++ b/bulklmm.jl_amd/csrc/kernels_eig.hip
@@ -1435,8 +1435,14 @@
   const int64_t sG = nb > 1 ? round_up((int64_t)8 * bt_groups(n), 32) : 0;
   if ((rc = ensure(ctx, ctx->btG, nb > 1 ? sizeof(double) * (size_t)nb * sG : sizeof(double) * 8 * (size_t)bt_groups(n)))) return rc;
   double* btG = ptr<double>(ctx->btG);
-  hipLaunchKernelGGL(k_eigf_pairs<256>, dim3(n + (bt_groups(n) + 3) / 4, nb), dim3(256), 0, ctx->stream, n, (const double*)wsb, lraw, stat,
-                     (const double*)Vg, btG, sW, sL, sS, sG);
+  const dim3 pgrid(n + (bt_groups(n) + 3) / 4, nb);
+  if (nb == 1 && ctx->raw_event_next) {
+    hipExtLaunchKernelGGL(k_eigf_pairs<256>, pgrid, dim3(256), 0, ctx->stream, nullptr, ctx->raw_event_next, 0, n, (const double*)wsb, lraw, stat,
+                          (const double*)Vg, btG, sW, sL, sS, sG);
+    ctx->raw_event_next = nullptr; ctx->raw_event_used = true;
+  } else {
+    hipLaunchKernelGGL(k_eigf_pairs<256>, pgrid, dim3(256), 0, ctx->stream, n, (const double*)wsb, lraw, stat, (const double*)Vg, btG, sW, sL, sS, sG);
+  }
   KCHECK();
   static const bool bt_stage_off = dev_env("BLMM_BT_STAGE") && dev_env("BLMM_BT_STAGE")[0] == '0';
   const int stage_v = (bt_lds_staged(2, n) <= 158 * 1024 && !bt_stage_off) ? 1 : 0;
diff --git a/bulklmm.jl_amd/csrc/kernels_lowrank.hip b/bulklmm.jl_amd/csrc/kernels_lowrank.hip
--- a/bulklmm.jl_amd/csrc/kernels_lowrank.hip
+++ b/bulklmm.jl_amd/csrc/kernels_lowrank.hip
@@ -143,7 +143,8 @@
 
 template <int NKR>
 __global__ void __launch_bounds__(1024) k_wbasis_reg(const double* __restrict__ lam, int n, double* __restrict__ Q,
-                                                     int* __restrict__ rk, int64_t* stat, int qcap, LrSeg seg, int64_t qstride) {
+                                                     int* __restrict__ rk, int64_t* stat, int qcap, LrSeg seg, int64_t qstride,
+                                                     int mode, const double* __restrict__ lraw) {
   extern __shared__ __attribute__((aligned(16))) double sh[];
   constexpr int TPS = 4, NS = 256, NT = 1024;
   const int sg = blockIdx.x;
@@ -157,13 +158,24 @@
   __shared__ double s_piv_val;
   const int t = threadIdx.x, lane = t & 63, wave = t >> 6, nwave = NT >> 6;
   const int s = t / TPS, part = t % TPS;
+  if (mode == WB_CHECK) {
+    if (t == 0) s_neg = (stat[ST_EIG_FAST] == 1 && __longlong_as_double((long long)stat[ST_EIG_BAD]) <= 1.0) ? 0 : 1;
+    __syncthreads();
+    for (int k = t; k < n; k += NT) if (__double_as_longlong(lam[k]) != __double_as_longlong(lraw[k])) s_neg = 1;
+    __syncthreads();
+    if (!s_neg) {
+      if (t == 0) atomicMax((unsigned long long*)&stat[ST_LR_RANK], (unsigned long long)rk[0]);
+      return;
+    }
+    __syncthreads();
+  }
   if (t == 0) s_neg = 0;
   __syncthreads();
   for (int k = t; k < n; k += NT) if (lam[k] < -1e-12) s_neg = 1;
   __syncthreads();
   if (s_neg) {
     for (int e = t; e < n * n; e += NT) Q[e] = ((e / n) == (e % n)) ? 1.0 : 0.0;
-    if (t == 0) { rk[0] = n; rk[1] = (n + 3) / 4; stat[ST_LR_RANK] = n; }
+    if (t == 0) { rk[0] = n; rk[1] = (n + 3) / 4; if (mode != WB_RAW) atomicMax((unsigned long long*)&stat[ST_LR_RANK], (unsigned long long)n); }
     return;
   }
   double delta;
@@ -260,7 +272,7 @@
     res2 = r2;
     __syncthreads();
   }
-  if (t == 0) { rk[0] = R; rk[1] = (R + 3) / 4; atomicMax((unsigned long long*)&stat[ST_LR_RANK], (unsigned long long)R); }
+  if (t == 0) { rk[0] = R; rk[1] = (R + 3) / 4; if (mode != WB_RAW) atomicMax((unsigned long long*)&stat[ST_LR_RANK], (unsigned long long)R); }
 }
 
 struct WbExch {
@@ -413,7 +425,14 @@
   return sg;
 }
 
-int launch_wbasis(blmm_ctx* ctx, const double* lam, int n, int npad, const LrSeg& seg, double* Wk, double* Q, int* rk, int64_t* stat) {
+bool wbasis_raw_ok(int n) {
+  static const char* mw_env = dev_env("BLMM_WBASIS");
+  return n <= 80 && !(mw_env && std::strcmp(mw_env, "lds") == 0);
+}
+
+int launch_wbasis(blmm_ctx* ctx, const double* lam, int n, int npad, const LrSeg& seg, double* Wk, double* Q, int* rk, int64_t* stat,
+                  int mode, const double* lraw) {
+  if (mode != WB_FULL && !wbasis_raw_ok(n)) return fail(ctx, BLMM_ERR_INVALID, "launch_wbasis: the raw-eigenvalue start needs the register-resident basis kernel");
   const size_t budget = 156 * 1024, work = sizeof(double) * (size_t)2 * n, row = sizeof(double) * (size_t)n;
   if (work + row > budget) return fail(ctx, BLMM_ERR_UNSUPPORTED, "n too large for the weight-basis kernel");
   int ns = 0;
@@ -424,7 +443,8 @@
     const int qcap = (int)std::min<size_t>(WB_QCAP, (budget - work) / row);
     const size_t lds = work + row * qcap;
     BLMM_HIP(hipFuncSetAttribute(reinterpret_cast<const void*>(&k_wbasis_reg<20>), hipFuncAttributeMaxDynamicSharedMemorySize, (int)lds));
-    hipLaunchKernelGGL(k_wbasis_reg<20>, dim3((unsigned)seg.S), dim3(1024), lds, ctx->stream, lam, n, Q, rk, stat, qcap, seg, (int64_t)npad * n);
+    hipLaunchKernelGGL(k_wbasis_reg<20>, dim3((unsigned)seg.S), dim3(1024), lds, ctx->stream, lam, n, Q, rk, stat, qcap, seg, (int64_t)npad * n,
+                       mode, lraw ? lraw : lam);
     KCHECK();
     return BLMM_OK;
   }
diff --git a/bulklmm.jl_amd/csrc/kernels_prep.hip b/bulklmm.jl_amd/csrc/kernels_prep.hip
--- a/bulklmm.jl_amd/csrc/kernels_prep.hip
+++ b/bulklmm.jl_amd/csrc/kernels_prep.hip
@@ -718,6 +718,36 @@
   return BLMM_OK;
 }
 
+constexpr int ROT_MBLK = 5;
+template <int MBLK>
+__device__ __forceinline__ void rotate_block(const double* __restrict__ Rp, int ldr, int n, int npad, const double* __restrict__ In,
+                                             int64_t ncols, int64_t col, int rb0, d4 (&acc)[MBLK]) {
+  const int lane = threadIdx.x & 63;
+  const int kk = lane >> 4;
+#pragma unroll
+  for (int b = 0; b < MBLK; ++b) acc[b] = (d4){0, 0, 0, 0};
+  const bool colok = col < ncols;
+  const double* pin = In + (colok ? col : 0) * (int64_t)n;
+  for (int i0 = 0; i0 < npad; i0 += 16) {
+    double bv[4], av[4][MBLK];
+#pragma unroll
+    for (int u = 0; u < 4; ++u) {
+      const int i = i0 + 4 * u + kk;
+      bv[u] = (colok && i < n) ? pin[i] : 0.0;
+      const double* pr = Rp + (size_t)(i < npad ? i : 0) * ldr + (lane & 15);
+#pragma unroll
+      for (int b = 0; b < MBLK; ++b) {
+        const int r0 = (rb0 + b) * 16;
+        av[u][b] = (r0 < ldr && i < npad) ? pr[r0] : 0.0;
+      }
+    }
+#pragma unroll
+    for (int u = 0; u < 4; ++u)
+#pragma unroll
+      for (int b = 0; b < MBLK; ++b) acc[b] = __builtin_amdgcn_mfma_f64_16x16x4f64(av[u][b], bv[u], acc[b], 0, 0, 0);
+  }
+}
+
 template <int MBLK>
 __global__ void __launch_bounds__(256) k_rotate(const double* __restrict__ Rp, int ldr, int n, int npad,
                                                 const double* __restrict__ In, int64_t ncols,
@@ -727,28 +757,7 @@
   const int rb0 = blockIdx.y * MBLK;
   const int kk = lane >> 4;
   d4 acc[MBLK];
-#pragma unroll
-  for (int b = 0; b < MBLK; ++b) acc[b] = (d4){0, 0, 0, 0};
-  const bool colok = col < ncols;
-  const double* pin = In + (colok ? col : 0) * (int64_t)n;
-  for (int i0 = 0; i0 < npad; i0 += 16) {
-    double bv[4], av[4][MBLK];
-#pragma unroll
-    for (int u = 0; u < 4; ++u) {
-      const int i = i0 + 4 * u + kk;
-      bv[u] = (colok && i < n) ? pin[i] : 0.0;
-      const double* pr = Rp + (size_t)(i < npad ? i : 0) * ldr + (lane & 15);
-#pragma unroll
-      for (int b = 0; b < MBLK; ++b) {
-        const int r0 = (rb0 + b) * 16;
-        av[u][b] = (r0 < ldr && i < npad) ? pr[r0] : 0.0;
-      }
-    }
-#pragma unroll
-    for (int u = 0; u < 4; ++u)
-#pragma unroll
-      for (int b = 0; b < MBLK; ++b) acc[b] = __builtin_amdgcn_mfma_f64_16x16x4f64(av[u][b], bv[u], acc[b], 0, 0, 0);
-  }
+  rotate_block<MBLK>(Rp, ldr, n, npad, In, ncols, col, rb0, acc);
   if (col < ncols_pad) {
 #pragma unroll
     for (int b = 0; b < MBLK; ++b)
@@ -943,7 +952,7 @@
       return BLMM_OK;
     }
   }
-  constexpr int MBLK = 5;
+  constexpr int MBLK = ROT_MBLK;
   const int nrb = (npad + 15) / 16;
   dim3 grid((unsigned)((ncols_pad + 63) / 64), (unsigned)((nrb + MBLK - 1) / MBLK));
   hipLaunchKernelGGL(k_rotate<MBLK>, grid, dim3(256), 0, ctx->stream, Rp, ldr, n, npad, In, ncols, Out, ldo, ncols_pad);
@@ -979,7 +988,7 @@
 int launch_rotate_single(blmm_ctx* ctx, const double* Rp, int ldr, int n, int npad, const double* In, int64_t ncols, double* Out, int64_t ldo) {
   if (ncols <= 0) return BLMM_OK;
   if (n <= 256) {
-    constexpr int MBLK = 5;
+    constexpr int MBLK = ROT_MBLK;
     const int nrb = (npad + 15) / 16;
     dim3 grid((unsigned)((ldo + 63) / 64), (unsigned)((nrb + MBLK - 1) / MBLK));
     hipLaunchKernelGGL(k_rotate<MBLK>, grid, dim3(256), 0, ctx->stream, Rp, ldr, n, npad, In, ncols, Out, ldo, ldo);
@@ -1356,22 +1365,49 @@
   int* fin;
 };
 
+template <int LPT>
+__device__ __forceinline__ void rotate_traits_tile(const BrentRot& rot, int n, int npad, int64_t m, double* __restrict__ Yt, int64_t ldy,
+                                                   double* sY) {
+  constexpr int TPW = 256 / LPT, NCG = TPW / 16;
+  static_assert(TPW % 16 == 0, "a workgroup's traits are whole 16-column groups");
+  const int lane = threadIdx.x & 63, wave = threadIdx.x >> 6, kk = lane >> 4;
+  const int nyb = ((npad + 15) / 16 + ROT_MBLK - 1) / ROT_MBLK;
+  const int64_t j0 = (int64_t)blockIdx.x * TPW;
+  for (int task = wave; task < NCG * nyb; task += 4) {
+    const int gc = task % NCG, rb0 = (task / NCG) * ROT_MBLK;
+    const int tl = 16 * gc + (lane & 15);
+    const int64_t col = j0 + tl;
+    d4 acc[ROT_MBLK];
+    rotate_block<ROT_MBLK>(rot.Rp, rot.ldr, n, npad, rot.Y, m, col, rb0, acc);
+#pragma unroll
+    for (int b = 0; b < ROT_MBLK; ++b)
+#pragma unroll
+      for (int r = 0; r < 4; ++r) {
+        const int row = (rb0 + b) * 16 + kk + 4 * r;
+        if (row < npad) Yt[(int64_t)row * ldy + col] = acc[b][r];
+        if (row < n && col < m) sY[(row / LPT) * 256 + tl * LPT + row % LPT] = acc[b][r];
+      }
+  }
+}
+
 template <int C, int LPT, bool REG>
 __global__ void __launch_bounds__(256, BRENT_MINW) k_brent(NullModel nm, const double* __restrict__ Yt, int64_t ldy, int64_t m,
                                                const double* __restrict__ Z0, const double* __restrict__ lam,
                                                const double* __restrict__ logtab, double* __restrict__ h2out,
                                                double* __restrict__ s2out, double* __restrict__ ellout, int64_t* stat,
-                                               BrentCont cont) {
+                                               BrentCont cont, BrentRot rot, double* __restrict__ Ytw) {
   extern __shared__ __attribute__((aligned(16))) double sh[];
   __shared__ dpair s_ln[BLMM_LOG_TABLE_N];
   const int n = nm.n;
   double* sLam = sh;
   double* sZ = sh + n;
+  double* sY = sh + LPT * NULL_NK * (1 + C);
   if (!REG) {
     for (int e = threadIdx.x; e < n; e += blockDim.x) sLam[e] = lam[e];
     for (int e = threadIdx.x; e < n * C; e += blockDim.x) sZ[e] = Z0[e];
   } else {
     stage_null_lz<C, LPT>(sh, n, Z0, lam);
+    if (rot.Y) for (int e = threadIdx.x; e < NULL_NK * 256; e += blockDim.x) sY[e] = 0.0;
   }
   stage_log_table<false>(s_ln, logtab);
   __syncthreads();
@@ -1383,10 +1419,18 @@
   const int nint = nm.optim_interval < 1 ? 1 : nm.optim_interval;
   double best_x;
   EllOut fin;
-  double* sY = sh + LPT * NULL_NK * (1 + C);
+  if constexpr (REG && (256 / LPT) % 16 == 0) {
+    if (rot.Y) {
+      rotate_traits_tile<LPT>(rot, n, nm.npad, m, Ytw, ldy, sY);
+      __syncthreads();
+      if ((int64_t)blockIdx.x * (256 / LPT) >= m) return;
+    }
+  }
   if constexpr (REG) {
-    stage_null_y<LPT>(sY, ycol, ldy, sub, n, valid);
-    __syncthreads();
+    if (!rot.Y) {
+      stage_null_y<LPT>(sY, ycol, ldy, sub, n, valid);
+      __syncthreads();
+    }
   }
   if constexpr (REG && (64 / LPT) > 1) {
     if (nint == 1) {
@@ -1527,9 +1571,22 @@
 
 template <int C, int LPT, bool REG>
 static int launch_brent_t(blmm_ctx* ctx, const NullModel& nm, const double* Yt, int64_t ldy, int64_t m, const double* Z0,
-                          const double* lam, double* h2, double* sigma2, double* ell, int64_t* stat, int phase, BrentSplit* sp) {
+                          const double* lam, double* h2, double* sigma2, double* ell, int64_t* stat, int phase, BrentSplit* sp,
+                          const BrentRot* rot) {
   const int64_t threads = m * LPT;
-  const unsigned blocks = (unsigned)((threads + 255) / 256);
+  unsigned blocks = (unsigned)((threads + 255) / 256);
+  BrentRot fused{};
+  if (rot && phase != 2) {
+    const char* re = dev_env("BLMM_BRENT_ROTATE");
+    constexpr int TPW = 256 / LPT;
+    if (REG && TPW % 16 == 0 && ldy % TPW == 0 && !(re && re[0] == '0')) {
+      fused = *rot;
+      blocks = (unsigned)(ldy / TPW);
+    } else {
+      int rc = launch_rotate(ctx, rot->Rp, rot->ldr, nm.n, nm.npad, rot->Y, m, const_cast<double*>(Yt), ldy, ldy);
+      if (rc) return rc;
+    }
+  }
   const size_t lds = REG ? sizeof(double) * ((size_t)LPT * NULL_NK * (1 + C) + (size_t)NULL_NK * 256) : sizeof(double) * (size_t)nm.n * (1 + C);
   if (lds > 48 * 1024)
     BLMM_HIP(hipFuncSetAttribute(reinterpret_cast<const void*>(&k_brent<C, LPT, REG>), hipFuncAttributeMaxDynamicSharedMemorySize, (int)lds));
@@ -1552,7 +1609,7 @@
   if (sp) { sp->active = two && phase == 1; sp->fin = cont.fin; sp->list = cont.list; sp->cnt = cont.cnt; }
   if (phase != 2) {
     hipLaunchKernelGGL((k_brent<C, LPT, REG>), dim3(blocks), dim3(256), lds, ctx->stream, nm, Yt, ldy, m, Z0, lam,
-                       ptr<double>(ctx->logtab), h2, sigma2, ell, stat, cont);
+                       ptr<double>(ctx->logtab), h2, sigma2, ell, stat, cont, fused, const_cast<double*>(Yt));
     KCHECK();
   }
   if (phase == 1 && two) return BLMM_OK;
@@ -1582,31 +1639,37 @@
 
 template <int C>
 static int launch_brent_c(blmm_ctx* ctx, const NullModel& nm, const double* Yt, int64_t ldy, int64_t m, const double* Z0,
-                          const double* lam, double* h2, double* sigma2, double* ell, int64_t* stat, int phase, BrentSplit* sp) {
+                          const double* lam, double* h2, double* sigma2, double* ell, int64_t* stat, int phase, BrentSplit* sp,
+                          const BrentRot* rot) {
   const int n = nm.n;
   static const int lpt_env = dev_env("BLMM_BRENT_LPT") ? atoi(dev_env("BLMM_BRENT_LPT")) : 0;
-  if (lpt_env == 8 && n <= 8 * NULL_NK) return launch_brent_t<C, 8, true>(ctx, nm, Yt, ldy, m, Z0, lam, h2, sigma2, ell, stat, phase, sp);
-  if (lpt_env == 16 && n <= 16 * NULL_NK) return launch_brent_t<C, 16, true>(ctx, nm, Yt, ldy, m, Z0, lam, h2, sigma2, ell, stat, phase, sp);
-  if (n <= 4 * NULL_NK) return launch_brent_t<C, 4, true>(ctx, nm, Yt, ldy, m, Z0, lam, h2, sigma2, ell, stat, phase, sp);
-  if (n <= 8 * NULL_NK) return launch_brent_t<C, 8, true>(ctx, nm, Yt, ldy, m, Z0, lam, h2, sigma2, ell, stat, phase, sp);
-  if (n <= 16 * NULL_NK) return launch_brent_t<C, 16, true>(ctx, nm, Yt, ldy, m, Z0, lam, h2, sigma2, ell, stat, phase, sp);
-  if (n <= 32 * NULL_NK) return launch_brent_t<C, 32, true>(ctx, nm, Yt, ldy, m, Z0, lam, h2, sigma2, ell, stat, phase, sp);
-  if (n <= 64 * NULL_NK) return launch_brent_t<C, 64, true>(ctx, nm, Yt, ldy, m, Z0, lam, h2, sigma2, ell, stat, phase, sp);
-  return launch_brent_t<C, BRENT_LPT, false>(ctx, nm, Yt, ldy, m, Z0, lam, h2, sigma2, ell, stat, phase, sp);
+  if (lpt_env == 8 && n <= 8 * NULL_NK) return launch_brent_t<C, 8, true>(ctx, nm, Yt, ldy, m, Z0, lam, h2, sigma2, ell, stat, phase, sp, rot);
+  if (lpt_env == 16 && n <= 16 * NULL_NK) return launch_brent_t<C, 16, true>(ctx, nm, Yt, ldy, m, Z0, lam, h2, sigma2, ell, stat, phase, sp, rot);
+  if (n <= 4 * NULL_NK) return launch_brent_t<C, 4, true>(ctx, nm, Yt, ldy, m, Z0, lam, h2, sigma2, ell, stat, phase, sp, rot);
+  if (n <= 8 * NULL_NK) return launch_brent_t<C, 8, true>(ctx, nm, Yt, ldy, m, Z0, lam, h2, sigma2, ell, stat, phase, sp, rot);
+  if (n <= 16 * NULL_NK) return launch_brent_t<C, 16, true>(ctx, nm, Yt, ldy, m, Z0, lam, h2, sigma2, ell, stat, phase, sp, rot);
+  if (n <= 32 * NULL_NK) return launch_brent_t<C, 32, true>(ctx, nm, Yt, ldy, m, Z0, lam, h2, sigma2, ell, stat, phase, sp, rot);
+  if (n <= 64 * NULL_NK) return launch_brent_t<C, 64, true>(ctx, nm, Yt, ldy, m, Z0, lam, h2, sigma2, ell, stat, phase, sp, rot);
+  return launch_brent_t<C, BRENT_LPT, false>(ctx, nm, Yt, ldy, m, Z0, lam, h2, sigma2, ell, stat, phase, sp, rot);
 }
 
 int launch_brent(blmm_ctx* ctx, const NullModel& nm, const double* Yt, int64_t ldy, int64_t m, const double* Z0,
-                 const double* lam, double* h2, double* sigma2, double* ell, int64_t* stat, int phase, BrentSplit* sp) {
+                 const double* lam, double* h2, double* sigma2, double* ell, int64_t* stat, int phase, BrentSplit* sp,
+                 const BrentRot* rot) {
   if (nm.c > CTPL && nm.c <= CMAX) {
     if (sp) sp->active = false;
+    if (rot && phase != 2) {
+      const int rc = launch_rotate(ctx, rot->Rp, rot->ldr, nm.n, nm.npad, rot->Y, m, const_cast<double*>(Yt), ldy, ldy);
+      if (rc) return rc;
+    }
     return phase == 2 ? BLMM_OK : launch_dyn_brent(ctx, nm, Yt, ldy, m, Z0, lam, h2, sigma2, ell, stat);
   }
   switch (nm.c) {
-    case 1: return launch_brent_c<1>(ctx, nm, Yt, ldy, m, Z0, lam, h2, sigma2, ell, stat, phase, sp);
-    case 2: return launch_brent_c<2>(ctx, nm, Yt, ldy, m, Z0, lam, h2, sigma2, ell, stat, phase, sp);
-    case 3: return launch_brent_c<3>(ctx, nm, Yt, ldy, m, Z0, lam, h2, sigma2, ell, stat, phase, sp);
-    case 4: return launch_brent_c<4>(ctx, nm, Yt, ldy, m, Z0, lam, h2, sigma2, ell, stat, phase, sp);
-#define BG(C) return launch_brent_t<C, 16, false>(ctx, nm, Yt, ldy, m, Z0, lam, h2, sigma2, ell, stat, phase, sp)
+    case 1: return launch_brent_c<1>(ctx, nm, Yt, ldy, m, Z0, lam, h2, sigma2, ell, stat, phase, sp, rot);
+    case 2: return launch_brent_c<2>(ctx, nm, Yt, ldy, m, Z0, lam, h2, sigma2, ell, stat, phase, sp, rot);
+    case 3: return launch_brent_c<3>(ctx, nm, Yt, ldy, m, Z0, lam, h2, sigma2, ell, stat, phase, sp, rot);
+    case 4: return launch_brent_c<4>(ctx, nm, Yt, ldy, m, Z0, lam, h2, sigma2, ell, stat, phase, sp, rot);
+#define BG(C) return launch_brent_t<C, 16, false>(ctx, nm, Yt, ldy, m, Z0, lam, h2, sigma2, ell, stat, phase, sp, rot)
     case 5: BG(5);
     case 6: BG(6);
     case 7: BG(7);
```
